# ajgupta93/d4pg-pytorch

Hardware: NVIDIA H100
Metric: learner grad-steps/sec (batch 256, 51 atoms) (higher is better)
Workload: dtype f32

## Files before the change

d4pg-pytorch_b200/csrc/adam.cu:

```cuda
#include "adam_dev.cuh"
#include <math.h>
#include <cmath>
#include <algorithm>

namespace d4pg {

__global__ void __launch_bounds__(256) adam_polyak_kernel(const AdamArgs a) {
  __shared__ float red[2][8];
  pdl_trigger(a.pdl);
  pdl_wait();
  if (int(blockIdx.y) == a.nseg) {
    if (blockIdx.x == 0) adam_tail(a, red);
    return;
  }
  step_stamp(a.trace, 7);
  adam_segment<false>(a, blockIdx.y, blockIdx.x, gridDim.x);
  step_stamp(a.trace, 7 + 16);
  pdl_trigger_end(a.pdl);
}

__global__ void __launch_bounds__(256) adam_polyak_clip_kernel(const AdamArgs a) {
  __shared__ float red[2][8];
  __shared__ double bcast;
  pdl_trigger(a.pdl);
  pdl_wait();
  if (int(blockIdx.y) == a.nseg) {
    if (blockIdx.x == 0) adam_tail(a, red);
    return;
  }
  step_stamp(a.trace, 7);
  adam_segment<true>(a, blockIdx.y, blockIdx.x, gridDim.x, &bcast);
  step_stamp(a.trace, 7 + 16);
  pdl_trigger_end(a.pdl);
}

static_assert(GRAD_NORM_CTAS == 64, "clip_coef sums the partials as one warp, two per lane");
__global__ void __launch_bounds__(256) grad_sqnorm_kernel(const GradNormArgs a) {
  __shared__ double red[8];
  pdl_trigger(a.pdl);
  pdl_wait();
  const int sg = blockIdx.y;
  const float4* g4 = reinterpret_cast<const float4*>(sg ? a.g[1] : a.g[0]);
  const int64_t n4 = (sg ? a.n[1] : a.n[0]) >> 2;
  double acc = 0.0;
  for (int64_t i = blockIdx.x * int64_t(256) + threadIdx.x; i < n4; i += int64_t(GRAD_NORM_CTAS) * 256) {
    const float4 g = g4[i];
    const double x = g.x, y = g.y, z = g.z, w = g.w;
    acc += (x * x + y * y) + (z * z + w * w);
  }
  acc = warp_sum_f64(acc);
  if ((threadIdx.x & 31) == 0) red[threadIdx.x >> 5] = acc;
  __syncthreads();
  if (threadIdx.x == 0) {
    double s = 0.0;
    for (int w = 0; w < 8; ++w) s += red[w];
    (sg ? a.partials[1] : a.partials[0])[blockIdx.x] = s;
  }
  pdl_trigger_end(a.pdl);
}

int launch_grad_sqnorm(const AdamArgs& a, cudaStream_t st) {
  GradNormArgs n{};
  for (int i = 0; i < a.nseg; ++i)
    if (a.seg[i].sq_partials) {
      n.g[n.nseg] = a.seg[i].g; n.partials[n.nseg] = const_cast<double*>(a.seg[i].sq_partials); n.n[n.nseg] = a.seg[i].n;
      ++n.nseg;
    }
  D4PG_REQUIRE(n.nseg > 0, D4PG_EINVAL, "launch_grad_sqnorm: no segment clips");
  n.pdl = pdl_mode();
  D4PG_MAX_CARVEOUT(grad_sqnorm_kernel);
  D4PG_CUDA_OK(launch_pdl(grad_sqnorm_kernel, dim3(GRAD_NORM_CTAS, n.nseg), dim3(256), 0, st, n));
  return D4PG_OK;
}


int launch_adam(const AdamArgs& a_in, cudaStream_t st) {
  AdamArgs a = a_in;
  a.pdl = pdl_mode();
  a.trace = (a.clock && debug_trace_buffer()) ? debug_trace_buffer() + STEP_TRACE_BASE : nullptr;
  int64_t nmax = 0;
  for (int i = 0; i < a.nseg; ++i) nmax = a.seg[i].n > nmax ? a.seg[i].n : nmax;
  int blocks = int((nmax / 4 + 255) / 256);
  if (blocks > 4 * device_sm_count()) blocks = 4 * device_sm_count();
  if (blocks < 1) blocks = 1;
  const int tail = ((a.clock || a.loss_out) && !a.skip_tail) ? 1 : 0;
  bool ex = adam_clips(a);
  for (int i = 0; i < a.nseg; ++i) ex = ex || a.seg[i].wd != 0.f;
  if (ex) {
    D4PG_MAX_CARVEOUT(adam_polyak_clip_kernel);
    D4PG_CUDA_OK(launch_pdl(adam_polyak_clip_kernel, dim3(blocks, a.nseg + tail), dim3(256), 0, st, a));
    return D4PG_OK;
  }
  D4PG_MAX_CARVEOUT(adam_polyak_kernel);
  D4PG_CUDA_OK(launch_pdl(adam_polyak_kernel, dim3(blocks, a.nseg + tail), dim3(256), 0, st, a));
  return D4PG_OK;
}

}

using namespace d4pg;

extern "C" int32_t d4pg_adam_polyak_ex(float* p, const float* g, float* m, float* v, float* target, int64_t n,
                                       double lr, double beta1, double beta2, double eps, int64_t step,
                                       double tau, float grad_scale, d4pg_stream_t stream,
                                       double weight_decay, double max_grad_norm, double* partials, float* norm_out) {
  D4PG_REQUIRE(p && g && m && v, D4PG_EINVAL, "d4pg_adam_polyak: null buffer");
  D4PG_REQUIRE(n > 0 && n % 4 == 0, D4PG_EINVAL, "d4pg_adam_polyak: n must be a positive multiple of 4 (flat layout is 4-aligned)");
  D4PG_REQUIRE(step >= 1, D4PG_EINVAL, "d4pg_adam_polyak: step is the post-increment count (>= 1)");
  D4PG_REQUIRE(std::isfinite(weight_decay) && weight_decay >= 0.0, D4PG_EINVAL,
               "d4pg_adam_polyak_ex: weight_decay must be finite and >= 0 (got %g)", weight_decay);
  D4PG_REQUIRE(max_grad_norm == 0.0 || max_grad_norm > 0.0, D4PG_EINVAL,
               "d4pg_adam_polyak_ex: max_grad_norm must be 0 (off), +inf (report only) or > 0 (got %g)", max_grad_norm);
  D4PG_REQUIRE(max_grad_norm == 0.0 || partials, D4PG_EINVAL,
               "d4pg_adam_polyak_ex: clipping needs a device workspace of %d doubles", GRAD_NORM_CTAS);
  AdamArgs a{};
  const double bc1 = 1.0 - pow(beta1, double(step));
  const double bc2 = 1.0 - pow(beta2, double(step));
  a.seg[0] = AdamSeg{p, g, m, v, target, n, nullptr, 0, float(-(lr / bc1)), -1};
  a.seg[0].wd = float(weight_decay);
  if (max_grad_norm > 0.0) { a.seg[0].sq_partials = partials; a.seg[0].max_norm = max_grad_norm; a.seg[0].norm_out = norm_out; }
  a.nseg = 1;
  a.w1 = float(1.0 - beta1); a.w2 = float(1.0 - beta2); a.beta2 = float(beta2); a.eps = float(eps);
  a.bc2_sqrt = float(sqrt(bc2)); a.tau = float(tau); a.one_minus_tau = float(1.0 - tau);
  a.grad_scale = grad_scale; a.pipe_slot = -1;
  if (adam_clips(a))
    if (int rc = launch_grad_sqnorm(a, as_stream(stream))) return rc;
  return launch_adam(a, as_stream(stream));
}

extern "C" int32_t d4pg_adam_polyak(float* p, const float* g, float* m, float* v, float* target, int64_t n,
                                    double lr, double beta1, double beta2, double eps, int64_t step,
                                    double tau, float grad_scale, d4pg_stream_t stream) {
  return d4pg_adam_polyak_ex(p, g, m, v, target, n, lr, beta1, beta2, eps, step, tau, grad_scale, stream, 0.0, 0.0, nullptr, nullptr);
}

namespace d4pg {
__global__ void polyak_kernel(float* t, const float* s, int64_t n, float tau, float omt) {
  for (int64_t i = blockIdx.x * int64_t(blockDim.x) + threadIdx.x; i < n; i += int64_t(gridDim.x) * blockDim.x)
    t[i] = __fadd_rn(__fmul_rn(omt, t[i]), __fmul_rn(tau, s[i]));
}
}

extern "C" int32_t d4pg_polyak(float* target, const float* src, int64_t n, double tau, d4pg_stream_t stream) {
  D4PG_REQUIRE(target && src && n > 0, D4PG_EINVAL, "d4pg_polyak: bad arguments");
  int blocks = int(std::min<int64_t>(4 * d4pg::device_sm_count(), (n + 255) / 256));
  polyak_kernel<<<blocks, 256, 0, as_stream(stream)>>>(target, src, n, float(tau), float(1.0 - tau));
  D4PG_LAUNCH_OK();
  return D4PG_OK;
}

extern "C" int32_t d4pg_copy_f32(float* dst, const float* src, int64_t n, d4pg_stream_t stream) {
  D4PG_REQUIRE(dst && src && n >= 0, D4PG_EINVAL, "d4pg_copy_f32: bad arguments");
  D4PG_CUDA_OK(cudaMemcpyAsync(dst, src, size_t(n) * sizeof(float), cudaMemcpyDeviceToDevice, as_stream(stream)));
  return D4PG_OK;
}
```

d4pg-pytorch_b200/csrc/adam.cuh:

```cuda
#pragma once
#include "common.cuh"

namespace d4pg {

struct LearnerClock {
  int64_t adam_step;
  int64_t beta_t;
  int64_t steps_done;
  int64_t reserved;
  float beta;
  float neg_step_size[2];
  float bc2_sqrt;
  float pad;
  int64_t s_adam_step, s_beta_t, s_steps_done;
  float d_neg_step_size[2][2];
  float d_bc2_sqrt[2];
};

struct ClockParams {
  double lr_actor, lr_critic, beta1, beta2;
  double per_beta0, per_beta_final; int64_t per_beta_iters;
};

__device__ __forceinline__ void clock_derive_pipelined(LearnerClock* c, const ClockParams& a, int slot) {
  const double step = double(c->s_adam_step + 1);
  const double bc1 = 1.0 - pow(a.beta1, step);
  const double bc2 = 1.0 - pow(a.beta2, step);
  c->d_neg_step_size[slot][0] = float(-(a.lr_actor / bc1));
  c->d_neg_step_size[slot][1] = float(-(a.lr_critic / bc1));
  c->d_bc2_sqrt[slot] = float(sqrt(bc2));
}
__device__ __forceinline__ void clock_derive(LearnerClock* c, const ClockParams& a) {
  const double step = double(c->adam_step + 1);
  const double bc1 = 1.0 - pow(a.beta1, step);
  const double bc2 = 1.0 - pow(a.beta2, step);
  c->neg_step_size[0] = float(-(a.lr_actor / bc1));
  c->neg_step_size[1] = float(-(a.lr_critic / bc1));
  c->bc2_sqrt = float(sqrt(bc2));
}
__device__ __forceinline__ float clock_beta(const LearnerClock* c, const ClockParams& a, bool pipelined = false) {
  const double frac = fmin(double(pipelined ? c->s_beta_t : c->beta_t) / double(a.per_beta_iters), 1.0);
  return float(a.per_beta0 + frac * (a.per_beta_final - a.per_beta0));
}

constexpr int D4PG_MAX_PEERS = 8;
struct PeerSignal {
  unsigned long long* local;
  unsigned long long* inbox[8];
  int world;
};
__device__ __forceinline__ void peer_signal_last_cta(const PeerSignal& s, unsigned nblocks) {
  __threadfence();
  unsigned long long* f = s.local;
  if (atomicAdd(f + 2, 1ull) == nblocks - 1) {
    f[2] = 0ull;
    const unsigned long long v = f[1] + 1ull;
    f[1] = v;
    __threadfence_system();
    for (int p = 0; p < s.world; ++p) asm volatile("st.relaxed.sys.global.u64 [%0], %1;" ::"l"(s.inbox[p]), "l"(v) : "memory");
  }
}
__device__ __forceinline__ void peer_wait_all(const unsigned long long* block, int world) {
  const int r = threadIdx.x;
  if (r < world) {
    const unsigned long long target = __ldcg(block + 1);
    unsigned long long v;
    do {
      asm volatile("ld.acquire.sys.global.u64 %0, [%1];" : "=l"(v) : "l"(block + 8 + r) : "memory");
    } while (v < target);
  }
  __syncthreads();
}

struct PeerInfo {
  int world, rank; int64_t n;
  float* x[D4PG_MAX_PEERS]; float* red[D4PG_MAX_PEERS];
  unsigned long long* flag[D4PG_MAX_PEERS]; unsigned long long* flag2[D4PG_MAX_PEERS];
  const float* mc; float* mc_uc;
};

struct AdamImgLayer { int64_t w_off, w_end; int ld, nchunks; uint8_t* img; uint8_t* img_t; };
struct AdamSeg {
  float* p; const float* g; float* m; float* v; float* target; int64_t n;
  float* g_out; int64_t g_off;
  float neg_step_size; int clock_slot;
  AdamImgLayer imgl[4]; int nimg;
  const double* sq_partials;
  double max_norm;
  float* norm_out;
  float wd;
};
struct AdamArgs {
  AdamSeg seg[2]; int nseg;
  float w1, w2, beta2, eps, bc2_sqrt, tau, one_minus_tau, grad_scale;
  LearnerClock* clock;
  unsigned long long* trace;
  const float* peer_g[D4PG_MAX_PEERS]; int npeers;
  const float* mc_g;
  int peer_reduced;
  const unsigned long long* my_flags; int rank;
  int pipe_slot;
  const float* loss_rows; const float* pi_rows; int B; float inv_count; float* loss_out;
  int pdl;
  int skip_tail;
};
int launch_adam(const AdamArgs& a, cudaStream_t st);

constexpr int GRAD_NORM_CTAS = 64;
constexpr double GRAD_NORM_EPS = 1e-6;
struct GradNormArgs { const float* g[2]; double* partials[2]; int64_t n[2]; int nseg; int pdl; };
static inline bool adam_clips(const AdamArgs& a) {
  for (int i = 0; i < a.nseg; ++i) if (a.seg[i].sq_partials) return true;
  return false;
}
int launch_grad_sqnorm(const AdamArgs& a, cudaStream_t st);


}
```

d4pg-pytorch_b200/csrc/common.cuh:

```cuda
#pragma once
#include <cuda_runtime.h>
#include <stdint.h>
#include <stdio.h>
#include <stdarg.h>
#include "../../include/d4pg_b200.h"

namespace d4pg {

void set_error(const char* fmt, ...);

#define D4PG_CUDA_OK(expr)                                                              \
  do {                                                                                  \
    cudaError_t _e = (expr);                                                            \
    if (_e != cudaSuccess) {                                                            \
      ::d4pg::set_error("%s:%d: %s -> %s", __FILE__, __LINE__, #expr, cudaGetErrorString(_e)); \
      return D4PG_ECUDA;                                                                \
    }                                                                                   \
  } while (0)

#define D4PG_REQUIRE(cond, code, ...)                                                   \
  do {                                                                                  \
    if (!(cond)) { ::d4pg::set_error(__VA_ARGS__); return (code); }                     \
  } while (0)

#define D4PG_LAUNCH_OK()                                                                \
  do {                                                                                  \
    cudaError_t _e = cudaGetLastError();                                                \
    if (_e != cudaSuccess) {                                                            \
      ::d4pg::set_error("%s:%d: kernel launch -> %s", __FILE__, __LINE__, cudaGetErrorString(_e)); \
      return D4PG_ECUDA;                                                                \
    }                                                                                   \
  } while (0)

#define D4PG_MAX_CARVEOUT(kernel)                                                                     \
  do {                                                                                                \
    static bool _carved = false;                                                                      \
    if (!_carved) {                                                                                   \
      cudaFuncSetAttribute(kernel, cudaFuncAttributePreferredSharedMemoryCarveout,                    \
                           int(cudaSharedmemCarveoutMaxShared));                                      \
      _carved = true;                                                                                 \
    }                                                                                                 \
  } while (0)

__device__ __forceinline__ void pdl_trigger_raw() { asm volatile("griddepcontrol.launch_dependents;" ::: "memory"); }
__device__ __forceinline__ void pdl_trigger(int mode) { if (mode == 1) pdl_trigger_raw(); }
__device__ __forceinline__ void pdl_trigger_end(int mode) { if (mode == 2) pdl_trigger_raw(); }
int pdl_mode();
int device_sm_count();
__device__ __forceinline__ void pdl_wait() { asm volatile("griddepcontrol.wait;" ::: "memory"); }
bool pdl_enabled();
template <typename... KArgs, typename... Args>
static inline cudaError_t launch_pdl(void (*kernel)(KArgs...), dim3 grid, dim3 block, size_t smem, cudaStream_t st,
                                     Args... args) {
  cudaLaunchConfig_t cfg{};
  cfg.gridDim = grid; cfg.blockDim = block; cfg.dynamicSmemBytes = smem; cfg.stream = st;
  cudaLaunchAttribute attr[1];
  attr[0].id = cudaLaunchAttributeProgrammaticStreamSerialization;
  attr[0].val.programmaticStreamSerializationAllowed = 1;
  cfg.attrs = attr; cfg.numAttrs = pdl_enabled() ? 1 : 0;
  return cudaLaunchKernelEx(&cfg, kernel, KArgs(args)...);
}

__device__ __forceinline__ void step_stamp(unsigned long long* tr, int slot) {
  if (tr && blockIdx.x == 0 && blockIdx.y == 0 && threadIdx.x == 0) {
    unsigned long long t;
    asm volatile("mov.u64 %0, %%globaltimer;" : "=l"(t));
    tr[slot] = t;
  }
}
unsigned long long* debug_trace_buffer();
constexpr int STEP_TRACE_BASE = 96;

static inline cudaStream_t as_stream(d4pg_stream_t s) { return reinterpret_cast<cudaStream_t>(s); }

__host__ __device__ static inline int64_t align4(int64_t x) { return (x + 3) & ~int64_t(3); }
__host__ __device__ static inline int cdiv(int a, int b) { return (a + b - 1) / b; }

__device__ __forceinline__ float warp_sum(float v) {
#pragma unroll
  for (int o = 16; o > 0; o >>= 1) v += __shfl_xor_sync(0xffffffffu, v, o);
  return v;
}
__device__ __forceinline__ float warp_max(float v) {
#pragma unroll
  for (int o = 16; o > 0; o >>= 1) v = fmaxf(v, __shfl_xor_sync(0xffffffffu, v, o));
  return v;
}

struct Philox {
  __device__ static inline void round(uint32_t (&c)[4], uint32_t k0, uint32_t k1) {
    const uint32_t M0 = 0xD2511F53u, M1 = 0xCD9E8D57u;
    uint32_t hi0 = __umulhi(M0, c[0]), lo0 = M0 * c[0];
    uint32_t hi1 = __umulhi(M1, c[2]), lo1 = M1 * c[2];
    uint32_t n0 = hi1 ^ c[1] ^ k0, n1 = lo1, n2 = hi0 ^ c[3] ^ k1, n3 = lo0;
    c[0] = n0; c[1] = n1; c[2] = n2; c[3] = n3;
  }
  __device__ static inline double uniform53(uint64_t seed, uint64_t counter, uint32_t lane) {
    uint32_t c[4] = {uint32_t(counter), uint32_t(counter >> 32), lane, 0x9E3779B9u};
    uint32_t k0 = uint32_t(seed), k1 = uint32_t(seed >> 32);
#pragma unroll
    for (int i = 0; i < 10; ++i) {
      round(c, k0, k1);
      k0 += 0x9E3779B9u; k1 += 0xBB67AE85u;
    }
    uint32_t a = c[0] >> 5, b = c[1] >> 6;
    return (double(a) * 67108864.0 + double(b)) * (1.0 / 9007199254740992.0);
  }
};

enum GemmEpi {
  EPI_NONE = 0, EPI_BIAS = 1, EPI_BIAS_RELU = 2, EPI_BIAS_TANH = 3,
  EPI_RELU_MASK = 4,
  EPI_TANH_MASK = 5
};
struct NetDims {
  int in[4], out[4];
  int ld[4];
  int epi[4];
  int64_t w_off[4], b_off[4];
  int64_t total;
};
static inline int dx_mask(const NetDims& d, int l) {
  return l > 0 && d.epi[l - 1] == EPI_BIAS_RELU ? EPI_RELU_MASK : EPI_NONE;
}
__host__ __device__ static inline int pitch4(int x) { return (x + 3) & ~3; }
NetDims actor_dims(int obs_dim, int act_dim);
NetDims critic_dims(int obs_dim, int act_dim, int n_atoms);

}
```

d4pg-pytorch_b200/csrc/gemm_ffma.cu:

```cuda
#include "gemm_ffma_dev.cuh"
#include "mlp_chain.cuh"
#include <algorithm>

namespace d4pg {

template <bool ALLOW_SPLIT>
__global__ void __launch_bounds__(GEMM_THREADS, 2) gemm_ffma_kernel(const __grid_constant__ GemmBatch batch) {
  __shared__ __align__(16) float smem[2 * KC * LDS_A + 2 * KC * LDS_B];
  static_assert(2 * KC * LDS_A + 2 * KC * LDS_B >= GEMM_WARPS * BM * BN, "partial-tile buffer must fit");
  pdl_trigger(batch.pdl);
  pdl_wait();
  int pi = 0;
#pragma unroll
  for (int i = 1; i < GEMM_MAX_PROBLEMS; ++i)
    if (i < batch.n && int(blockIdx.x) >= batch.p[i].tile_begin) pi = i;
  const GemmProblem P = batch.p[pi];
  gemm_tile_dispatch<ALLOW_SPLIT>(P, smem, blockIdx.x - P.tile_begin);
  pdl_trigger_end(batch.pdl);
}

template <bool ALLOW_SPLIT>
__global__ void __launch_bounds__(GEMM_THREADS, 3) gemm_wide_kernel(const __grid_constant__ GemmWideBatch batch) {
  extern __shared__ __align__(16) float smem[];
  pdl_trigger(batch.pdl);
  pdl_wait();
  int pi = 0;
#pragma unroll
  for (int i = 1; i < GEMM_WIDE_MAX; ++i)
    if (i < batch.n && int(blockIdx.x) >= batch.p[i].tile_begin) pi = i;
  const GemmProblem& P = batch.p[pi];
  const int tile = blockIdx.x - P.tile_begin;
  step_stamp(batch.trace, 6);
  if (ALLOW_SPLIT && P.ksplit > 1) {
    const int per_slice = P.tiles_m * P.tiles_n;
    const int ks = tile / per_slice, t2 = tile - ks * per_slice;
    const int tm = t2 / P.tiles_n, tn = t2 - tm * P.tiles_n;
    const int kbeg = ks * P.kslice;
    gemm_dw_tile_async<true>(P, smem, tm * BM, tn * BN, tn, kbeg, min(P.K, kbeg + P.kslice));
  } else {
    const int tm = tile / P.tiles_n, tn = tile - tm * P.tiles_n;
    gemm_dw_tile_async<false>(P, smem, tm * BM, tn * BN, tn, 0, P.K);
  }
  step_stamp(batch.trace, 6 + 16);
  if (batch.has_peer_sig) {
    __syncthreads();
    if (threadIdx.x == 0) peer_signal_last_cta(batch.peer_sig, gridDim.x);
  }
  pdl_trigger_end(batch.pdl);
}

GemmProblem gemm_fwd(const float* X, int ldx, const float* X2, int ldx2, int K1, const float* W, int ldw,
                     const float* bias, float* Y, int ldy, int M, int N, int K, int epi) {
  GemmProblem p{};
  p.A = X; p.lda = ldx; p.A2 = X2 ? X2 : X; p.lda2 = X2 ? ldx2 : ldx; p.K1 = X2 ? K1 : K;
  p.Bm = W; p.ldb = ldw; p.bias = bias; p.C = Y; p.ldc = ldy; p.M = M; p.N = N; p.K = K;
  p.mode = GEMM_FWD; p.epi = epi;
  return p;
}
GemmProblem gemm_dx(const float* dZ, int lddz, const float* W, int ldw, float* dX, int lddx,
                    int M, int N_in, int K_out, int epi, const float* aux, int ldaux) {
  GemmProblem p{};
  p.A = dZ; p.lda = lddz; p.A2 = dZ; p.lda2 = lddz; p.K1 = K_out;
  p.Bm = W; p.ldb = ldw; p.C = dX; p.ldc = lddx; p.M = M; p.N = N_in; p.K = K_out;
  p.mode = GEMM_DX; p.epi = epi; p.aux = aux; p.ldaux = ldaux;
  return p;
}
GemmProblem gemm_dw(const float* dZ, int lddz, const float* X, int ldx, float* dW, int lddw,
                    float* db, int N_out, int K_in, int M_batch) {
  GemmProblem p{};
  p.A = dZ; p.lda = lddz; p.A2 = dZ; p.lda2 = lddz; p.K1 = M_batch;
  p.Bm = X; p.ldb = ldx; p.C = dW; p.ldc = lddw; p.bias_grad = db;
  p.M = N_out; p.N = K_in; p.K = M_batch;
  p.mode = GEMM_DW; p.epi = EPI_NONE;
  return p;
}
void gemm_batch_begin(GemmBatch& b) { b.n = 0; b.total_tiles = 0; b.trace = nullptr; }
static bool aligned16(const void* p) { return (reinterpret_cast<uintptr_t>(p) & 15) == 0; }
static void prepare_problem(GemmProblem& p) {
  bool avec, bvec;
  if (p.mode == GEMM_DW) avec = aligned16(p.A) && p.lda % 4 == 0 && p.M % 4 == 0;
  else avec = aligned16(p.A) && p.lda % 4 == 0 && p.K1 % 4 == 0;
  if (p.mode == GEMM_FWD) bvec = aligned16(p.Bm) && p.ldb % 4 == 0 && p.K % 4 == 0;
  else bvec = aligned16(p.Bm) && p.ldb % 4 == 0 && p.N % 4 == 0;
  p.flags = (avec ? GEMM_A_VEC : 0) | (bvec ? GEMM_B_VEC : 0);
  if (p.mode == GEMM_DW && aligned16(p.A) && p.lda % 4 == 0 && aligned16(p.Bm) && p.ldb % 4 == 0) p.flags |= GEMM_ASYNC_OK;
  p.ksplit = 1; p.kslice = p.K;
  if (p.mode == GEMM_DW && p.K >= 1024) {
    p.ksplit = std::min(8, cdiv(p.K, 512));
    p.kslice = cdiv(cdiv(p.K, p.ksplit), 64) * 64;
    p.ksplit = cdiv(p.K, p.kslice);
  }
  p.tiles_m = cdiv(p.M, BM); p.tiles_n = cdiv(p.N, BN);
}
void gemm_batch_add(GemmBatch& b, const GemmProblem& pin) {
  GemmProblem p = pin;
  prepare_problem(p);
  p.tile_begin = b.total_tiles;
  b.total_tiles += p.tiles_m * p.tiles_n * p.ksplit;
  b.p[b.n++] = p;
}
void gemm_batch_retile(GemmBatch& b, int bm, int bn) {
  b.total_tiles = 0;
  for (int i = 0; i < b.n; ++i) {
    GemmProblem& p = b.p[i];
    p.tiles_m = cdiv(p.M, bm); p.tiles_n = cdiv(p.N, bn); p.tile_begin = b.total_tiles;
    b.total_tiles += p.tiles_m * p.tiles_n * p.ksplit;
  }
}
void gemm_wide_begin(GemmWideBatch& b, const PeerSignal* sig) {
  b.n = 0; b.total_tiles = 0; b.pdl = 0; b.trace = nullptr; b.has_peer_sig = sig ? 1 : 0;
  if (sig) b.peer_sig = *sig;
}
void gemm_wide_add(GemmWideBatch& b, const GemmProblem& pin) {
  if (b.n >= GEMM_WIDE_MAX) { b.n = GEMM_WIDE_MAX + 1; return; }
  GemmProblem p = pin;
  prepare_problem(p);
  p.tile_begin = b.total_tiles;
  b.total_tiles += p.tiles_m * p.tiles_n * p.ksplit;
  b.p[b.n++] = p;
}
int gemm_wide_launch(GemmWideBatch& b, cudaStream_t st) {
  D4PG_REQUIRE(b.n > 0 && b.n <= GEMM_WIDE_MAX, D4PG_EINVAL, "gemm_wide_launch: %d problems (max %d)", b.n, GEMM_WIDE_MAX);
  bool split = false;
  for (int i = 0; i < b.n; ++i) {
    split = split || b.p[i].ksplit > 1;
    D4PG_REQUIRE(b.p[i].mode == GEMM_DW && (b.p[i].flags & GEMM_ASYNC_OK), D4PG_ENOTSUP,
                 "gemm_wide_launch: problem %d is not a dW with 16-B aligned, 16-B pitched operands", i);
  }
  D4PG_MAX_CARVEOUT(gemm_wide_kernel<false>);
  D4PG_MAX_CARVEOUT(gemm_wide_kernel<true>);
  const size_t smem = DW_SMEM_FLOATS * sizeof(float);
  static bool smem_set = false;
  if (!smem_set) {
    D4PG_CUDA_OK(cudaFuncSetAttribute(gemm_wide_kernel<false>, cudaFuncAttributeMaxDynamicSharedMemorySize, int(smem)));
    D4PG_CUDA_OK(cudaFuncSetAttribute(gemm_wide_kernel<true>, cudaFuncAttributeMaxDynamicSharedMemorySize, int(smem)));
    smem_set = true;
  }
  b.pdl = pdl_mode();
  b.trace = debug_trace_buffer() ? debug_trace_buffer() + STEP_TRACE_BASE : nullptr;
  if (split) D4PG_CUDA_OK(launch_pdl(gemm_wide_kernel<true>, dim3(b.total_tiles), dim3(GEMM_THREADS), smem, st, b));
  else D4PG_CUDA_OK(launch_pdl(gemm_wide_kernel<false>, dim3(b.total_tiles), dim3(GEMM_THREADS), smem, st, b));
  return D4PG_OK;
}
bool gemm_batch_has_splitk(const GemmBatch& b) {
  for (int i = 0; i < b.n; ++i) if (b.p[i].ksplit > 1) return true;
  return false;
}
int gemm_launch(GemmBatch& b, int precision, cudaStream_t st) {
  if (precision == 0) return gemm_batch_launch(b, st);
  if (precision == 3) return gemm_bf16_batch_launch(b, st);
  gemm_tc_prepare(b);
  return gemm_tc_batch_launch(b, precision == 1 ? 3 : 1, st);
}
int gemm_batch_launch(const GemmBatch& b, cudaStream_t st) {
  D4PG_REQUIRE(b.n > 0 && b.n <= GEMM_MAX_PROBLEMS, D4PG_EINVAL, "gemm_batch_launch: %d problems", b.n);
  for (int i = 0; i < b.n; ++i)
    D4PG_REQUIRE(b.p[i].mode != GEMM_FWD || b.p[i].K1 == b.p[i].K || b.p[i].K1 % KC == 0, D4PG_ENOTSUP,
                 "gemm_batch_launch: concat split K1=%d must be a multiple of %d", b.p[i].K1, KC);
  D4PG_MAX_CARVEOUT(gemm_ffma_kernel<false>);
  D4PG_MAX_CARVEOUT(gemm_ffma_kernel<true>);
  const_cast<GemmBatch&>(b).pdl = pdl_mode();
  if (gemm_batch_has_splitk(b)) D4PG_CUDA_OK(launch_pdl(gemm_ffma_kernel<true>, dim3(b.total_tiles), dim3(GEMM_THREADS), 0, st, b));
  else D4PG_CUDA_OK(launch_pdl(gemm_ffma_kernel<false>, dim3(b.total_tiles), dim3(GEMM_THREADS), 0, st, b));
  return D4PG_OK;
}

}
```

d4pg-pytorch_b200/csrc/learner.cu:

```cuda
#include "common.cuh"
#include "gemm_ffma.cuh"
#include "adam.cuh"
#include <string.h>
#include <stdlib.h>
#include <initializer_list>
#include <new>
#include <string>
#include <vector>

#include "internal.cuh"
#include "mlp_chain.cuh"
#include "mlp_tc_chain.cuh"

namespace d4pg {

struct Batch { float *s, *a, *s2; double* r; uint8_t* done; int32_t* idx; float* wts; uint8_t* hz; };

struct Workspace {
  Batch batch[2];
  float *h1[5], *h2[5], *h3[5], *out[5];
  float *m, *q_probs, *target_probs, *dlogits_q, *dlogits_pi, *loss_rows, *pi_rows;
  float *c_dz22, *c_dz2, *c_dz1, *p_dz22, *p_dz2, *a_dz3, *a_dz22, *a_dh2, *a_dz1;
  LearnerClock* clock;
  float* xchg;
  unsigned long long* pipe_epoch;
  double* sq_partials;
  int64_t total;
};

enum StepPlan { PLAN_LEVELS, PLAN_CHAIN, PLAN_TC_CHAIN };
constexpr int CHAIN_MAX_BATCH = 512;
static bool chain_pre_ok(const d4pg_learner_config_t& c) { return c.precision == 0 && c.act_dim <= 8; }
static bool chain_plan_fits(const d4pg_learner_config_t& c) {
  const int H = D4PG_HIDDEN, S = c.obs_dim, A = c.act_dim, N = c.n_atoms;
  ChainArgs f, b;
  chain_args_begin(f, c.batch, nullptr, c.precision);
  chain_add(f, 0, chain_fwd(nullptr, 0, nullptr, H, S, EPI_BIAS_RELU, nullptr, 0, 1));
  chain_add(f, 0, chain_fwd(nullptr, 0, nullptr, H, H, EPI_BIAS_RELU, nullptr, 0, 1));
  ChainSlot fc2 = chain_fwd(nullptr, 0, nullptr, H, H + A, EPI_BIAS_RELU, nullptr, 0, 1);
  if (chain_pre_ok(c)) chain_pre_layer(fc2, nullptr, 0, nullptr, nullptr, 0, A, H, EPI_BIAS_TANH, nullptr, 0, 0, H, false);
  else chain_add(f, 0, chain_fwd(nullptr, 0, nullptr, A, H, EPI_BIAS_TANH, nullptr, 0, 1));
  chain_add(f, 0, fc2);
  chain_add(f, 0, chain_fwd(nullptr, 0, nullptr, N, H, EPI_BIAS, nullptr, 0, 0));
  chain_args_begin(b, c.batch, nullptr, c.precision);
  chain_add(b, 0, chain_dx(nullptr, 0, H, N, EPI_RELU_MASK, nullptr, 0, nullptr, 0, 1));
  chain_add(b, 0, chain_dx(nullptr, 0, H, H, EPI_RELU_MASK, nullptr, 0, nullptr, 0, 1));
  ChainSlot fc3 = chain_dx(nullptr, 0, H, A, EPI_RELU_MASK, nullptr, 0, nullptr, 0, 1);
  if (chain_pre_ok(c)) chain_pre_layer(fc3, nullptr, 0, nullptr, nullptr, 0, A, H, EPI_TANH_MASK, nullptr, 0, 0, H, true);
  else chain_add(b, 0, chain_dx(nullptr, 0, A, H, EPI_TANH_MASK, nullptr, 0, nullptr, 0, 1));
  chain_add(b, 0, fc3);
  return chain_fits(f) && chain_fits(b);
}
static StepPlan step_plan(const d4pg_learner_config_t& c) {
  if (c.batch > CHAIN_MAX_BATCH || c.chain != 1) return PLAN_LEVELS;
  if (c.precision == 3) return PLAN_LEVELS;
  if (c.precision >= 1 && c.obs_dim <= 32 && c.act_dim <= 32 && c.n_atoms <= 256) return PLAN_TC_CHAIN;
  return chain_plan_fits(c) ? PLAN_CHAIN : PLAN_LEVELS;
}
static d4pg_learner_config_t with_head_width(const d4pg_learner_config_t& c) {
  d4pg_learner_config_t e = c;
  if (c.dist_type == 1) e.n_atoms = 3 * c.n_components;
  return e;
}
static_assert((CHAIN_MAX_BATCH + SAMPLE_ROWS - 1) / SAMPLE_ROWS <= TCC_THREADS, "sampler epochs exceed the chain CTA's threads");

static Workspace carve(float* base, int B, int S, int A, int N, StepPlan plan, bool prefetch, bool clip, bool tails) {
  Workspace w{};
  int64_t off = 0;
  auto take = [&](int64_t n) { float* p = base ? base + off : nullptr; off += align4(n); return p; };
  const int H = D4PG_HIDDEN, Sp = pitch4(S), Ap = pitch4(A), Np = pitch4(N);
  auto take_rows = [&](Batch& h) {
    h.s = take(int64_t(B) * Sp); h.a = take(int64_t(B) * Ap); h.s2 = take(int64_t(B) * Sp);
    h.r = reinterpret_cast<double*>(take(int64_t(B) * 2));
    h.done = reinterpret_cast<uint8_t*>(take((B + 3) / 4));
  };
  take_rows(w.batch[0]);
  for (int k = 0; k < 5; ++k) {
    if (k != 4) w.h1[k] = take(int64_t(B) * H);
    w.h2[k] = take(int64_t(B) * H); w.h3[k] = take(int64_t(B) * H);
  }
  w.out[0] = take(int64_t(B) * Ap); w.out[3] = take(int64_t(B) * Ap);
  w.out[1] = take(int64_t(B) * Np); w.out[2] = take(int64_t(B) * Np); w.out[4] = take(int64_t(B) * Np);
  w.m = take(int64_t(B) * Np); w.q_probs = take(int64_t(B) * Np); w.target_probs = take(int64_t(B) * Np);
  w.dlogits_q = take(int64_t(B) * Np); w.dlogits_pi = take(int64_t(B) * Np);
  w.loss_rows = take(B); w.pi_rows = take(B);
  w.c_dz22 = take(int64_t(B) * H); w.c_dz2 = take(int64_t(B) * H); w.c_dz1 = take(int64_t(B) * H);
  w.p_dz22 = take(int64_t(B) * H); w.p_dz2 = take(int64_t(B) * H);
  w.a_dz3 = take(int64_t(B) * Ap); w.a_dz22 = take(int64_t(B) * H); w.a_dh2 = take(int64_t(B) * H);
  w.a_dz1 = take(int64_t(B) * H);
  w.clock = reinterpret_cast<LearnerClock*>(take(sizeof(LearnerClock) / 4 + 4));
  w.xchg = plan != PLAN_LEVELS ? take(std::max(chain_xchg_floats(B), tcc_xchg_floats(B))) : nullptr;
  w.pipe_epoch = reinterpret_cast<unsigned long long*>(take(2 * int64_t((B + SAMPLE_ROWS - 1) / SAMPLE_ROWS)));
  if (prefetch) {
    take_rows(w.batch[1]);
    for (int k = 0; k < 2; ++k) { w.batch[k].idx = reinterpret_cast<int32_t*>(take(B)); w.batch[k].wts = take(B); }
  }
  if (clip) w.sq_partials = reinterpret_cast<double*>(take(2 * GRAD_NORM_CTAS * 2));
  if (tails)
    for (int k = 0; k < (prefetch ? 2 : 1); ++k) w.batch[k].hz = reinterpret_cast<uint8_t*>(take((B + 3) / 4));
  w.total = off;
  return w;
}
}

using namespace d4pg;

struct d4pg_learner {
  d4pg_learner_config_t cfg;
  d4pg_learner_buffers_t buf;
  d4pg_replay* replay;
  d4pg_comm* comm;
  StepPlan plan;
  Workspace ws;
  NetDims da, dc;
  ClockParams clock_params;
  cudaGraphExec_t graph_exec[4];
  bool graph_ready[4];
  cudaGraphExec_t multi_exec[2];
  bool multi_ready[2];
  int pipe_par;
  int last_par;
  bool prefetch_valid;
  int64_t seen_gen;
  int64_t steps_done;
  int kernels_per_step;
  cudaStream_t side; cudaEvent_t ev_fork, ev_join;
  ChainArgs chain_fwd_args, chain_bwd_args;
  uint8_t* tcc_images; TccPackArgs tcc_pack_fwd, tcc_pack_dx; TccImage tcc_img[32];
  cudaEvent_t ev_fork2, ev_join2;
  TccArgs tcc_fwd_args, tcc_bwd_args;
  GemmWideBatch dw_batch;
  double* host_u[4]; int32_t* host_pos[4]; float* host_losses; cudaEvent_t ev_in, ev_out, ev_h2d[4];
  int64_t host_steps;
  float* loss_ring[2]; cudaEvent_t ev_loss[2]; int64_t loss_steps;
  cudaStream_t ing; cudaEvent_t ev_ing; unsigned long long* gate_flag;
  bool images_dirty;
  const float* norm_affine; float norm_clip;
  double* gtab;
  bool profiling;
  std::vector<cudaEvent_t> ev;
  std::vector<std::string> ev_name;
  std::vector<int> ev_reps;
};

static bool prefetching(const d4pg_learner_config_t& c) { return c.prefetch != 0 && c.sample_mode == 1; }
static bool host_pipe(const d4pg_learner_config_t& c) { return c.prefetch != 0 && c.sample_mode == 0 && c.use_graph != 0; }
static bool piped(const d4pg_learner_config_t& c) { return prefetching(c) || host_pipe(c); }
static bool clipping(const d4pg_learner_config_t& c) { return c.max_grad_norm_actor != 0.0 || c.max_grad_norm_critic != 0.0; }

enum Net { ACTOR, ACTOR_TARGET, CRITIC, CRITIC_TARGET };
struct Layer { const float* W; int ldw; const float* bias; int n_out, k_in, epi; };
static Layer layer(const d4pg_learner* L, Net net, int l) {
  const bool critic = net >= CRITIC;
  const NetDims& d = critic ? L->dc : L->da;
  const float* P[4] = {L->buf.actor, L->buf.actor_target, L->buf.critic, L->buf.critic_target};
  return Layer{P[net] + d.w_off[l], d.ld[l], P[net] + d.b_off[l], d.out[l], d.in[l], d.epi[l]};
}
static int64_t critic_fc2_action_off(const d4pg_learner* L) { return L->dc.w_off[1] + D4PG_HIDDEN; }
struct LayerDx { const float* W; int ldw, n_in, k_out; };
static LayerDx layer_dx(const d4pg_learner* L, Net net, int l) {
  const Layer y = layer(L, net, l);
  return LayerDx{y.W, y.ldw, (net == CRITIC && l == 1) ? D4PG_HIDDEN : y.k_in, y.n_out};
}
static LayerDx critic_fc2_action_dx(const d4pg_learner* L) {
  return LayerDx{L->buf.critic + critic_fc2_action_off(L), L->dc.ld[1], L->cfg.act_dim, D4PG_HIDDEN};
}

enum { U_A_F1, U_A_F2, U_A_F22, U_A_F3, U_A_D3, U_A_D22, U_A_D2, U_AT_F1, U_AT_F2, U_AT_F22, U_AT_F3,
       U_C_F1, U_C_F2, U_C_F22, U_C_F3, U_C_D3, U_C_D22, U_C_D2H, U_C_D2A, U_CT_F1, U_CT_F2, U_CT_F22, U_CT_F3, U_COUNT };
static int fwd_image(Net net, int l) {
  const int fc1[4] = {U_A_F1, U_AT_F1, U_C_F1, U_CT_F1};
  return fc1[net] + l;
}

static int tcc_setup(d4pg_learner* L) {
  TccPackArgs& pf = L->tcc_pack_fwd; TccPackArgs& pd = L->tcc_pack_dx;
  tcc_pack_begin(pf, nullptr); tcc_pack_begin(pd, nullptr);
  int use_of[U_COUNT]; bool is_dx[U_COUNT];
  auto add_dx = [&](int id, const LayerDx& d) {
    is_dx[id] = true;
    use_of[id] = tcc_pack_add(pd, d.W, d.ldw, GEMM_DX, d.n_in, d.k_out);
  };
  for (int net = ACTOR; net <= CRITIC_TARGET; ++net)
    for (int l = 0; l < 4; ++l) {
      const Layer y = layer(L, Net(net), l);
      const int id = fwd_image(Net(net), l);
      is_dx[id] = false;
      use_of[id] = tcc_pack_add(pf, y.W, y.ldw, GEMM_FWD, y.n_out, y.k_in);
    }
  add_dx(U_A_D3, layer_dx(L, ACTOR, 3));
  add_dx(U_A_D22, layer_dx(L, ACTOR, 2));
  add_dx(U_A_D2, layer_dx(L, ACTOR, 1));
  add_dx(U_C_D3, layer_dx(L, CRITIC, 3));
  add_dx(U_C_D22, layer_dx(L, CRITIC, 2));
  add_dx(U_C_D2H, layer_dx(L, CRITIC, 1));
  add_dx(U_C_D2A, critic_fc2_action_dx(L));
  for (int i = 0; i < U_COUNT; ++i) D4PG_REQUIRE(use_of[i] >= 0, D4PG_ENOTSUP, "tcc_setup: too many weight images");
  const long long fwd_bytes = tcc_pack_bytes(pf), all_bytes = fwd_bytes + tcc_pack_bytes(pd);
  D4PG_CUDA_OK(cudaMalloc(&L->tcc_images, size_t(all_bytes)));
  D4PG_CUDA_OK(cudaMemset(L->tcc_images, 0, size_t(all_bytes)));
  tcc_pack_set_base(pf, L->tcc_images, 0);
  tcc_pack_set_base(pd, L->tcc_images, fwd_bytes);
  for (int i = 0; i < U_COUNT; ++i) L->tcc_img[i] = tcc_image(is_dx[i] ? pd : pf, use_of[i]);
  (void)tcc_watchdog_device();
  return D4PG_OK;
}

enum Exchange { XCHG_NONE, XCHG_ALLREDUCE, XCHG_PULL, XCHG_MC, XCHG_MC2, XCHG_RS };
static Exchange exchange_mode(d4pg_learner* L, PeerInfo* peers) {
  if (L->cfg.world_size <= 1) return XCHG_NONE;
  if (!comm_peer_info(L->comm, peers)) return XCHG_ALLREDUCE;
  static const int comm_mode = [] { const char* e = getenv("D4PG_COMM_MODE");
                                    return !e ? 0 : (e[0] == 'p' ? 1 : (e[0] == 'r' ? 2 : (e[0] == 'm' && e[1] == 'c' && e[2] == '2' ? 4 : 3))); }();
  static const int mc_from = [] { const char* e = getenv("D4PG_COMM_MC_FROM"); return e ? atoi(e) : 3; }();
  static const int mc2_from = [] { const char* e = getenv("D4PG_COMM_MC2_FROM"); return e ? atoi(e) : 1000; }();
  const bool mc_avail = peers->mc != nullptr && L->plan != PLAN_LEVELS;
  if (mc_avail && (comm_mode == 4 || (comm_mode == 0 && peers->world >= mc2_from))) return XCHG_MC2;
  if (mc_avail && (comm_mode == 3 || (comm_mode == 0 && peers->world >= mc_from))) return XCHG_MC;
  return comm_mode == 2 ? XCHG_RS : XCHG_PULL;
}

struct Step {
  d4pg_learner* L; cudaStream_t st;
  const d4pg_learner_config_t& c; const d4pg_learner_buffers_t& b; const Workspace& w;
  Batch bt;
  int par; bool cold;
  bool pf;
  bool h7;
  int B, S, A, N, Sp, Ap, Np;
  Exchange xm; PeerInfo peers; int gpar;
  float *Ga, *Gc;
  int nk;
};
static bool peer_exchange(const Step& x) { return x.xm >= XCHG_PULL; }

constexpr int PROFILE_REPS = 16;
template <class F>
static int run_launch(Step& x, const char* name, bool repeatable, F launch) {
  d4pg_learner* L = x.L;
  int rc;
  if (L->profiling) {
    cudaEvent_t e0, e1; cudaEventCreate(&e0); cudaEventCreate(&e1);
    cudaEventRecord(e0, x.st); rc = launch();
    for (int r = 1; repeatable && r < PROFILE_REPS && rc == 0; ++r) rc = launch();
    cudaEventRecord(e1, x.st);
    L->ev.push_back(e0); L->ev.push_back(e1); L->ev_reps.push_back(repeatable ? PROFILE_REPS : 1);
    L->ev_name.push_back(name);
  } else rc = launch();
  if (rc == 0) ++x.nk;
  return rc;
}
#define RUN(name, repeatable, call) \
  do { if (int rc_ = run_launch(x, name, repeatable, [&] { return (call); })) return rc_; } while (0)
static int run_level(Step& x, std::initializer_list<GemmProblem> problems) {
  GemmBatch g;
  gemm_batch_begin(g);
  for (const GemmProblem& p : problems) gemm_batch_add(g, p);
  RUN("gemm_launch", !gemm_batch_has_splitk(g), gemm_launch(g, x.c.precision, x.st));
  return D4PG_OK;
}

static int sample_batch(Step& x) {
  const d4pg_learner_config_t& c = x.c;
  RUN("learner_sample", false,
      learner_sample(x.L->replay, x.B, c.prioritized, c.sample_mode == 0 ? x.b.uniforms : nullptr,
                     (c.sample_mode == 0 && !c.prioritized) ? x.b.positions : nullptr,
                     c.philox_seed, x.w.clock, x.L->clock_params,
                     x.bt.idx, x.bt.wts, x.bt.s, x.bt.a, x.bt.r, x.bt.s2, x.bt.done, x.bt.hz, x.Sp, x.Ap, x.L->norm_affine,
                     x.L->norm_clip, x.pf ? x.par : -1, x.st));
  return D4PG_OK;
}

static void tcc_begin(const Step& x, TccArgs& a, int step_slot) {
  tcc_args_begin(a, x.B, reinterpret_cast<uint8_t*>(x.w.xchg), x.c.precision == 1 ? 3 : 1);
  a.step_slot = step_slot;
}
static int tcc_fwd_group(TccArgs& fa, int ci, int sl, const Step& x, Net net, int l, float* C, int ldc, int publish) {
  const Layer y = layer(x.L, net, l);
  return tcc_slot_group(fa, ci, sl, x.L->tcc_img[fwd_image(net, l)], y.epi, y.bias, nullptr, 0, C, ldc, publish);
}
static void tcc_build_actor_critic(TccArgs& fa, int ci, const Step& x, Net an, Net cn, const float* s, int ka, int kc,
                                   bool keep, bool actor_only = false) {
  const Workspace& w = x.w;
  const int H = D4PG_HIDDEN;
  int l, p1, p2 = -1;
  tcc_chain_x0(fa, ci, s, x.Sp, x.S);
  l = tcc_slot_begin(fa, ci); tcc_slot_src_x(fa, ci, l);
  p1 = tcc_fwd_group(fa, ci, l, x, an, 0, keep ? w.h1[ka] : nullptr, H, 1);
  if (!actor_only) p2 = tcc_fwd_group(fa, ci, l, x, cn, 0, nullptr, H, 1);
  l = tcc_slot_begin(fa, ci); tcc_slot_src_plane(fa, ci, l, p1, 8);
  p1 = tcc_fwd_group(fa, ci, l, x, an, 1, keep ? w.h2[ka] : nullptr, H, 1);
  l = tcc_slot_begin(fa, ci); tcc_slot_src_plane(fa, ci, l, p1, 8);
  p1 = tcc_fwd_group(fa, ci, l, x, an, 2, keep ? w.h3[ka] : nullptr, H, 1);
  l = tcc_slot_begin(fa, ci); tcc_slot_src_plane(fa, ci, l, p1, 8);
  const int pa = tcc_fwd_group(fa, ci, l, x, an, 3, w.out[ka], x.Ap, 1);
  if (actor_only) return;
  l = tcc_slot_begin(fa, ci); tcc_slot_src_plane(fa, ci, l, p2, 8); tcc_slot_src_plane(fa, ci, l, pa, 1);
  p1 = tcc_fwd_group(fa, ci, l, x, cn, 1, keep ? w.h2[kc] : nullptr, H, 1);
  l = tcc_slot_begin(fa, ci); tcc_slot_src_plane(fa, ci, l, p1, 8);
  p1 = tcc_fwd_group(fa, ci, l, x, cn, 2, keep ? w.h3[kc] : nullptr, H, 1);
  l = tcc_slot_begin(fa, ci); tcc_slot_src_plane(fa, ci, l, p1, 8);
  tcc_fwd_group(fa, ci, l, x, cn, 3, w.out[kc], x.Np, 0);
}
static void tcc_build_Q(TccArgs& fa, int ci, const Step& x, const float* act, float* h1, float* h2, float* h3, float* logits) {
  const int H = D4PG_HIDDEN;
  int l, p1;
  tcc_chain_x0(fa, ci, x.bt.s, x.Sp, x.S);
  l = tcc_slot_begin(fa, ci); tcc_slot_src_x(fa, ci, l); tcc_slot_reconvert_x(fa, ci, l, act, x.Ap, x.A);
  p1 = tcc_fwd_group(fa, ci, l, x, CRITIC, 0, h1, H, 1);
  l = tcc_slot_begin(fa, ci); tcc_slot_src_plane(fa, ci, l, p1, 8); tcc_slot_src_x(fa, ci, l);
  p1 = tcc_fwd_group(fa, ci, l, x, CRITIC, 1, h2, H, 1);
  l = tcc_slot_begin(fa, ci); tcc_slot_src_plane(fa, ci, l, p1, 8);
  p1 = tcc_fwd_group(fa, ci, l, x, CRITIC, 2, h3, H, 1);
  l = tcc_slot_begin(fa, ci); tcc_slot_src_plane(fa, ci, l, p1, 8);
  tcc_fwd_group(fa, ci, l, x, CRITIC, 3, logits, x.Np, 0);
}
static int forward_tc_chain(Step& x, bool pack_fwd) {
  d4pg_learner* L = x.L; const Workspace& w = x.w;
  if (pack_fwd) RUN("launch_tcc_pack", false, launch_tcc_pack(L->tcc_pack_fwd, x.st));
  D4PG_CUDA_OK(cudaEventRecord(L->ev_fork2, x.st));
  D4PG_CUDA_OK(cudaStreamWaitEvent(L->side, L->ev_fork2, 0));
  RUN("launch_tcc_pack", false, launch_tcc_pack(L->tcc_pack_dx, L->side));
  D4PG_CUDA_OK(cudaEventRecord(L->ev_join2, L->side));
  TccArgs& fa = L->tcc_fwd_args;
  tcc_begin(x, fa, 1);
  tcc_build_actor_critic(fa, 0, x, ACTOR_TARGET, CRITIC_TARGET, x.bt.s2, 0, 1, false);
  tcc_build_actor_critic(fa, 1, x, ACTOR, CRITIC, x.bt.s, 3, 4, true, x.h7);
  tcc_build_Q(fa, 2, x, x.bt.a, w.h1[2], w.h2[2], w.h3[2], w.out[2]);
  if (host_pipe(x.c) && !x.cold) {
    fa.wait_epoch = w.pipe_epoch; fa.wait_clock = reinterpret_cast<const long long*>(&w.clock->steps_done);
    fa.wait_n = cdiv(x.B, SAMPLE_ROWS);
  }
  RUN("launch_mlp_tc_chain", true, launch_mlp_tc_chain(fa, x.st));
  return D4PG_OK;
}

static ChainSlot chain_layer(const Step& x, Net net, int l, float* C, int ldc, int publish) {
  const Layer y = layer(x.L, net, l);
  return chain_fwd(y.W, y.ldw, y.bias, y.n_out, y.k_in, y.epi, C, ldc, publish);
}
static void chain_build_actor_critic(const Step& x, ChainArgs& ca, int ci, Net an, Net cn, const float* s, int ka,
                                     float* c_h1, int kc) {
  const Workspace& w = x.w;
  const int H = D4PG_HIDDEN;
  ChainSlot sl; int t, a3 = -1;
  sl = chain_layer(x, an, 0, w.h1[ka], H, 1); chain_src_global(sl, s, x.Sp); t = chain_add(ca, ci, sl);
  sl = chain_layer(x, an, 1, w.h2[ka], H, 1); chain_src_plane(sl, t); t = chain_add(ca, ci, sl);
  sl = chain_layer(x, an, 2, w.h3[ka], H, 1); chain_src_plane(sl, t); const int a22 = chain_add(ca, ci, sl);
  if (!chain_pre_ok(x.c)) { sl = chain_layer(x, an, 3, w.out[ka], x.Ap, 1); chain_src_plane(sl, a22); a3 = chain_add(ca, ci, sl); }
  sl = chain_layer(x, cn, 0, c_h1, H, 1); chain_src_global(sl, s, x.Sp); t = chain_add(ca, ci, sl);
  sl = chain_layer(x, cn, 1, w.h2[kc], H, 1); chain_src_plane(sl, t);
  if (chain_pre_ok(x.c)) {
    const Layer y = layer(x.L, an, 3);
    chain_pre_layer(sl, y.W, y.ldw, y.bias, nullptr, 0, y.n_out, y.k_in, y.epi, w.out[ka], x.Ap, a22, H, false);
  } else chain_src2_plane(sl, H, a3);
  t = chain_add(ca, ci, sl);
  sl = chain_layer(x, cn, 2, w.h3[kc], H, 1); chain_src_plane(sl, t); t = chain_add(ca, ci, sl);
  sl = chain_layer(x, cn, 3, w.out[kc], x.Np, 0); chain_src_plane(sl, t); chain_add(ca, ci, sl);
}
static int forward_chain(Step& x) {
  const Workspace& w = x.w;
  const int H = D4PG_HIDDEN;
  ChainArgs& ca = x.L->chain_fwd_args;
  chain_args_begin(ca, x.B, w.xchg, x.c.precision);
  chain_build_actor_critic(x, ca, 0, ACTOR_TARGET, CRITIC_TARGET, x.bt.s2, 0, w.h1[1], 1);
  ChainSlot sl; int t;
  sl = chain_layer(x, CRITIC, 0, w.h1[2], H, 1); chain_src_global(sl, x.bt.s, x.Sp); t = chain_add(ca, 2, sl);
  sl = chain_layer(x, CRITIC, 1, w.h2[2], H, 1); chain_src_plane(sl, t); chain_src2_global(sl, H, x.bt.a, x.Ap); t = chain_add(ca, 2, sl);
  sl = chain_layer(x, CRITIC, 2, w.h3[2], H, 1); chain_src_plane(sl, t); t = chain_add(ca, 2, sl);
  sl = chain_layer(x, CRITIC, 3, w.out[2], x.Np, 0); chain_src_plane(sl, t); chain_add(ca, 2, sl);
  chain_build_actor_critic(x, ca, 1, ACTOR, CRITIC, x.bt.s, 3, nullptr, 4);
  RUN("launch_mlp_chain", true, launch_mlp_chain(ca, x.st));
  return D4PG_OK;
}

static GemmProblem level_fwd(const Step& x, Net net, int l, const float* X, int ldx, float* Y, int ldy,
                             const float* act = nullptr) {
  const Layer y = layer(x.L, net, l);
  return gemm_fwd(X, ldx, act, act ? x.Ap : 0, act ? D4PG_HIDDEN : 0, y.W, y.ldw, y.bias, Y, ldy, x.B, y.n_out, y.k_in, y.epi);
}
static int forward_levels(Step& x) {
  const Workspace& w = x.w; const Batch& bt = x.bt;
  const int H = D4PG_HIDDEN, Sp = x.Sp, Ap = x.Ap, Np = x.Np;
  int rc = run_level(x, {level_fwd(x, ACTOR_TARGET, 0, bt.s2, Sp, w.h1[0], H),
                         level_fwd(x, CRITIC_TARGET, 0, bt.s2, Sp, w.h1[1], H),
                         level_fwd(x, CRITIC, 0, bt.s, Sp, w.h1[2], H),
                         level_fwd(x, ACTOR, 0, bt.s, Sp, w.h1[3], H)});
  if (!rc) rc = run_level(x, {level_fwd(x, ACTOR_TARGET, 1, w.h1[0], H, w.h2[0], H),
                              level_fwd(x, CRITIC, 1, w.h1[2], H, w.h2[2], H, bt.a),
                              level_fwd(x, ACTOR, 1, w.h1[3], H, w.h2[3], H)});
  if (!rc) rc = run_level(x, {level_fwd(x, ACTOR_TARGET, 2, w.h2[0], H, w.h3[0], H),
                              level_fwd(x, CRITIC, 2, w.h2[2], H, w.h3[2], H),
                              level_fwd(x, ACTOR, 2, w.h2[3], H, w.h3[3], H)});
  if (!rc) rc = run_level(x, {level_fwd(x, ACTOR_TARGET, 3, w.h3[0], H, w.out[0], Ap),
                              level_fwd(x, CRITIC, 3, w.h3[2], H, w.out[2], Np),
                              level_fwd(x, ACTOR, 3, w.h3[3], H, w.out[3], Ap)});
  if (!rc) rc = run_level(x, {level_fwd(x, CRITIC_TARGET, 1, w.h1[1], H, w.h2[1], H, w.out[0]),
                              level_fwd(x, CRITIC, 1, w.h1[2], H, w.h2[4], H, w.out[3])});
  if (!rc) rc = run_level(x, {level_fwd(x, CRITIC_TARGET, 2, w.h2[1], H, w.h3[1], H),
                              level_fwd(x, CRITIC, 2, w.h2[4], H, w.h3[4], H)});
  if (!rc) rc = run_level(x, {level_fwd(x, CRITIC_TARGET, 3, w.h3[1], H, w.out[1], Np),
                              level_fwd(x, CRITIC, 3, w.h3[4], H, w.out[4], Np)});
  return rc;
}

static HeadCommon head_common(const Step& x, bool only_policy) {
  const d4pg_learner_config_t& c = x.c; const Workspace& w = x.w;
  HeadCommon h{};
  h.target = w.out[1]; h.q = w.out[2]; h.pi = (x.h7 && !only_policy) ? nullptr : w.out[4];
  h.rewards = x.bt.r; h.dones = x.bt.done; h.B = x.B; h.ld = x.Np;
  h.discount = (c.proj_mode == 1) ? pow(c.gamma, double(c.n_steps)) : c.gamma; h.prio_eps = c.prio_eps;
  h.grad_scale = 1.0f / (float(x.B) * float(c.world_size > 1 ? c.world_size : 1));
  h.loss_rows = w.loss_rows; h.td = x.b.td; h.prio = x.b.prio; h.dq = w.dlogits_q;
  h.pi_rows = w.pi_rows; h.dpi = w.dlogits_pi;
  h.is_weights = ((c.loss_flags & 1) && c.prioritized) ? x.bt.wts : nullptr;
  h.only_policy = only_policy ? 1 : 0;
  h.sampler_clock = (x.pf && !only_policy) ? w.clock : nullptr;
  h.horizon = x.bt.hz; h.gtab = x.L->gtab;
  return h;
}
static int launch_step_heads(Step& x, bool only_policy) {
  const d4pg_learner_config_t& c = x.c; const Workspace& w = x.w;
  const HeadCommon h = head_common(x, only_policy);
  const int ce_priority = (c.loss_flags & 2) ? 1 : 0;
  const bool rep = !x.pf;
  if (c.dist_type == 1) {
    MogArgs ma{h, c.n_components};
    RUN("launch_mog_heads", rep, launch_mog_heads(ma, x.st));
  } else if (c.dist_type == 2) {
    QrArgs qa{h, x.N, c.qr_kappa, ce_priority};
    RUN("launch_qr_heads", rep, launch_qr_heads(qa, x.st));
  } else {
    HeadsArgs ha{};
    ha.h = h; ha.N = x.N; ha.ce_priority = ce_priority;
    ha.v_min = c.v_min; ha.delta = (c.v_max - c.v_min) / double(x.N - 1);
    ha.v_max = proj_clip_top(c.v_min, c.v_max, x.N, ha.delta);
    ha.m = w.m; ha.target_probs = w.target_probs; ha.q_probs = w.q_probs;
    RUN("launch_heads", rep, launch_heads(ha, c.proj_mode, x.st));
  }
  return D4PG_OK;
}

static int side_branch(Step& x) {
  d4pg_learner* L = x.L; const d4pg_learner_config_t& c = x.c;
  D4PG_CUDA_OK(cudaEventRecord(L->ev_fork, x.st));
  D4PG_CUDA_OK(cudaStreamWaitEvent(L->side, L->ev_fork, 0));
  if (c.prioritized)
    RUN("launch_tree_update", false,
        launch_tree_update(L->replay, x.B, x.bt.idx, x.b.prio, L->side, host_pipe(c) ? L->gate_flag : nullptr));
  else if (host_pipe(c)) RUN("launch_gate_signal", false, launch_gate_signal(L->gate_flag, L->side));
  if (prefetching(c)) {
    const int q = x.par ^ 1;
    const Batch& o = x.w.batch[q];
    RUN("learner_sample", false,
        learner_sample(L->replay, x.B, c.prioritized, nullptr, nullptr, c.philox_seed, x.w.clock, L->clock_params,
                       o.idx, o.wts, o.s, o.a, o.r, o.s2, o.done, o.hz, x.Sp, x.Ap, L->norm_affine, L->norm_clip, q, L->side));
  }
  if (x.pf) {
    D4PG_CUDA_OK(cudaMemcpyAsync(x.b.idx, x.bt.idx, size_t(x.B) * sizeof(int32_t), cudaMemcpyDeviceToDevice, L->side));
    if (x.b.weights && c.prioritized)
      D4PG_CUDA_OK(cudaMemcpyAsync(x.b.weights, x.bt.wts, size_t(x.B) * sizeof(float), cudaMemcpyDeviceToDevice, L->side));
  }
  D4PG_CUDA_OK(cudaEventRecord(L->ev_join, L->side));
  return D4PG_OK;
}

static int choose_gradient_buffers(Step& x) {
  const d4pg_learner_buffers_t& b = x.b;
  x.Ga = b.grad_actor; x.Gc = b.grad_critic;
  x.peers = PeerInfo{};
  x.xm = exchange_mode(x.L, &x.peers);
  x.gpar = x.pf ? x.par : int(x.L->steps_done & 1);
  if (peer_exchange(x)) {
    const bool use_mc_buf = x.xm == XCHG_MC || x.xm == XCHG_MC2;
    x.Ga = (use_mc_buf ? x.peers.mc_uc : x.peers.x[x.peers.rank]) + int64_t(x.gpar) * x.peers.n;
    x.Gc = x.Ga + x.L->da.total;
  }
  if (x.B >= 1024)
    D4PG_CUDA_OK(cudaMemsetAsync(x.Ga, 0, size_t(x.L->da.total + x.L->dc.total) * sizeof(float), x.st));
  return D4PG_OK;
}

static void tcc_build_bwd_C(TccArgs& ba, int ci, const Step& x) {
  const TccImage* U = x.L->tcc_img; const Workspace& w = x.w;
  const int H = D4PG_HIDDEN;
  int l, p1;
  tcc_chain_pre(ba, ci, w.dlogits_q, x.Np, x.N);
  l = tcc_slot_begin(ba, ci); tcc_slot_src_pre(ba, ci, l);
  p1 = tcc_slot_group(ba, ci, l, U[U_C_D3], EPI_RELU_MASK, nullptr, w.h3[2], H, w.c_dz22, H, 1);
  l = tcc_slot_begin(ba, ci); tcc_slot_src_plane(ba, ci, l, p1, 8);
  p1 = tcc_slot_group(ba, ci, l, U[U_C_D22], EPI_RELU_MASK, nullptr, w.h2[2], H, w.c_dz2, H, 1);
  l = tcc_slot_begin(ba, ci); tcc_slot_src_plane(ba, ci, l, p1, 8);
  tcc_slot_group(ba, ci, l, U[U_C_D2H], EPI_RELU_MASK, nullptr, w.h1[2], H, w.c_dz1, H, 0);
}
static void tcc_build_bwd_P(TccArgs& ba, int ci, const Step& x) {
  const TccImage* U = x.L->tcc_img; const Workspace& w = x.w;
  const int H = D4PG_HIDDEN;
  int l, p1;
  tcc_chain_pre(ba, ci, w.dlogits_pi, x.Np, x.N);
  l = tcc_slot_begin(ba, ci); tcc_slot_src_pre(ba, ci, l);
  p1 = tcc_slot_group(ba, ci, l, U[U_C_D3], EPI_RELU_MASK, nullptr, w.h3[4], H, nullptr, H, 1);
  l = tcc_slot_begin(ba, ci); tcc_slot_src_plane(ba, ci, l, p1, 8);
  p1 = tcc_slot_group(ba, ci, l, U[U_C_D22], EPI_RELU_MASK, nullptr, w.h2[4], H, nullptr, H, 1);
  l = tcc_slot_begin(ba, ci); tcc_slot_src_plane(ba, ci, l, p1, 8);
  p1 = tcc_slot_group(ba, ci, l, U[U_C_D2A], EPI_TANH_MASK, nullptr, w.out[3], x.Ap, w.a_dz3, x.Ap, 1);
  l = tcc_slot_begin(ba, ci); tcc_slot_src_plane(ba, ci, l, p1, 1);
  p1 = tcc_slot_group(ba, ci, l, U[U_A_D3], EPI_RELU_MASK, nullptr, w.h3[3], H, w.a_dz22, H, 1);
  l = tcc_slot_begin(ba, ci); tcc_slot_src_plane(ba, ci, l, p1, 8);
  p1 = tcc_slot_group(ba, ci, l, U[U_A_D22], EPI_NONE, nullptr, nullptr, 0, w.a_dh2, H, 1);
  l = tcc_slot_begin(ba, ci); tcc_slot_src_plane(ba, ci, l, p1, 8);
  tcc_slot_group(ba, ci, l, U[U_A_D2], EPI_RELU_MASK, nullptr, w.h1[3], H, w.a_dz1, H, 0);
}
static int backward_tc_chain(Step& x) {
  D4PG_CUDA_OK(cudaStreamWaitEvent(x.st, x.L->ev_join2, 0));
  TccArgs& ba = x.L->tcc_bwd_args;
  tcc_begin(x, ba, 5);
  tcc_build_bwd_C(ba, 0, x);
  if (!x.h7) tcc_build_bwd_P(ba, 1, x);
  RUN("launch_mlp_tc_chain", true, launch_mlp_tc_chain(ba, x.st));
  return D4PG_OK;
}

static ChainSlot chain_layer_dx(const LayerDx& d, int epi, const float* aux, int ldaux, float* C, int ldc, int publish) {
  return chain_dx(d.W, d.ldw, d.n_in, d.k_out, epi, aux, ldaux, C, ldc, publish);
}
static int backward_chain(Step& x) {
  d4pg_learner* L = x.L; const Workspace& w = x.w;
  const int H = D4PG_HIDDEN, Ap = x.Ap, Np = x.Np;
  ChainArgs& cb = L->chain_bwd_args;
  chain_args_begin(cb, x.B, w.xchg, x.c.precision); cb.trace_base = 6 * CHAIN_MAX_SLOTS;
  ChainSlot sl; int t;
  sl = chain_layer_dx(layer_dx(L, CRITIC, 3), EPI_RELU_MASK, w.h3[2], H, w.c_dz22, H, 1); chain_src_global(sl, w.dlogits_q, Np); t = chain_add(cb, 0, sl);
  sl = chain_layer_dx(layer_dx(L, CRITIC, 2), EPI_RELU_MASK, w.h2[2], H, w.c_dz2, H, 1); chain_src_plane(sl, t); t = chain_add(cb, 0, sl);
  sl = chain_layer_dx(layer_dx(L, CRITIC, 1), EPI_RELU_MASK, w.h1[2], H, w.c_dz1, H, 0); chain_src_plane(sl, t); chain_add(cb, 0, sl);

  sl = chain_layer_dx(layer_dx(L, CRITIC, 3), EPI_RELU_MASK, w.h3[4], H, w.p_dz22, H, 1); chain_src_global(sl, w.dlogits_pi, Np); t = chain_add(cb, 1, sl);
  sl = chain_layer_dx(layer_dx(L, CRITIC, 2), EPI_RELU_MASK, w.h2[4], H, w.p_dz2, H, 1); chain_src_plane(sl, t); t = chain_add(cb, 1, sl);
  const LayerDx da = critic_fc2_action_dx(L);
  if (chain_pre_ok(x.c)) {
    sl = chain_layer_dx(layer_dx(L, ACTOR, 3), EPI_RELU_MASK, w.h3[3], H, w.a_dz22, H, 1);
    chain_pre_layer(sl, da.W, da.ldw, nullptr, w.out[3], Ap, da.n_in, da.k_out, EPI_TANH_MASK, w.a_dz3, Ap, t, H, true);
    t = chain_add(cb, 1, sl);
  } else {
    sl = chain_layer_dx(da, EPI_TANH_MASK, w.out[3], Ap, w.a_dz3, Ap, 1); chain_src_plane(sl, t); t = chain_add(cb, 1, sl);
    sl = chain_layer_dx(layer_dx(L, ACTOR, 3), EPI_RELU_MASK, w.h3[3], H, w.a_dz22, H, 1); chain_src_plane(sl, t); t = chain_add(cb, 1, sl);
  }
  sl = chain_layer_dx(layer_dx(L, ACTOR, 2), EPI_NONE, nullptr, 0, w.a_dh2, H, 1); chain_src_plane(sl, t); t = chain_add(cb, 1, sl);
  sl = chain_layer_dx(layer_dx(L, ACTOR, 1), EPI_RELU_MASK, w.h1[3], H, w.a_dz1, H, 0); chain_src_plane(sl, t); chain_add(cb, 1, sl);
  RUN("launch_mlp_chain", true, launch_mlp_chain(cb, x.st));
  return D4PG_OK;
}

static GemmProblem dw_problem(const Step& x, Net net, int l) {
  const Workspace& w = x.w; const NetDims& da = x.L->da; const NetDims& dc = x.L->dc;
  const int B = x.B, S = x.S, A = x.A, N = x.N, H = D4PG_HIDDEN, Sp = x.Sp, Ap = x.Ap, Np = x.Np;
  const int* la = da.ld; const int* lc = dc.ld;
  float* Ga = x.Ga; float* Gc = x.Gc;
  if (net == CRITIC) switch (l) {
    case 0: return gemm_dw(w.c_dz1, H, x.bt.s, Sp, Gc + dc.w_off[0], lc[0], Gc + dc.b_off[0], H, S, B);
    case 1: return gemm_dw(w.c_dz2, H, w.h1[2], H, Gc + dc.w_off[1], lc[1], Gc + dc.b_off[1], H, H, B);
    case 2: return gemm_dw(w.c_dz22, H, w.h2[2], H, Gc + dc.w_off[2], lc[2], Gc + dc.b_off[2], H, H, B);
    default: return gemm_dw(w.dlogits_q, Np, w.h3[2], H, Gc + dc.w_off[3], lc[3], Gc + dc.b_off[3], N, H, B);
  }
  switch (l) {
    case 0: return gemm_dw(w.a_dz1, H, x.bt.s, Sp, Ga + da.w_off[0], la[0], Ga + da.b_off[0], H, S, B);
    case 1: return gemm_dw(w.a_dh2, H, w.h1[3], H, Ga + da.w_off[1], la[1], Ga + da.b_off[1], H, H, B);
    case 2: return gemm_dw(w.a_dz22, H, w.h2[3], H, Ga + da.w_off[2], la[2], Ga + da.b_off[2], H, H, B);
    default: return gemm_dw(w.a_dz3, Ap, w.h3[3], H, Ga + da.w_off[3], la[3], Ga + da.b_off[3], A, H, B);
  }
}
static GemmProblem dw_critic_fc2_action(const Step& x) {
  return gemm_dw(x.w.c_dz2, D4PG_HIDDEN, x.bt.a, x.Ap, x.Gc + critic_fc2_action_off(x.L), x.L->dc.ld[1], nullptr,
                 D4PG_HIDDEN, x.A, x.B);
}
static int dw_wide(Step& x, bool critic, bool actor) {
  GemmWideBatch& gw = x.L->dw_batch;
  PeerSignal sig1{};
  if (peer_exchange(x)) sig1 = comm_peer_signal(x.peers, 0);
  gemm_wide_begin(gw, peer_exchange(x) ? &sig1 : nullptr);
  if (critic) gemm_wide_add(gw, dw_problem(x, CRITIC, 2));
  if (critic) gemm_wide_add(gw, dw_problem(x, CRITIC, 1));
  if (actor) gemm_wide_add(gw, dw_problem(x, ACTOR, 2));
  if (actor) gemm_wide_add(gw, dw_problem(x, ACTOR, 1));
  if (critic) gemm_wide_add(gw, dw_problem(x, CRITIC, 3));
  if (critic) gemm_wide_add(gw, dw_critic_fc2_action(x));
  if (critic) gemm_wide_add(gw, dw_problem(x, CRITIC, 0));
  if (actor) gemm_wide_add(gw, dw_problem(x, ACTOR, 3));
  if (actor) gemm_wide_add(gw, dw_problem(x, ACTOR, 0));
  RUN("gemm_wide_launch", false, gemm_wide_launch(gw, x.st));
  return D4PG_OK;
}

static GemmProblem level_dx(const Step& x, const LayerDx& d, const float* dZ, int lddz, float* dX, int lddx, int epi,
                            const float* aux, int ldaux) {
  return gemm_dx(dZ, lddz, d.W, d.ldw, dX, lddx, x.B, d.n_in, d.k_out, epi, aux, ldaux);
}
static int backward_levels(Step& x) {
  d4pg_learner* L = x.L; const Workspace& w = x.w;
  const int H = D4PG_HIDDEN, Ap = x.Ap, Np = x.Np;
  int rc = run_level(x, {level_dx(x, layer_dx(L, CRITIC, 3), w.dlogits_q, Np, w.c_dz22, H, EPI_RELU_MASK, w.h3[2], H),
                         level_dx(x, layer_dx(L, CRITIC, 3), w.dlogits_pi, Np, w.p_dz22, H, EPI_RELU_MASK, w.h3[4], H),
                         dw_problem(x, CRITIC, 3)});
  if (!rc) rc = run_level(x, {level_dx(x, layer_dx(L, CRITIC, 2), w.c_dz22, H, w.c_dz2, H, EPI_RELU_MASK, w.h2[2], H),
                              level_dx(x, layer_dx(L, CRITIC, 2), w.p_dz22, H, w.p_dz2, H, EPI_RELU_MASK, w.h2[4], H),
                              dw_problem(x, CRITIC, 2)});
  if (!rc) rc = run_level(x, {level_dx(x, layer_dx(L, CRITIC, 1), w.c_dz2, H, w.c_dz1, H, EPI_RELU_MASK, w.h1[2], H),
                              level_dx(x, critic_fc2_action_dx(L), w.p_dz2, H, w.a_dz3, Ap, EPI_TANH_MASK, w.out[3], Ap),
                              dw_problem(x, CRITIC, 1),
                              dw_critic_fc2_action(x)});
  if (!rc) rc = run_level(x, {dw_problem(x, CRITIC, 0),
                              level_dx(x, layer_dx(L, ACTOR, 3), w.a_dz3, Ap, w.a_dz22, H, EPI_RELU_MASK, w.h3[3], H),
                              dw_problem(x, ACTOR, 3)});
  if (!rc) rc = run_level(x, {level_dx(x, layer_dx(L, ACTOR, 2), w.a_dz22, H, w.a_dh2, H, EPI_NONE, nullptr, 0),
                              dw_problem(x, ACTOR, 2)});
  if (!rc) rc = run_level(x, {level_dx(x, layer_dx(L, ACTOR, 1), w.a_dh2, H, w.a_dz1, H, EPI_RELU_MASK, w.h1[3], H),
                              dw_problem(x, ACTOR, 1)});
  if (!rc) rc = run_level(x, {dw_problem(x, ACTOR, 0)});
  return rc;
}

static bool inline_sync(const Step& x) { return peer_exchange(x) && x.L->plan != PLAN_LEVELS; }
static int exchange_gradients(Step& x) {
  d4pg_learner* L = x.L;
  if (peer_exchange(x) && !inline_sync(x)) RUN("comm_peer_barrier", false, comm_peer_barrier(L->comm, x.st));
  if (x.xm == XCHG_MC2) RUN("comm_mc_reduce_bcast", false, comm_mc_reduce_bcast(L->comm, x.gpar, x.st));
  else if (x.xm == XCHG_RS) RUN("comm_peer_reduce_scatter", false, comm_peer_reduce_scatter(L->comm, x.gpar, x.st));
  else if (x.xm == XCHG_ALLREDUCE)
    RUN("comm_allreduce", false, comm_allreduce(L->comm, x.Ga, L->da.total + L->dc.total, x.st));
  return D4PG_OK;
}

static AdamArgs adam_args(const Step& x) {
  d4pg_learner* L = x.L; const d4pg_learner_config_t& c = x.c; const d4pg_learner_buffers_t& b = x.b;
  const NetDims& da = L->da; const NetDims& dc = L->dc; const PeerInfo& peers = x.peers;
  AdamArgs aa{};
  aa.seg[0] = AdamSeg{b.actor, x.Ga, b.adam_m_actor, b.adam_v_actor, b.actor_target, da.total, nullptr, 0, 0.f, 0};
  aa.seg[1] = AdamSeg{b.critic, x.Gc, b.adam_m_critic, b.adam_v_critic, b.critic_target, dc.total, nullptr, 0, 0.f, 1};
  if (peer_exchange(x)) {
    aa.npeers = peers.world;
    for (int r = 0; r < peers.world; ++r) aa.peer_g[r] = peers.x[r] + int64_t(x.gpar) * peers.n;
    aa.seg[0].g_out = b.grad_actor; aa.seg[0].g_off = 0;
    aa.seg[1].g_out = b.grad_critic; aa.seg[1].g_off = da.total;
    aa.my_flags = inline_sync(x) ? peers.flag[peers.rank] : nullptr; aa.rank = peers.rank;
    if (x.xm == XCHG_MC) aa.mc_g = peers.mc + int64_t(x.gpar) * peers.n;
    if (x.xm == XCHG_MC2) {
      aa.peer_reduced = 1;
      aa.seg[0].g = peers.mc_uc + 2 * peers.n; aa.seg[1].g = peers.mc_uc + 2 * peers.n + da.total;
      aa.my_flags = peers.flag2[peers.rank];
    }
    if (x.xm == XCHG_RS) {
      aa.peer_reduced = 1;
      aa.seg[0].g = peers.red[peers.rank]; aa.seg[1].g = peers.red[peers.rank] + da.total;
      aa.my_flags = peers.flag2[peers.rank];
    }
  }
  aa.nseg = 2;
  aa.seg[0].wd = float(c.weight_decay_actor); aa.seg[1].wd = float(c.weight_decay_critic);
  const double max_norm[2] = {c.max_grad_norm_actor, c.max_grad_norm_critic};
  for (int sg = 0; sg < 2; ++sg)
    if (max_norm[sg] != 0.0) {
      aa.seg[sg].sq_partials = x.w.sq_partials + sg * GRAD_NORM_CTAS; aa.seg[sg].max_norm = max_norm[sg];
      aa.seg[sg].norm_out = b.losses + 2 + sg;
    }
  if (L->plan == PLAN_TC_CHAIN) {
    const TccImage* U = L->tcc_img;
    const NetDims* nd[2] = {&da, &dc};
    const Net online[2] = {ACTOR, CRITIC}, target[2] = {ACTOR_TARGET, CRITIC_TARGET};
    for (int sg = 0; sg < 2; ++sg) {
      aa.seg[sg].nimg = 4;
      for (int ly = 0; ly < 4; ++ly) {
        AdamImgLayer& I = aa.seg[sg].imgl[ly];
        I.w_off = nd[sg]->w_off[ly]; I.w_end = I.w_off + int64_t(nd[sg]->out[ly]) * nd[sg]->ld[ly];
        I.ld = nd[sg]->ld[ly]; I.nchunks = U[fwd_image(online[sg], ly)].kchunks;
        I.img = const_cast<uint8_t*>(U[fwd_image(online[sg], ly)].ptr);
        I.img_t = const_cast<uint8_t*>(U[fwd_image(target[sg], ly)].ptr);
      }
    }
  }
  aa.w1 = float(1.0 - c.beta1); aa.w2 = float(1.0 - c.beta2); aa.beta2 = float(c.beta2); aa.eps = float(c.adam_eps);
  aa.tau = float(c.tau); aa.one_minus_tau = float(1.0 - c.tau); aa.grad_scale = 1.0f; aa.clock = x.w.clock;
  aa.pipe_slot = x.pf ? x.par : -1;
  aa.loss_rows = x.w.loss_rows; aa.pi_rows = x.w.pi_rows; aa.B = x.B; aa.inv_count = 1.0f / float(x.B); aa.loss_out = b.losses;
  return aa;
}
static int launch_update(Step& x, const AdamArgs& a) {
  if (adam_clips(a)) RUN("launch_grad_sqnorm", true, launch_grad_sqnorm(a, x.st));
  RUN("launch_adam", false, launch_adam(a, x.st));
  return D4PG_OK;
}
static int post_update_half(Step& x, const AdamArgs& aa) {
  d4pg_learner* L = x.L; const Workspace& w = x.w;
  AdamArgs ac = aa;
  ac.seg[0] = aa.seg[1]; ac.nseg = 1; ac.skip_tail = 1;
  if (int rc = launch_update(x, ac)) return rc;
  RUN("launch_tcc_pack", false, launch_tcc_pack(L->tcc_pack_dx, x.st));
  TccArgs& fb = L->tcc_fwd_args;
  tcc_begin(x, fb, 1);
  tcc_build_Q(fb, 0, x, w.out[3], nullptr, w.h2[4], w.h3[4], w.out[4]);
  RUN("launch_mlp_tc_chain", true, launch_mlp_tc_chain(fb, x.st));
  if (int rc = launch_step_heads(x, true)) return rc;
  TccArgs& bb = L->tcc_bwd_args;
  tcc_begin(x, bb, 5);
  tcc_build_bwd_P(bb, 0, x);
  RUN("launch_mlp_tc_chain", true, launch_mlp_tc_chain(bb, x.st));
  if (int rc = dw_wide(x, false, true)) return rc;
  AdamArgs ab = aa;
  ab.nseg = 1;
  return launch_update(x, ab);
}

static int update(Step& x) {
  const AdamArgs aa = adam_args(x);
  if (x.h7) return post_update_half(x, aa);
  return launch_update(x, aa);
}

static int enqueue_step(d4pg_learner* L, cudaStream_t st, int par, bool cold, bool pack_fwd) {
  const d4pg_learner_config_t& c = L->cfg;
  const bool pf = piped(c);
  Step x{L, st, c, L->buf, L->ws, L->ws.batch[par], par, cold, pf, (c.loss_flags & 4) != 0,
         c.batch, c.obs_dim, c.act_dim, c.n_atoms, pitch4(c.obs_dim), pitch4(c.act_dim), pitch4(c.n_atoms)};
  const StepPlan plan = L->plan;
  const bool side = c.prioritized || pf;
  int rc = (!pf || cold) ? sample_batch(x) : D4PG_OK;
  if (!rc) rc = plan == PLAN_TC_CHAIN ? forward_tc_chain(x, pack_fwd) : plan == PLAN_CHAIN ? forward_chain(x) : forward_levels(x);
  if (!rc) rc = launch_step_heads(x, false);
  if (!rc && side) rc = side_branch(x);
  if (!rc) rc = choose_gradient_buffers(x);
  if (!rc && plan == PLAN_TC_CHAIN) rc = backward_tc_chain(x);
  if (!rc && plan == PLAN_CHAIN) rc = backward_chain(x);
  if (!rc) rc = plan == PLAN_LEVELS ? backward_levels(x) : dw_wide(x, true, !x.h7);
  if (!rc) rc = exchange_gradients(x);
  if (!rc) rc = update(x);
  if (rc) return rc;
  if (side) D4PG_CUDA_OK(cudaStreamWaitEvent(st, L->ev_join, 0));
  L->kernels_per_step = x.nk;
  return D4PG_OK;
}
#undef RUN

extern "C" int64_t d4pg_learner_workspace_floats(const d4pg_learner_config_t* cfg) {
  if (!cfg) return -1;
  const d4pg_learner_config_t ec = with_head_width(*cfg);
  return carve(nullptr, ec.batch, ec.obs_dim, ec.act_dim, ec.n_atoms, step_plan(ec), piped(ec), clipping(ec),
               ec.nstep_tails != 0).total;
}

extern "C" int32_t d4pg_learner_create(const d4pg_learner_config_t* cfg, const d4pg_learner_buffers_t* buf,
                                       d4pg_replay_t* replay, d4pg_comm_t* comm, d4pg_learner_t** out) {
  D4PG_REQUIRE(cfg && buf && replay && out, D4PG_EINVAL, "d4pg_learner_create: null argument");
  D4PG_REQUIRE(cfg->batch > 0 && cfg->obs_dim > 0 && cfg->act_dim > 0, D4PG_EINVAL, "d4pg_learner_create: bad dims");
  D4PG_REQUIRE(cfg->dist_type >= 0 && cfg->dist_type <= 2, D4PG_EINVAL,
               "d4pg_learner_create: dist_type must be 0 (categorical), 1 (mixture of Gaussians) or 2 (quantile regression)");
  if (cfg->dist_type == 2) {
    D4PG_REQUIRE(cfg->n_atoms >= 2 && cfg->n_atoms <= D4PG_MAX_ATOMS, D4PG_EINVAL,
                 "d4pg_learner_create: the quantile critic's n_atoms (its N quantiles) must be in [2,%d]", D4PG_MAX_ATOMS);
    D4PG_REQUIRE(std::isfinite(cfg->qr_kappa) && cfg->qr_kappa > 0.0, D4PG_EINVAL,
                 "d4pg_learner_create: qr_kappa must be finite and > 0 (got %g)", cfg->qr_kappa);
  } else if (cfg->dist_type == 1) {
    D4PG_REQUIRE(cfg->n_components >= 1 && cfg->n_components <= D4PG_MAX_COMPONENTS, D4PG_EINVAL,
                 "d4pg_learner_create: n_components must be in [1,%d]", D4PG_MAX_COMPONENTS);
    D4PG_REQUIRE(!(cfg->loss_flags & 2), D4PG_ENOTSUP,
                 "d4pg_learner_create: loss_flags & 2 (cross-entropy priority) is not supported by the mixture critic: the cross-entropy of a density can be negative");
  } else {
    D4PG_REQUIRE(cfg->n_atoms >= 2 && cfg->n_atoms <= D4PG_MAX_ATOMS, D4PG_EINVAL, "d4pg_learner_create: n_atoms must be in [2,%d]", D4PG_MAX_ATOMS);
    D4PG_REQUIRE(cfg->v_max > cfg->v_min, D4PG_EINVAL, "d4pg_learner_create: v_max <= v_min");
  }
  const d4pg_learner_config_t ec = with_head_width(*cfg);
  D4PG_REQUIRE(cfg->proj_mode == 0 || cfg->proj_mode == 1, D4PG_EINVAL, "d4pg_learner_create: proj_mode must be 0/1");
  D4PG_REQUIRE(cfg->precision >= 0 && cfg->precision <= 3, D4PG_ENOTSUP,
               "d4pg_learner_create: precision %d unknown (0 fp32 FFMA, 1 3xTF32 wgmma, 2 TF32 wgmma, 3 bf16 wgmma)", cfg->precision);
  D4PG_REQUIRE(!clipping(*cfg) || cfg->world_size <= 1, D4PG_EINVAL,
               "d4pg_learner_create: max_grad_norm is not supported with world_size > 1: the ranks' gradients are summed "
               "inside the Adam kernel, so the norm of the summed gradient does not exist before the update");
  D4PG_REQUIRE(cfg->obs_norm == 0 || cfg->obs_norm == 1, D4PG_EINVAL, "d4pg_learner_create: obs_norm must be 0 or 1");
  D4PG_REQUIRE(!cfg->obs_norm || cfg->world_size <= 1, D4PG_EINVAL,
               "d4pg_learner_create: obs_norm is not supported with world_size > 1: each rank would normalize with the "
               "statistics of its own shard");
  double norm_clip = 0.0;
  const float* norm_affine = cfg->obs_norm ? replay_obs_norm(replay, &norm_clip) : nullptr;
  D4PG_REQUIRE(!cfg->obs_norm || norm_affine, D4PG_EINVAL,
               "d4pg_learner_create: obs_norm needs a replay with an observation normalizer (d4pg_replay_set_obs_norm)");
  D4PG_REQUIRE(cfg->nstep_tails == 0 || cfg->nstep_tails == 1, D4PG_EINVAL, "d4pg_learner_create: nstep_tails must be 0 or 1");
  D4PG_REQUIRE(!cfg->nstep_tails || cfg->proj_mode == 1 || cfg->n_steps <= 1, D4PG_EINVAL,
               "d4pg_learner_create: nstep_tails with proj_mode 0 (gamma for every row) and n_steps > 1: a per-row horizon "
               "has no meaning there");
  D4PG_REQUIRE(!cfg->nstep_tails || replay_horizons(replay), D4PG_EINVAL,
               "d4pg_learner_create: nstep_tails needs a replay with a horizon column (d4pg_replay_set_horizons)");
  D4PG_REQUIRE(cfg->world_size <= 1 || comm, D4PG_EINVAL, "d4pg_learner_create: world_size>1 needs a communicator");
  D4PG_REQUIRE(cfg->chain == 0 || cfg->chain == 1, D4PG_EINVAL, "d4pg_learner_create: chain must be 0 or 1");
  for (double mn : {cfg->max_grad_norm_actor, cfg->max_grad_norm_critic})
    D4PG_REQUIRE(mn == 0.0 || mn > 0.0, D4PG_EINVAL,
                 "d4pg_learner_create: max_grad_norm must be 0 (off), +inf (report only) or > 0 (got %g)", mn);
  for (double wd : {cfg->weight_decay_actor, cfg->weight_decay_critic})
    D4PG_REQUIRE(std::isfinite(wd) && wd >= 0.0, D4PG_EINVAL, "d4pg_learner_create: weight_decay must be finite and >= 0 (got %g)", wd);
  D4PG_REQUIRE(!(cfg->loss_flags & 4) || (step_plan(ec) == PLAN_TC_CHAIN && cfg->world_size <= 1), D4PG_ENOTSUP,
               "d4pg_learner_create: loss_flags & 4 (post-update-critic actor gradient) needs the tensor-core chain plan: precision 1 or 2 (not 0 or 3), chain 1, "
               "batch <= 512, obs_dim <= 32, act_dim <= 32, on one GPU");
  D4PG_REQUIRE(buf->actor && buf->actor_target && buf->critic && buf->critic_target && buf->grad_actor && buf->grad_critic &&
               buf->adam_m_actor && buf->adam_v_actor && buf->adam_m_critic && buf->adam_v_critic &&
               buf->idx && buf->prio && buf->td && buf->losses && buf->workspace, D4PG_EINVAL,
               "d4pg_learner_create: null device buffer");
  d4pg_learner* L = new (std::nothrow) d4pg_learner();
  D4PG_REQUIRE(L, D4PG_EINVAL, "d4pg_learner_create: out of host memory");
  L->cfg = ec; L->buf = *buf; L->replay = replay; L->comm = comm; L->plan = step_plan(ec);
  L->da = actor_dims(cfg->obs_dim, cfg->act_dim);
  L->dc = critic_dims(ec.obs_dim, ec.act_dim, ec.n_atoms);
  if (buf->grad_critic != buf->grad_actor + L->da.total) {
    set_error("d4pg_learner_create: grad_critic must equal grad_actor + P_a (one flat gradient buffer)");
    delete L; return D4PG_EINVAL;
  }
  L->ws = carve(buf->workspace, ec.batch, ec.obs_dim, ec.act_dim, ec.n_atoms, L->plan, piped(ec), clipping(ec),
                ec.nstep_tails != 0);
  if (!piped(ec)) { L->ws.batch[0].idx = buf->idx; L->ws.batch[0].wts = buf->weights; }
  L->clock_params = ClockParams{ec.lr_actor, ec.lr_critic, ec.beta1, ec.beta2, ec.per_beta0, ec.per_beta_final,
                                ec.per_beta_iters > 0 ? ec.per_beta_iters : 1};
  for (int i = 0; i < 4; ++i) { L->graph_exec[i] = nullptr; L->graph_ready[i] = false; }
  for (int i = 0; i < 2; ++i) { L->multi_exec[i] = nullptr; L->multi_ready[i] = false; }
  L->pipe_par = 0; L->last_par = 0; L->prefetch_valid = false; L->seen_gen = -1;
  L->steps_done = 0; L->kernels_per_step = 0;
  L->profiling = false;
  (void)debug_trace_buffer();
  if (L->plan == PLAN_TC_CHAIN)
    if (int rc = tcc_setup(L)) { delete L; return rc; }
  L->host_steps = 0; L->host_losses = nullptr; L->ev_in = nullptr; L->ev_out = nullptr;
  for (int i = 0; i < 4; ++i) { L->host_u[i] = nullptr; L->host_pos[i] = nullptr; L->ev_h2d[i] = nullptr; }
  for (int i = 0; i < 2; ++i) { L->loss_ring[i] = nullptr; L->ev_loss[i] = nullptr; }
  L->loss_steps = 0;
  L->ing = nullptr; L->ev_ing = nullptr; L->gate_flag = nullptr; L->images_dirty = true;
  L->norm_affine = norm_affine; L->norm_clip = float(norm_clip);
  L->gtab = nullptr;
  if (cfg->nstep_tails) {
    double g[D4PG_STEPS_MAX_N];
    for (int k = 0; k < D4PG_STEPS_MAX_N; ++k) g[k] = pow(cfg->gamma, double(k));
    if (cudaMalloc(reinterpret_cast<void**>(&L->gtab), sizeof(g)) != cudaSuccess ||
        cudaMemcpy(L->gtab, g, sizeof(g), cudaMemcpyHostToDevice) != cudaSuccess) {
      set_error("d4pg_learner_create: horizon table upload failed"); delete L; return D4PG_ECUDA;
    }
  }
  if (host_pipe(*cfg)) {
    L->gate_flag = replay_gate_flag(replay);
    const bool ok = L->gate_flag && cudaStreamCreateWithFlags(&L->ing, cudaStreamNonBlocking) == cudaSuccess &&
                    cudaEventCreateWithFlags(&L->ev_ing, cudaEventDisableTiming) == cudaSuccess;
    if (!ok) {
      set_error("d4pg_learner_create: ingest stream setup failed"); delete L; return D4PG_ECUDA;
    }
  }
  {
    const size_t nb = size_t(cfg->batch);
    bool ok = cudaEventCreateWithFlags(&L->ev_in, cudaEventDisableTiming) == cudaSuccess &&
              cudaEventCreateWithFlags(&L->ev_out, cudaEventDisableTiming) == cudaSuccess &&
              cudaHostAlloc(reinterpret_cast<void**>(&L->host_losses), 4 * sizeof(float), cudaHostAllocDefault) == cudaSuccess;
    for (int i = 0; i < 2 && ok; ++i)
      ok = cudaEventCreateWithFlags(&L->ev_loss[i], cudaEventDisableTiming) == cudaSuccess &&
           cudaHostAlloc(reinterpret_cast<void**>(&L->loss_ring[i]), 4 * sizeof(float), cudaHostAllocDefault) == cudaSuccess;
    for (int i = 0; i < 4 && ok; ++i)
      ok = cudaEventCreateWithFlags(&L->ev_h2d[i], cudaEventDisableTiming) == cudaSuccess &&
           cudaHostAlloc(reinterpret_cast<void**>(&L->host_u[i]), nb * sizeof(double), cudaHostAllocMapped) == cudaSuccess &&
           cudaHostAlloc(reinterpret_cast<void**>(&L->host_pos[i]), nb * sizeof(int32_t), cudaHostAllocMapped) == cudaSuccess;
    if (!ok) { set_error("d4pg_learner_create: pinned staging allocation failed"); delete L; return D4PG_ECUDA; }
  }
  if (cudaStreamCreateWithFlags(&L->side, cudaStreamNonBlocking) != cudaSuccess ||
      cudaEventCreateWithFlags(&L->ev_fork, cudaEventDisableTiming) != cudaSuccess ||
      cudaEventCreateWithFlags(&L->ev_join, cudaEventDisableTiming) != cudaSuccess ||
      cudaEventCreateWithFlags(&L->ev_fork2, cudaEventDisableTiming) != cudaSuccess ||
      cudaEventCreateWithFlags(&L->ev_join2, cudaEventDisableTiming) != cudaSuccess) {
    set_error("d4pg_learner_create: stream/event creation failed"); delete L; return D4PG_ECUDA;
  }
  trace_set_side_stream(L->side);
  cudaError_t e = cudaMemset(L->ws.clock, 0, sizeof(LearnerClock));
  if (e == cudaSuccess) e = cudaMemset(L->ws.pipe_epoch, 0, sizeof(unsigned long long) * size_t(cdiv(cfg->batch, SAMPLE_ROWS)));
  if (e != cudaSuccess) { set_error("d4pg_learner_create: %s", cudaGetErrorString(e)); delete L; return D4PG_ECUDA; }
  *out = L;
  return D4PG_OK;
}

extern "C" int32_t d4pg_learner_destroy(d4pg_learner_t* L) {
  if (!L) return D4PG_OK;
  for (int i = 0; i < 4; ++i) if (L->graph_exec[i]) cudaGraphExecDestroy(L->graph_exec[i]);
  for (int i = 0; i < 2; ++i) if (L->multi_exec[i]) cudaGraphExecDestroy(L->multi_exec[i]);
  cudaEventDestroy(L->ev_fork); cudaEventDestroy(L->ev_join); cudaEventDestroy(L->ev_fork2); cudaEventDestroy(L->ev_join2);
  cudaStreamDestroy(L->side);
  if (L->tcc_images) cudaFree(L->tcc_images);
  if (L->gtab) cudaFree(L->gtab);
  if (L->ing) { cudaStreamSynchronize(L->ing); cudaStreamDestroy(L->ing); }
  if (L->ev_ing) cudaEventDestroy(L->ev_ing);
  if (L->ev_in) cudaEventDestroy(L->ev_in);
  if (L->ev_out) cudaEventDestroy(L->ev_out);
  if (L->host_losses) cudaFreeHost(L->host_losses);
  for (int i = 0; i < 2; ++i) {
    if (L->ev_loss[i]) cudaEventDestroy(L->ev_loss[i]);
    if (L->loss_ring[i]) cudaFreeHost(L->loss_ring[i]);
  }
  for (int i = 0; i < 4; ++i) {
    if (L->ev_h2d[i]) cudaEventDestroy(L->ev_h2d[i]);
    if (L->host_u[i]) cudaFreeHost(L->host_u[i]);
    if (L->host_pos[i]) cudaFreeHost(L->host_pos[i]);
  }
  delete L;
  return D4PG_OK;
}

static void next_variant(d4pg_learner* L, int* par, bool* cold) {
  if (!piped(L->cfg)) { *par = 0; *cold = true; return; }
  *par = L->pipe_par;
  *cold = host_pipe(L->cfg) || !L->prefetch_valid || replay_generation(L->replay) != L->seen_gen;
}
static void commit_variant(d4pg_learner* L, int par) {
  ++L->steps_done;
  if (!piped(L->cfg)) return;
  L->last_par = par; L->pipe_par = par ^ 1; L->prefetch_valid = true; L->seen_gen = replay_generation(L->replay);
}

static int wait_for_ingest(d4pg_learner* L, cudaStream_t st) {
  if (!L->ing) return D4PG_OK;
  D4PG_CUDA_OK(cudaEventRecord(L->ev_ing, L->ing));
  D4PG_CUDA_OK(cudaStreamWaitEvent(st, L->ev_ing, 0));
  return D4PG_OK;
}

template <class F>
static int capture_graph(cudaStream_t st, cudaGraphExec_t* exec, const char* what, F body) {
  D4PG_REQUIRE(st != nullptr, D4PG_EINVAL, "%s: graph capture needs a non-default stream", what);
  cudaGraph_t graph = nullptr;
  D4PG_CUDA_OK(cudaStreamBeginCapture(st, cudaStreamCaptureModeThreadLocal));
  const int rc = body();
  cudaError_t e = cudaStreamEndCapture(st, &graph);
  if (rc != D4PG_OK) { if (graph) cudaGraphDestroy(graph); return rc; }
  if (e != cudaSuccess) { set_error("%s: end capture: %s", what, cudaGetErrorString(e)); return D4PG_ECUDA; }
  e = cudaGraphInstantiate(exec, graph, 0);
  cudaGraphDestroy(graph);
  if (e != cudaSuccess) { set_error("%s: instantiate: %s", what, cudaGetErrorString(e)); return D4PG_ECUDA; }
  return D4PG_OK;
}

static int step_eager(d4pg_learner* L, cudaStream_t st, int par, bool cold) {
  const int rc = enqueue_step(L, st, par, cold, !(host_pipe(L->cfg) && !cold));
  if (rc == D4PG_OK) { commit_variant(L, par); if (L->ing) replay_arm_gate(L->replay); }
  return rc;
}

static int launch_variant(d4pg_learner* L, cudaStream_t st, int par, bool cold) {
  if (!L->cfg.use_graph) return step_eager(L, st, par, cold);
  const int v = piped(L->cfg) ? par * 2 + (cold ? 1 : 0) : int(L->steps_done & 1);
  if (!L->graph_ready[v]) {
    const int rc = capture_graph(st, &L->graph_exec[v], "d4pg_learner_step",
                                 [&] { return enqueue_step(L, st, par, cold, !(host_pipe(L->cfg) && !cold)); });
    if (rc) return rc;
    L->graph_ready[v] = true;
  }
  D4PG_CUDA_OK(cudaGraphLaunch(L->graph_exec[v], st));
  commit_variant(L, par);
  if (L->ing) replay_arm_gate(L->replay);
  return D4PG_OK;
}

extern "C" int32_t d4pg_learner_step(d4pg_learner_t* L, d4pg_stream_t stream) {
  D4PG_REQUIRE(L, D4PG_EINVAL, "d4pg_learner_step: null handle");
  cudaStream_t st = as_stream(stream);
  int par; bool cold;
  next_variant(L, &par, &cold);
  if (int rc = wait_for_ingest(L, st)) return rc;
  return launch_variant(L, st, par, cold);
}

static int presample(d4pg_learner* L, int par, const double* uniforms, const int32_t* positions, cudaStream_t st) {
  const d4pg_learner_config_t& c = L->cfg; const Workspace& w = L->ws; const Batch& o = w.batch[par];
  return learner_sample(L->replay, c.batch, c.prioritized, uniforms, !c.prioritized ? positions : nullptr, c.philox_seed,
                        w.clock, L->clock_params, o.idx, o.wts, o.s, o.a, o.r, o.s2, o.done, o.hz, pitch4(c.obs_dim),
                        pitch4(c.act_dim), L->norm_affine, L->norm_clip, par, st, true, w.pipe_epoch);
}

static int step_host_common(d4pg_learner_t* L, const double* uniforms, const uint32_t* mt_words, const int32_t* positions,
                            d4pg_stream_t caller_stream, d4pg_stream_t learner_stream) {
  cudaStream_t cs = as_stream(caller_stream), ls = as_stream(learner_stream);
  const int B = L->cfg.batch;
  D4PG_CUDA_OK(cudaEventRecord(L->ev_in, cs));
  D4PG_CUDA_OK(cudaStreamWaitEvent(ls, L->ev_in, 0));
  const bool pipe = L->ing != nullptr && (uniforms || mt_words || positions);
  const int par = int(L->host_steps & (pipe ? 3 : 1));
  double* du = L->buf.uniforms;
  int32_t* dpos = L->buf.positions;
  if (uniforms || mt_words || positions) {
    if (L->host_steps >= (pipe ? 4 : 2)) D4PG_CUDA_OK(cudaEventSynchronize(L->ev_h2d[par]));
    if (uniforms || mt_words) {
      D4PG_REQUIRE(du, D4PG_ESTATE, "d4pg_learner_step_host: no device uniforms buffer");
      double* u = L->host_u[par];
      if (uniforms) memcpy(u, uniforms, size_t(B) * sizeof(double));
      else
        for (int i = 0; i < B; ++i)
          u[i] = (double(mt_words[2 * i] >> 5) * 67108864.0 + double(mt_words[2 * i + 1] >> 6)) * (1.0 / 9007199254740992.0);
      if (pipe) D4PG_CUDA_OK(cudaHostGetDevicePointer(reinterpret_cast<void**>(&du), u, 0));
      else D4PG_CUDA_OK(cudaMemcpyAsync(du, u, size_t(B) * sizeof(double), cudaMemcpyHostToDevice, ls));
    }
    if (positions) {
      D4PG_REQUIRE(dpos, D4PG_ESTATE, "d4pg_learner_step_host: no device positions buffer");
      memcpy(L->host_pos[par], positions, size_t(B) * sizeof(int32_t));
      if (pipe) D4PG_CUDA_OK(cudaHostGetDevicePointer(reinterpret_cast<void**>(&dpos), L->host_pos[par], 0));
      else D4PG_CUDA_OK(cudaMemcpyAsync(dpos, L->host_pos[par], size_t(B) * sizeof(int32_t), cudaMemcpyHostToDevice, ls));
    }
    if (!pipe) D4PG_CUDA_OK(cudaEventRecord(L->ev_h2d[par], ls));
    ++L->host_steps;
  }
  int rc;
  if (pipe) {
    const int bpar = L->pipe_par;
    rc = replay_gate_consume(L->replay, L->ing);
    if (rc) return rc;
    rc = presample(L, bpar, du, dpos, L->ing);
    if (rc) return rc;
    D4PG_CUDA_OK(cudaEventRecord(L->ev_h2d[par], L->ing));
    D4PG_CUDA_OK(cudaEventRecord(L->ev_ing, L->ing));
    if (L->images_dirty && L->plan == PLAN_TC_CHAIN) {
      rc = launch_tcc_pack(L->tcc_pack_fwd, ls);
      if (rc) return rc;
    }
    L->images_dirty = false;
    if (L->plan != PLAN_TC_CHAIN) D4PG_CUDA_OK(cudaStreamWaitEvent(ls, L->ev_ing, 0));
    rc = launch_variant(L, ls, bpar, false);
  } else {
    rc = d4pg_learner_step(L, learner_stream);
  }
  if (rc) return rc;
  {
    const int slot = int(L->loss_steps & 1);
    D4PG_CUDA_OK(cudaMemcpyAsync(L->loss_ring[slot], L->buf.losses, 4 * sizeof(float), cudaMemcpyDeviceToHost, ls));
    D4PG_CUDA_OK(cudaEventRecord(L->ev_loss[slot], ls));
    ++L->loss_steps;
  }
  D4PG_CUDA_OK(cudaEventRecord(L->ev_out, ls));
  D4PG_CUDA_OK(cudaStreamWaitEvent(cs, L->ev_out, 0));
  return D4PG_OK;
}

extern "C" int32_t d4pg_learner_fetch_losses(d4pg_learner_t* L, int32_t lag, float* out4) {
  D4PG_REQUIRE(L && out4 && (lag == 0 || lag == 1), D4PG_EINVAL, "d4pg_learner_fetch_losses: lag must be 0 or 1");
  D4PG_REQUIRE(L->loss_steps > lag, D4PG_ESTATE, "d4pg_learner_fetch_losses: no such step yet");
  const int slot = int((L->loss_steps - 1 - lag) & 1);
  D4PG_CUDA_OK(cudaEventSynchronize(L->ev_loss[slot]));
  for (int i = 0; i < 4; ++i) out4[i] = L->loss_ring[slot][i];
  return D4PG_OK;
}

extern "C" int32_t d4pg_learner_step_host(d4pg_learner_t* L, const double* uniforms, const int32_t* positions,
                                          d4pg_stream_t caller_stream, d4pg_stream_t learner_stream) {
  D4PG_REQUIRE(L, D4PG_EINVAL, "d4pg_learner_step_host: null handle");
  return step_host_common(L, uniforms, nullptr, positions, caller_stream, learner_stream);
}

extern "C" int32_t d4pg_learner_step_host_mt(d4pg_learner_t* L, const uint32_t* mt_words,
                                             d4pg_stream_t caller_stream, d4pg_stream_t learner_stream) {
  D4PG_REQUIRE(L && mt_words, D4PG_EINVAL, "d4pg_learner_step_host_mt: null argument");
  return step_host_common(L, nullptr, mt_words, nullptr, caller_stream, learner_stream);
}

extern "C" int32_t d4pg_learner_read_losses(d4pg_learner_t* L, float* out4, d4pg_stream_t learner_stream) {
  D4PG_REQUIRE(L && out4, D4PG_EINVAL, "d4pg_learner_read_losses: null argument");
  cudaStream_t ls = as_stream(learner_stream);
  D4PG_CUDA_OK(cudaMemcpyAsync(L->host_losses, L->buf.losses, 4 * sizeof(float), cudaMemcpyDeviceToHost, ls));
  D4PG_CUDA_OK(cudaStreamSynchronize(ls));
  for (int i = 0; i < 4; ++i) out4[i] = L->host_losses[i];
  return D4PG_OK;
}

constexpr int RUN_UNROLL = 8;
extern "C" int32_t d4pg_learner_run(d4pg_learner_t* L, int32_t n_steps, d4pg_stream_t stream) {
  D4PG_REQUIRE(L && n_steps > 0, D4PG_EINVAL, "d4pg_learner_run: bad arguments");
  cudaStream_t st = as_stream(stream);
  int n = n_steps;
  while (n > 0) {
    int par; bool cold;
    next_variant(L, &par, &cold);
    if (L->cfg.use_graph && prefetching(L->cfg) && !cold && n >= RUN_UNROLL && st != nullptr) {
      if (!L->multi_ready[par]) {
        const int rc = capture_graph(st, &L->multi_exec[par], "d4pg_learner_run", [&] {
          int rc = D4PG_OK;
          for (int i = 0; i < RUN_UNROLL && rc == D4PG_OK; ++i) rc = enqueue_step(L, st, par ^ (i & 1), false, i == 0);
          return rc;
        });
        if (rc) return rc;
        L->multi_ready[par] = true;
      }
      D4PG_CUDA_OK(cudaGraphLaunch(L->multi_exec[par], st));
      for (int i = 0; i < RUN_UNROLL; ++i) commit_variant(L, par ^ (i & 1));
      n -= RUN_UNROLL;
      continue;
    }
    int rc = d4pg_learner_step(L, stream);
    if (rc) return rc;
    --n;
  }
  return D4PG_OK;
}

extern "C" int32_t d4pg_learner_profile_step(d4pg_learner_t* L, d4pg_stream_t stream, int32_t max_launches,
                                             float* ms_out, char* names_out, int32_t name_stride, int32_t* n_out) {
  D4PG_REQUIRE(L && ms_out && n_out && max_launches > 0, D4PG_EINVAL, "d4pg_learner_profile_step: bad arguments");
  cudaStream_t st = as_stream(stream);
  int par; bool cold;
  next_variant(L, &par, &cold);
  if (int rc = wait_for_ingest(L, st)) return rc;
  L->profiling = true; L->ev.clear(); L->ev_name.clear(); L->ev_reps.clear();
  const int rc = step_eager(L, st, par, cold);
  L->profiling = false;
  cudaError_t e = cudaStreamSynchronize(st);
  const int n = int(L->ev_name.size());
  *n_out = n < max_launches ? n : max_launches;
  for (int i = 0; i < n; ++i) {
    float ms = 0.f;
    if (e == cudaSuccess) cudaEventElapsedTime(&ms, L->ev[2 * i], L->ev[2 * i + 1]);
    ms /= float(L->ev_reps[i]);
    if (i < max_launches) {
      ms_out[i] = ms;
      if (names_out && name_stride > 1) {
        strncpy(names_out + size_t(i) * name_stride, L->ev_name[i].c_str(), name_stride - 1);
        names_out[size_t(i) * name_stride + name_stride - 1] = 0;
      }
    }
    cudaEventDestroy(L->ev[2 * i]); cudaEventDestroy(L->ev[2 * i + 1]);
  }
  L->ev.clear(); L->ev_name.clear(); L->ev_reps.clear();
  if (e != cudaSuccess) { set_error("d4pg_learner_profile_step: %s", cudaGetErrorString(e)); return D4PG_ECUDA; }
  return rc;
}

extern "C" int32_t d4pg_learner_weights_changed(d4pg_learner_t* L) {
  D4PG_REQUIRE(L, D4PG_EINVAL, "d4pg_learner_weights_changed: null handle");
  L->images_dirty = true;
  return D4PG_OK;
}
extern "C" void* d4pg_learner_ingest_stream(const d4pg_learner_t* L) { return L ? static_cast<void*>(L->ing) : nullptr; }
extern "C" int64_t d4pg_learner_steps_done(const d4pg_learner_t* L) { return L ? L->steps_done : -1; }
extern "C" int32_t d4pg_learner_kernels_per_step(const d4pg_learner_t* L) { return L ? L->kernels_per_step : -1; }

extern "C" int32_t d4pg_learner_set_counters(d4pg_learner_t* L, int64_t adam_step, int64_t beta_t, d4pg_stream_t stream) {
  D4PG_REQUIRE(L && adam_step >= 0 && beta_t >= 0, D4PG_EINVAL, "d4pg_learner_set_counters: bad arguments");
  LearnerClock c{};
  c.adam_step = adam_step; c.beta_t = beta_t; c.steps_done = adam_step;
  c.s_adam_step = adam_step; c.s_beta_t = beta_t; c.s_steps_done = adam_step;
  L->prefetch_valid = false;
  D4PG_CUDA_OK(cudaMemsetAsync(L->ws.pipe_epoch, 0, sizeof(unsigned long long) * size_t(cdiv(L->cfg.batch, SAMPLE_ROWS)), as_stream(stream)));
  D4PG_CUDA_OK(cudaMemcpyAsync(L->ws.clock, &c, sizeof(c), cudaMemcpyHostToDevice, as_stream(stream)));
  D4PG_CUDA_OK(cudaStreamSynchronize(as_stream(stream)));
  return D4PG_OK;
}

extern "C" int32_t d4pg_learner_tensor(d4pg_learner_t* L, const char* name, void** ptr, int64_t* count, int32_t* ld) {
  D4PG_REQUIRE(L && name && ptr && count && ld, D4PG_EINVAL, "d4pg_learner_tensor: null argument");
  const Workspace& w = L->ws; const Batch& bt = w.batch[L->last_par];
  const int64_t B = L->cfg.batch;
  const int Sp = pitch4(L->cfg.obs_dim), Ap = pitch4(L->cfg.act_dim), Np = pitch4(L->cfg.n_atoms);
  struct E { const char* n; void* p; int64_t c; int ld; };
  const E table[] = {
      {"s", bt.s, B * Sp, Sp}, {"a", bt.a, B * Ap, Ap}, {"r", bt.r, B, 1}, {"s2", bt.s2, B * Sp, Sp}, {"done", bt.done, B, 1},
      {"h", bt.hz, bt.hz ? B : 0, 1},
      {"target_logits", w.out[1], B * Np, Np}, {"q_logits", w.out[2], B * Np, Np}, {"pi_logits", w.out[4], B * Np, Np},
      {"m", w.m, B * Np, Np}, {"q_probs", w.q_probs, B * Np, Np}, {"target_probs", w.target_probs, B * Np, Np},
      {"dlogits_q", w.dlogits_q, B * Np, Np}, {"dlogits_pi", w.dlogits_pi, B * Np, Np},
      {"actor_out", w.out[3], B * Ap, Ap}, {"actor_target_out", w.out[0], B * Ap, Ap},
      {"loss_rows", w.loss_rows, B, 1}, {"pi_rows", w.pi_rows, B, 1},
      {"h1_c", w.h1[2], B * 256, 256}, {"h2_c", w.h2[2], B * 256, 256}, {"h3_c", w.h3[2], B * 256, 256},
      {"h1_a", w.h1[3], B * 256, 256}, {"h2_a", w.h2[3], B * 256, 256}, {"h3_a", w.h3[3], B * 256, 256},
      {"h2_p", w.h2[4], B * 256, 256}, {"h3_p", w.h3[4], B * 256, 256},
      {"h1_at", w.h1[0], B * 256, 256}, {"h2_at", w.h2[0], B * 256, 256}, {"h3_at", w.h3[0], B * 256, 256},
      {"h1_ct", w.h1[1], B * 256, 256}, {"h2_ct", w.h2[1], B * 256, 256}, {"h3_ct", w.h3[1], B * 256, 256},
      {"p_dz22", w.p_dz22, B * 256, 256}, {"p_dz2", w.p_dz2, B * 256, 256},
      {"c_dz22", w.c_dz22, B * 256, 256}, {"c_dz2", w.c_dz2, B * 256, 256}, {"c_dz1", w.c_dz1, B * 256, 256},
      {"a_dz3", w.a_dz3, B * Ap, Ap}, {"a_dz22", w.a_dz22, B * 256, 256}, {"a_dh2", w.a_dh2, B * 256, 256},
      {"a_dz1", w.a_dz1, B * 256, 256}};
  for (const E& e : table)
    if (e.p && strcmp(e.n, name) == 0) { *ptr = e.p; *count = e.c; *ld = e.ld; return D4PG_OK; }
  set_error("d4pg_learner_tensor: unknown tensor '%s'", name);
  return D4PG_EINVAL;
}
```

d4pg-pytorch_b200/csrc/mlp_chain.cu:

```cuda
#include "gemm_ffma_dev.cuh"
#include "mlp_chain_dev.cuh"
#include <stdlib.h>
#include <algorithm>

namespace d4pg {

__device__ __forceinline__ void tf32_split(float x, uint32_t& hi, uint32_t& lo) {
  asm("cvt.rna.tf32.f32 %0, %1;" : "=r"(hi) : "f"(x));
  const float r = x - __uint_as_float(hi);
  asm("cvt.rna.tf32.f32 %0, %1;" : "=r"(lo) : "f"(r));
}
__device__ __forceinline__ void mma_tf32(float (&c)[4], const uint32_t (&a)[4], const uint32_t (&b)[2]) {
  asm volatile("mma.sync.aligned.m16n8k8.row.col.f32.tf32.tf32.f32 {%0,%1,%2,%3}, {%4,%5,%6,%7}, {%8,%9}, {%0,%1,%2,%3};"
               : "+f"(c[0]), "+f"(c[1]), "+f"(c[2]), "+f"(c[3])
               : "r"(a[0]), "r"(a[1]), "r"(a[2]), "r"(a[3]), "r"(b[0]), "r"(b[1]));
}
constexpr int CHAIN_RED_PITCH = 36;

template <int MODE, int PREC>
__device__ __forceinline__ void chain_tile_mma(const ChainSlot& S, float* As, const float* Ws, int m0, int n0, int B, float* xout,
                                               const float (&eop)[4], unsigned long long* tr) {
  const int tid = threadIdx.x, warp = tid >> 5, lane = tid & 31;
  const int g = lane >> 2, t4 = lane & 3;
  const int N = S.N, K = S.K;
  const int P = chain_wpitch(K);
  float acc[2][4][4];
#pragma unroll
  for (int m = 0; m < 2; ++m)
#pragma unroll
    for (int nn = 0; nn < 4; ++nn)
#pragma unroll
      for (int i = 0; i < 4; ++i) acc[m][nn][i] = 0.f;
  const int nks = (K + 7) >> 3;
  for (int ks = warp; ks < nks; ks += GEMM_WARPS) {
    const int ka = ks * 8 + t4, kb = ka + 4;
    const bool va = ka < K, vb = kb < K;
    const int sw = t4 << 3;
    uint32_t ah[2][4], al[2][4], bh[4][2], bl[4][2];
#pragma unroll
    for (int m = 0; m < 2; ++m) {
      const int r0 = (m * 16 + g) ^ sw, r1 = (m * 16 + g + 8) ^ sw;
      const float x0 = va ? As[ka * CHAIN_ROWS + r0] : 0.f, x1 = va ? As[ka * CHAIN_ROWS + r1] : 0.f;
      const float x2 = vb ? As[kb * CHAIN_ROWS + r0] : 0.f, x3 = vb ? As[kb * CHAIN_ROWS + r1] : 0.f;
      tf32_split(x0, ah[m][0], al[m][0]); tf32_split(x1, ah[m][1], al[m][1]);
      tf32_split(x2, ah[m][2], al[m][2]); tf32_split(x3, ah[m][3], al[m][3]);
    }
#pragma unroll
    for (int nn = 0; nn < 4; ++nn) {
      float y0, y1;
      if (MODE == GEMM_FWD) { y0 = va ? Ws[(nn * 8 + g) * P + ka] : 0.f; y1 = vb ? Ws[(nn * 8 + g) * P + kb] : 0.f; }
      else { y0 = va ? Ws[ka * BN + ((nn * 8 + g) ^ sw)] : 0.f; y1 = vb ? Ws[kb * BN + ((nn * 8 + g) ^ sw)] : 0.f; }
      tf32_split(y0, bh[nn][0], bl[nn][0]); tf32_split(y1, bh[nn][1], bl[nn][1]);
    }
#pragma unroll
    for (int m = 0; m < 2; ++m)
#pragma unroll
      for (int nn = 0; nn < 4; ++nn) {
        if (PREC == 1) { mma_tf32(acc[m][nn], al[m], bh[nn]); mma_tf32(acc[m][nn], ah[m], bl[nn]); }
        mma_tf32(acc[m][nn], ah[m], bh[nn]);
      }
  }
  __syncthreads();
  if (tr) { unsigned long long t; asm volatile("mov.u64 %0, %%globaltimer;" : "=l"(t)); tr[3] = t; }
  float* red = As;
#pragma unroll
  for (int m = 0; m < 2; ++m)
#pragma unroll
    for (int nn = 0; nn < 4; ++nn) {
      float* q = red + (warp * BM + m * 16 + g) * CHAIN_RED_PITCH + nn * 8 + 2 * t4;
      *reinterpret_cast<float2*>(q) = make_float2(acc[m][nn][0], acc[m][nn][1]);
      *reinterpret_cast<float2*>(q + 8 * CHAIN_RED_PITCH) = make_float2(acc[m][nn][2], acc[m][nn][3]);
    }
  __syncthreads();
  const int orow = tid >> 3, ocol = (tid & 7) * 4;
  float4 sum = *reinterpret_cast<const float4*>(&red[orow * CHAIN_RED_PITCH + ocol]);
#pragma unroll
  for (int w = 1; w < GEMM_WARPS; ++w) {
    const float4 t = *reinterpret_cast<const float4*>(&red[(w * BM + orow) * CHAIN_RED_PITCH + ocol]);
    sum.x += t.x; sum.y += t.y; sum.z += t.z; sum.w += t.w;
  }
  const int gi = m0 + orow;
  const float v[4] = {sum.x, sum.y, sum.z, sum.w};
  const int epi = S.epi;
  float* __restrict__ C = S.C; const int ldc = S.ldc;
#pragma unroll
  for (int cc = 0; cc < 4; ++cc) {
    const int gj = n0 + ocol + cc;
    if (gj >= N) continue;
    float x = v[cc];
    if (gi < B) {
      const float e = eop[cc];
      switch (epi) {
        case EPI_BIAS: x += e; break;
        case EPI_BIAS_RELU: x = fmaxf(x + e, 0.f); break;
        case EPI_BIAS_TANH: x = tanhf(x + e); break;
        case EPI_RELU_MASK: x = (e > 0.f) ? x : 0.f; break;
        case EPI_TANH_MASK: x *= (1.f - e * e); break;
        default: break;
      }
      if (C) C[size_t(gi) * ldc + gj] = x;
    } else x = 0.f;
    if (xout) xout[gj * CHAIN_ROWS + orow] = x;
  }
}

template <int PREC>
__global__ void __cluster_dims__(CHAIN_CLUSTER, 1, 1) __launch_bounds__(GEMM_THREADS, 2)
mlp_chain_kernel(const __grid_constant__ ChainArgs args) {
  constexpr bool SWZ = PREC != 0;
  extern __shared__ __align__(16) float chain_smem[];
  float* As = chain_smem;
  float* W0 = chain_smem + args.a_floats;
  const int wf = args.w_floats;
  const int tid = threadIdx.x;
  const int rank = int(cluster_ctarank());
  const int cid = blockIdx.x / CHAIN_CLUSTER;
  const int chain = cid / args.row_blocks, rb_i = cid - chain * args.row_blocks;
  const int m0 = rb_i * CHAIN_ROWS, B = args.B;
  const int ns = args.nslots[chain];
  float* planes = args.xchg + (size_t(chain) * args.row_blocks + rb_i) * (size_t(CHAIN_MAX_SLOTS) * CHAIN_PLANE);
  const int n0 = rank * BN;

  if (n0 < args.slot[chain][0].N) fetch_weights<SWZ>(W0, args.slot[chain][0], n0, tid);
  cp_async_commit();
  unsigned long long* tr0 = (args.trace && int(blockIdx.x) == args.trace_cta && tid == 0) ? args.trace : nullptr;
  const long long clk0 = clock64();
  step_stamp(args.step_trace, args.step_slot);
  if (args.step_trace && args.step_slot == 1 && tid == 0 && blockIdx.x < 256) {
    unsigned smid;
    asm volatile("mov.u32 %0, %%smid;" : "=r"(smid));
    reinterpret_cast<unsigned char*>(args.step_trace + (128 - STEP_TRACE_BASE))[blockIdx.x] = (unsigned char)smid;
  }
  for (int l = 0; l < ns; ++l) {
    const ChainSlot& S = args.slot[chain][l];
    const bool has_tile = n0 < S.N;
    unsigned long long* tr = tr0 ? tr0 + 6 * l : nullptr;
    CTRACE(0);
    float eop[4] = {0.f, 0.f, 0.f, 0.f};
    if (has_tile && S.epi != EPI_NONE) {
      const int gi = m0 + (tid >> 3);
#pragma unroll
      for (int cc = 0; cc < 4; ++cc) {
        const int gj = n0 + ((S.mode == GEMM_FWD && PREC == 0) ? (tid & 7) + 8 * cc : (tid & 7) * 4 + cc);
        if (gj < S.N && gi < B) eop[cc] = (S.mode == GEMM_FWD) ? __ldg(S.bias + gj) : __ldg(S.aux + size_t(gi) * S.ldaux + gj);
      }
    }
    if (l > 0) cluster_wait();
    CTRACE(1);
    if (PREC == 0 && S.has_pre && has_tile) {
      float* Wp = W0 + ((l + 1) & 1) * wf;
      fetch_weights<SWZ>(Wp, S.pre_W, S.pre_ldw, S.pre_N, S.pre_K, S.mode, 0, tid);
      fill_from_plane<SWZ>(As, 0, planes + size_t(S.pre_src) * CHAIN_PLANE, S.pre_K, tid);
      cp_async_commit();
      float pe[4] = {0.f, 0.f, 0.f, 0.f};
      {
        const int gi = m0 + (tid >> 3);
#pragma unroll
        for (int cc = 0; cc < 4; ++cc) {
          const int gj = (S.mode == GEMM_FWD) ? (tid & 7) + 8 * cc : (tid & 7) * 4 + cc;
          if (gj < S.pre_N && gi < B)
            pe[cc] = (S.mode == GEMM_FWD) ? __ldg(S.pre_bias + gj) : __ldg(S.pre_aux + size_t(gi) * S.pre_ldaux + gj);
        }
      }
      cp_async_wait<0>();
      __syncthreads();
      const TileDesc D{S.pre_N, S.pre_K, S.pre_epi, rank == 0 ? S.pre_C : nullptr, S.pre_ldc};
      float* sout = As + S.pre_row * CHAIN_ROWS;
      if (S.mode == GEMM_FWD) chain_tile<GEMM_FWD>(D, As, As, Wp, m0, 0, B, nullptr, sout, pe, nullptr);
      else chain_tile<GEMM_DX>(D, As, As, Wp, m0, 0, B, nullptr, sout, pe, nullptr);
      __syncthreads();
    }
    if (has_tile) {
      const int K = S.K, K1 = S.K1;
      if (S.src >= 0) fill_from_plane<SWZ>(As, 0, planes + size_t(S.src) * CHAIN_PLANE, K1, tid);
      else if (S.src == -1) fill_from_rows<SWZ>(As, 0, S.Ag, S.ldag, m0, B, K1, tid);
      if (K > K1) {
        if (S.src2 >= 0) fill_from_plane<SWZ>(As, K1, planes + size_t(S.src2) * CHAIN_PLANE, K - K1, tid);
        else if (S.src2 == -1) fill_from_rows<SWZ>(As, K1, S.A2g, S.lda2g, m0, B, K - K1, tid);
      }
    }
    cp_async_commit();
    if (l + 1 < ns && n0 < args.slot[chain][l + 1].N) fetch_weights<SWZ>(W0 + ((l + 1) & 1) * wf, args.slot[chain][l + 1], n0, tid);
    cp_async_commit();
    cp_async_wait<1>();
    __syncthreads();
    CTRACE(2);
    if (has_tile) {
      float* xout = S.publish ? planes + size_t(l) * CHAIN_PLANE : nullptr;
      if (PREC == 0) {
        const TileDesc D = tile_of(S);
        const float* Am = As + S.a_row0 * CHAIN_ROWS;
        if (S.mode == GEMM_FWD) chain_tile<GEMM_FWD>(D, Am, As, W0 + (l & 1) * wf, m0, n0, B, xout, nullptr, eop, tr);
        else chain_tile<GEMM_DX>(D, Am, As, W0 + (l & 1) * wf, m0, n0, B, xout, nullptr, eop, tr);
      } else {
        if (S.mode == GEMM_FWD) chain_tile_mma<GEMM_FWD, PREC>(S, As, W0 + (l & 1) * wf, m0, n0, B, xout, eop, tr);
        else chain_tile_mma<GEMM_DX, PREC>(S, As, W0 + (l & 1) * wf, m0, n0, B, xout, eop, tr);
      }
    }
    CTRACE(4);
    if (l + 1 < ns) cluster_arrive();
    CTRACE(5);
  }
  cp_async_wait<0>();
  step_stamp(args.step_trace, args.step_slot + 16);
  if (tr0) tr0[6 * CHAIN_MAX_SLOTS - 1] = (unsigned long long)(clock64() - clk0);
}

static unsigned long long* chain_trace_buffer() { return debug_trace_buffer(); }

int64_t chain_xchg_floats(int B) {
  return int64_t(CHAIN_MAX) * cdiv(B, CHAIN_ROWS) * CHAIN_MAX_SLOTS * CHAIN_PLANE;
}
void chain_args_begin(ChainArgs& a, int B, float* xchg, int precision) {
  a = ChainArgs{};
  a.B = B; a.row_blocks = cdiv(B, CHAIN_ROWS); a.xchg = xchg; a.precision = precision;
  a.a_floats = precision ? GEMM_WARPS * BM * CHAIN_RED_PITCH : GEMM_WARPS * BM * BN;
  a.w_floats = 0;
}
int chain_add(ChainArgs& a, int c, const ChainSlot& s) {
  if (c >= a.nchains) a.nchains = c + 1;
  const int l = a.nslots[c]++;
  a.slot[c][l] = s;
  const int af = int(align4(int64_t(s.has_pre ? std::max(s.K, s.pre_row + 8) : s.K) * CHAIN_ROWS));
  const int wf = s.mode == GEMM_FWD ? BN * chain_wpitch(s.K) : int(align4(int64_t(s.K) * BN));
  if (af > a.a_floats) a.a_floats = af;
  if (wf > a.w_floats) a.w_floats = wf;
  return l;
}
size_t chain_smem_bytes(const ChainArgs& a) { return size_t(a.a_floats + 2 * a.w_floats) * sizeof(float); }
bool chain_fits(const ChainArgs& a) {
  for (int c = 0; c < a.nchains; ++c)
    for (int l = 0; l < a.nslots[c]; ++l)
      if (a.slot[c][l].N > CHAIN_CLUSTER * BN) return false;
  return chain_smem_bytes(a) <= CHAIN_SMEM_MAX;
}
ChainSlot chain_fwd(const float* W, int ldw, const float* bias, int N, int K, int epi, float* C, int ldc, int publish) {
  ChainSlot s{};
  s.W = W; s.ldw = ldw; s.bias = bias; s.N = N; s.K = K; s.K1 = K; s.epi = epi; s.C = C; s.ldc = ldc;
  s.mode = GEMM_FWD; s.publish = publish; s.src = -1; s.src2 = -1;
  return s;
}
ChainSlot chain_dx(const float* W, int ldw, int N_in, int K_out, int epi, const float* aux, int ldaux,
                   float* C, int ldc, int publish) {
  ChainSlot s{};
  s.W = W; s.ldw = ldw; s.N = N_in; s.K = K_out; s.K1 = K_out; s.epi = epi; s.aux = aux; s.ldaux = ldaux;
  s.C = C; s.ldc = ldc; s.mode = GEMM_DX; s.publish = publish; s.src = -1; s.src2 = -1;
  return s;
}
void chain_src_global(ChainSlot& s, const float* Ag, int ldag) { s.Ag = Ag; s.ldag = ldag; s.src = -1; }
void chain_src_plane(ChainSlot& s, int slot) { s.src = slot; }
void chain_src2_global(ChainSlot& s, int K1, const float* A2g, int lda2g) { s.K1 = K1; s.A2g = A2g; s.lda2g = lda2g; s.src2 = -1; }
void chain_src2_plane(ChainSlot& s, int K1, int slot) { s.K1 = K1; s.src2 = slot; }
void chain_pre_layer(ChainSlot& s, const float* W, int ldw, const float* bias, const float* aux, int ldaux, int N, int K, int epi,
                     float* C, int ldc, int src_slot, int pre_row, bool whole_operand) {
  s.has_pre = 1; s.pre_W = W; s.pre_ldw = ldw; s.pre_bias = bias; s.pre_aux = aux; s.pre_ldaux = ldaux;
  s.pre_N = N; s.pre_K = K; s.pre_epi = epi; s.pre_C = C; s.pre_ldc = ldc; s.pre_src = src_slot; s.pre_row = pre_row;
  if (whole_operand) { s.src = -2; s.K1 = s.K; s.a_row0 = pre_row; }
  else { s.src2 = -2; s.K1 = s.K - N; s.a_row0 = 0; }
}

int launch_mlp_chain(ChainArgs& a, cudaStream_t st) {
  D4PG_REQUIRE(a.nchains > 0 && a.nchains <= CHAIN_MAX, D4PG_EINVAL, "launch_mlp_chain: %d chains", a.nchains);
  for (int c = 0; c < a.nchains; ++c) {
    D4PG_REQUIRE(a.nslots[c] > 0 && a.nslots[c] <= CHAIN_MAX_SLOTS, D4PG_EINVAL, "launch_mlp_chain: chain %d has %d slots", c, a.nslots[c]);
    for (int l = 0; l < a.nslots[c]; ++l) {
      const ChainSlot& s = a.slot[c][l];
      D4PG_REQUIRE(s.N > 0, D4PG_EINVAL, "launch_mlp_chain: slot %d has no columns", l);
      D4PG_REQUIRE(s.ldw % 4 == 0 && (reinterpret_cast<uintptr_t>(s.W) & 15) == 0, D4PG_EINVAL, "launch_mlp_chain: weights must be 16-B pitched");
      D4PG_REQUIRE(s.src < l && s.src2 < l, D4PG_EINVAL, "launch_mlp_chain: slot %d reads a later plane", l);
      D4PG_REQUIRE(s.src >= 0 || s.src == -2 || (s.Ag && s.ldag % 4 == 0 && s.ldag >= s.K1), D4PG_EINVAL, "launch_mlp_chain: bad global A source");
      D4PG_REQUIRE(s.K == s.K1 || s.src2 >= 0 || s.src2 == -2 || (s.A2g && s.lda2g % 4 == 0 && s.lda2g >= s.K - s.K1), D4PG_EINVAL, "launch_mlp_chain: bad second A source");
      D4PG_REQUIRE((s.src != -2 && s.src2 != -2) || s.has_pre, D4PG_EINVAL, "launch_mlp_chain: slot %d expects a pre-layer", l);
      if (s.has_pre) {
        D4PG_REQUIRE(a.precision == 0, D4PG_ENOTSUP, "launch_mlp_chain: pre-layers exist for the fp32 tile only");
        D4PG_REQUIRE(s.pre_N > 0 && s.pre_N <= 8 && s.pre_K <= D4PG_HIDDEN && s.pre_row >= D4PG_HIDDEN && s.pre_src >= 0 && s.pre_src < l &&
                     a.slot[c][s.pre_src].publish && a.slot[c][s.pre_src].N >= s.pre_K && s.pre_ldw % 4 == 0 &&
                     (reinterpret_cast<uintptr_t>(s.pre_W) & 15) == 0, D4PG_EINVAL, "launch_mlp_chain: bad pre-layer in slot %d", l);
      }
      D4PG_REQUIRE(s.src < 0 || (a.slot[c][s.src].publish && a.slot[c][s.src].N >= s.K1), D4PG_EINVAL, "launch_mlp_chain: slot %d reads an unpublished plane", l);
      D4PG_REQUIRE(s.K == s.K1 || s.src2 < 0 || (a.slot[c][s.src2].publish && a.slot[c][s.src2].N >= s.K - s.K1), D4PG_EINVAL, "launch_mlp_chain: slot %d reads an unpublished plane", l);
    }
  }
  const size_t smem = chain_smem_bytes(a);
  D4PG_REQUIRE(chain_fits(a), D4PG_ENOTSUP, "launch_mlp_chain: %zu B of shared memory needed (at most %zu) or a layer wider than %d",
               smem, CHAIN_SMEM_MAX, CHAIN_CLUSTER * BN);
  D4PG_REQUIRE(a.precision >= 0 && a.precision <= 2, D4PG_EINVAL, "launch_mlp_chain: precision %d", a.precision);
  static size_t smem_set[3] = {0, 0, 0};
  void (*kern)(ChainArgs) = a.precision == 0 ? mlp_chain_kernel<0> : a.precision == 1 ? mlp_chain_kernel<1> : mlp_chain_kernel<2>;
  if (smem > smem_set[a.precision]) {
    D4PG_CUDA_OK(cudaFuncSetAttribute(kern, cudaFuncAttributeMaxDynamicSharedMemorySize, int(smem)));
    D4PG_CUDA_OK(cudaFuncSetAttribute(kern, cudaFuncAttributePreferredSharedMemoryCarveout, int(cudaSharedmemCarveoutMaxShared)));
    smem_set[a.precision] = smem;
  }
  a.trace = chain_trace_buffer() ? chain_trace_buffer() + a.trace_base : nullptr;
  a.step_trace = chain_trace_buffer() ? chain_trace_buffer() + STEP_TRACE_BASE : nullptr;
  a.step_slot = a.trace_base ? 5 : 1;
  { const char* e = getenv("D4PG_TRACE_CTA"); a.trace_cta = e ? atoi(e) : 0; if (a.trace_cta >= a.nchains * a.row_blocks * CHAIN_CLUSTER) a.trace_cta = 0; }
  cudaLaunchConfig_t cfg{};
  cfg.gridDim = dim3(a.nchains * a.row_blocks * CHAIN_CLUSTER); cfg.blockDim = dim3(GEMM_THREADS);
  cfg.dynamicSmemBytes = smem; cfg.stream = st;
  cfg.attrs = nullptr; cfg.numAttrs = 0;
  D4PG_CUDA_OK(cudaLaunchKernelEx(&cfg, kern, a));
  return D4PG_OK;
}

}
```

d4pg-pytorch_b200/csrc/mlp_chain.cuh:

```cuda
#pragma once
#include "gemm_ffma.cuh"
#include "adam.cuh"

namespace d4pg {

constexpr int CHAIN_MAX_SLOTS = 8;
constexpr int CHAIN_MAX = 3;
constexpr int CHAIN_CLUSTER = 8;
constexpr int CHAIN_ROWS = 32;
constexpr int CHAIN_PLANE = D4PG_HIDDEN * CHAIN_ROWS;

struct ChainSlot {
  const float* W; const float* bias; const float* aux;
  const float* Ag; const float* A2g;
  float* C;
  int ldw, ldaux, ldag, lda2g, ldc;
  int N, K, K1;
  int src, src2;
  int mode, epi;
  int publish;
  int has_pre, pre_src, pre_row, a_row0;
  const float* pre_W; const float* pre_bias; const float* pre_aux; float* pre_C;
  int pre_ldw, pre_ldaux, pre_ldc, pre_N, pre_K, pre_epi;
};

struct ChainArgs {
  ChainSlot slot[CHAIN_MAX][CHAIN_MAX_SLOTS];
  int nslots[CHAIN_MAX];
  int nchains, B, row_blocks;
  int precision;
  int a_floats, w_floats;
  float* xchg;
  unsigned long long* trace;
  int trace_base;
  unsigned long long* step_trace; int step_slot;
  int trace_cta;
};

int64_t chain_xchg_floats(int B);
void chain_args_begin(ChainArgs& a, int B, float* xchg, int precision = 0);
int chain_add(ChainArgs& a, int c, const ChainSlot& s);
ChainSlot chain_fwd(const float* W, int ldw, const float* bias, int N, int K, int epi, float* C, int ldc, int publish);
ChainSlot chain_dx(const float* W, int ldw, int N_in, int K_out, int epi, const float* aux, int ldaux,
                   float* C, int ldc, int publish);
void chain_src_global(ChainSlot& s, const float* Ag, int ldag);
void chain_src_plane(ChainSlot& s, int slot);
void chain_src2_global(ChainSlot& s, int K1, const float* A2g, int lda2g);
void chain_src2_plane(ChainSlot& s, int K1, int slot);
void chain_pre_layer(ChainSlot& s, const float* W, int ldw, const float* bias, const float* aux, int ldaux, int N, int K, int epi,
                     float* C, int ldc, int src_slot, int pre_row, bool whole_operand);
constexpr size_t CHAIN_SMEM_MAX = 220 * 1024;
size_t chain_smem_bytes(const ChainArgs& a);
bool chain_fits(const ChainArgs& a);
int launch_mlp_chain(ChainArgs& a, cudaStream_t st);

constexpr int GEMM_WIDE_MAX = 12;
struct GemmWideBatch {
  GemmProblem p[GEMM_WIDE_MAX];
  int n, total_tiles, pdl;
  unsigned long long* trace;
  PeerSignal peer_sig; int has_peer_sig;
};
void gemm_wide_begin(GemmWideBatch& b, const PeerSignal* sig = nullptr);
void gemm_wide_add(GemmWideBatch& b, const GemmProblem& p);
int gemm_wide_launch(GemmWideBatch& b, cudaStream_t st);

}
```

d4pg-pytorch_b200/csrc/mlp_tc_chain.cu:

```cuda
#include "mlp_tc_chain.cuh"
#include "tc_common.cuh"
#include <stdlib.h>
#include <string.h>

namespace d4pg {

using namespace tc;

constexpr uint32_t TCC_OFF_A = 0;
constexpr uint32_t TCC_OFF_W = TCC_ABUFS * TCC_A_CHUNK;
constexpr uint32_t TCC_OFF_BAR = TCC_OFF_W + TCC_MAX_CHUNKS * TCC_W_CHUNK;
constexpr uint32_t TCC_SMEM = TCC_OFF_BAR + 256 + 1024;
static_assert(TCC_SMEM <= 227 * 1024, "the chain kernel's shared memory exceeds what a Hopper CTA may use");
constexpr int TCC_CONSUMERS = 256;
constexpr int TCC_TRACE_PER_SLOT = 12;

__device__ __forceinline__ void tcc_cluster_arrive() { asm volatile("barrier.cluster.arrive.release.aligned;" ::: "memory"); }
__device__ __forceinline__ void tcc_cluster_wait() { asm volatile("barrier.cluster.wait.acquire.aligned;" ::: "memory"); }
__device__ __forceinline__ unsigned tcc_ctarank() {
  unsigned r;
  asm volatile("mov.u32 %0, %%cluster_ctarank;" : "=r"(r));
  return r;
}
__device__ __forceinline__ unsigned long long tcc_gtime() {
  unsigned long long t;
  asm volatile("mov.u64 %0, %%globaltimer;" : "=l"(t));
  return t;
}
__device__ __forceinline__ void tcc_bulk_load(void* smem_dst, const void* gsrc, uint32_t bytes, uint64_t* bar) {
  asm volatile("cp.async.bulk.shared::cluster.global.mbarrier::complete_tx::bytes [%0], [%1], %2, [%3];"
               ::"r"(smem_u32(smem_dst)), "l"(gsrc), "r"(bytes), "r"(smem_u32(bar)) : "memory");
}
__device__ __forceinline__ void tcc_wait(uint64_t* bar, uint32_t parity, unsigned long long* dbg, unsigned code, unsigned aux) {
  if (mbar_try_wait(bar, parity)) return;
  const long long t0 = clock64();
  bool recorded = false;
  while (!mbar_try_wait(bar, parity)) {
    const long long dt = clock64() - t0;
    if (dt > 4000000000ll && !recorded) {
      recorded = true;
      if (dbg) {
        if (atomicCAS(dbg, 0ull, 1ull) == 0ull) {
          dbg[1] = (unsigned long long)code | ((unsigned long long)parity << 24) | ((unsigned long long)blockIdx.x << 32);
          dbg[2] = aux;
        }
        const unsigned kind = code & 0xFFu;
        if (kind < 6 && atomicCAS(dbg + 4 + 2 * kind, 0ull, 1ull) == 0ull) {
          dbg[4 + 2 * kind] = (unsigned long long)code | ((unsigned long long)parity << 24) | ((unsigned long long)blockIdx.x << 32);
          dbg[5 + 2 * kind] = aux;
        }
        __threadfence_system();
      }
    }
    if (dt > 5000000000ll) __trap();
  }
}
#define TCC_CODE(kind, slot, rank) (unsigned(kind) | (unsigned(slot) << 8) | (unsigned(rank) << 16))
enum { WD_LOADER_DFULL = 2, WD_MMA_WFULL = 3, WD_MMA_FULL = 4 };

__device__ __forceinline__ float4 tcc_hi4(float4 v) { return make_float4(tf32_hi(v.x), tf32_hi(v.y), tf32_hi(v.z), tf32_hi(v.w)); }
__device__ __forceinline__ float4 tcc_lo4(float4 v, float4 h) {
  return make_float4(tf32_lo(v.x, h.x), tf32_lo(v.y, h.y), tf32_lo(v.z, h.z), tf32_lo(v.w, h.w));
}

__device__ __forceinline__ void tcc_convert_chunk(uint8_t* dst, const float* __restrict__ src, int ld, int k0, int ncols,
                                                  int m0, int B, int et) {
#pragma unroll
  for (int p = 0; p < 2; ++p) {
    const int e = et + p * 256, row = e >> 3, u = e & 7, k = k0 + (u << 2);
    float4 v = make_float4(0.f, 0.f, 0.f, 0.f);
    if (m0 + row < B && k < ncols) {
      v = __ldg(reinterpret_cast<const float4*>(src + size_t(m0 + row) * ld + k));
      if (k + 1 >= ncols) v.y = 0.f;
      if (k + 2 >= ncols) v.z = 0.f;
      if (k + 3 >= ncols) v.w = 0.f;
    }
    const float4 h = tcc_hi4(v);
    const uint32_t off = sw128_kmajor_off(row, u << 2);
    *reinterpret_cast<float4*>(dst + off) = h;
    *reinterpret_cast<float4*>(dst + TCC_A_HALF + off) = tcc_lo4(v, h);
  }
}

__device__ __forceinline__ bool tcc_group_active(const TccSlot& S, int g, int n0) { return g < S.ngroups && n0 < S.g[g].N; }
__device__ __forceinline__ bool tcc_slot_active(const TccSlot& S, int n0) { return tcc_group_active(S, 0, n0) || tcc_group_active(S, 1, n0); }

__device__ __forceinline__ void tcc_issue_weights(const TccSlot& S, int rank, int n0, uint8_t* Wb, uint64_t* wfull) {
  const uint32_t gbytes = uint32_t(S.nchunks) * TCC_W_CHUNK;
  uint32_t bytes = 0;
#pragma unroll
  for (int g = 0; g < TCC_MAX_GROUPS; ++g)
    if (tcc_group_active(S, g, n0)) bytes += gbytes;
  mbar_expect_tx(wfull, bytes);
#pragma unroll
  for (int g = 0; g < TCC_MAX_GROUPS; ++g)
    if (tcc_group_active(S, g, n0)) tcc_bulk_load(Wb + g * gbytes, S.g[g].wimg + size_t(rank) * gbytes, gbytes, wfull);
}

template <int PASSES>
__global__ void __cluster_dims__(TCC_CLUSTER, 1, 1) __launch_bounds__(TCC_THREADS, 1)
mlp_tc_chain_kernel(const __grid_constant__ TccArgs args) {
  static_assert(PASSES == 1 || PASSES == 3, "the chain kernel runs one TF32 pass or 3xTF32");
  extern __shared__ uint8_t tcc_smem_raw[];
  uint8_t* smem = reinterpret_cast<uint8_t*>((reinterpret_cast<uintptr_t>(tcc_smem_raw) + 1023) & ~uintptr_t(1023));
  uint8_t* Ab = smem + TCC_OFF_A;
  uint8_t* Xb = Ab + 8 * TCC_A_CHUNK;
  uint8_t* Wb = smem + TCC_OFF_W;
  uint64_t* bars = reinterpret_cast<uint64_t*>(smem + TCC_OFF_BAR);
  uint64_t* full = bars;
  uint64_t* wfull = bars + TCC_ABUFS;
  uint64_t* dfull = wfull + 1;

  const int tid = threadIdx.x, warp = tid >> 5, lane = tid & 31;
  const int rank = int(tcc_ctarank());
  const int cid = blockIdx.x / TCC_CLUSTER;
  const int chain = cid / args.row_blocks, rb = cid - chain * args.row_blocks;
  const int m0 = rb * TCC_ROWS, B = args.B;
  const TccChain& CH = args.chain[chain];
  const int ns = CH.nslots;
  const int n0 = rank * TCC_BN;
  uint8_t* planes = args.xchg + (size_t(chain) * args.row_blocks + rb) * (size_t(TCC_PLANES) * TCC_PLANE_BYTES);
  const int npre = CH.pre ? (CH.precols + TCC_KC - 1) / TCC_KC : 0;
  unsigned long long* tr0 = (args.trace && int(blockIdx.x) == args.trace_cta) ? args.trace : nullptr;
  if (args.wait_epoch) {
    if (tid < args.wait_n) {
      const unsigned long long target = (unsigned long long)(*reinterpret_cast<const volatile long long*>(args.wait_clock) + 1);
      unsigned long long v;
      do { asm volatile("ld.acquire.gpu.global.u64 %0, [%1];" : "=l"(v) : "l"(args.wait_epoch + tid) : "memory"); } while (v < target);
    }
    __syncthreads();
  }
  step_stamp(args.step_trace, args.step_slot);

  if (tid == TCC_CONSUMERS) {
    for (int i = 0; i < TCC_ABUFS + 2; ++i) mbar_init(&bars[i], 1);
    mbar_fence_init();
  }
  if (tid < TCC_CONSUMERS) {
    if (CH.x0) tcc_convert_chunk(Xb, CH.x0, CH.x0ld, 0, CH.x0cols, m0, B, tid);
    for (int p = 0; p < npre; ++p) tcc_convert_chunk(Ab + p * TCC_A_CHUNK, CH.pre, CH.preld, p * TCC_KC, CH.precols, m0, B, tid);
    fence_proxy_async();
  }
  __syncthreads();

  if (tid == TCC_CONSUMERS)
    for (int p = 0; p < npre; ++p) mbar_arrive(&full[p]);
  uint32_t fph = 0;
  int nact = 0;
  if (tid == TCC_CONSUMERS && tcc_slot_active(CH.slot[0], n0)) tcc_issue_weights(CH.slot[0], rank, n0, Wb, wfull);

  for (int l = 0; l < ns; ++l) {
    const TccSlot& S = CH.slot[l];
    const bool active = tcc_slot_active(S, n0);
    unsigned long long* tr = tr0 ? tr0 + TCC_TRACE_PER_SLOT * l : nullptr;
    bool arrived = false;

    if (tid >= TCC_CONSUMERS) {
      if (lane == 0) {
        if (tr) tr[0] = tcc_gtime();
        if (active && S.nloads > 0) {
          asm volatile("fence.proxy.async.global;" ::: "memory");
          for (int i = 0; i < S.nloads; ++i) {
            const TccLoad L = S.ld[i];
            const uint32_t bytes = uint32_t(L.count) * TCC_A_CHUNK;
            mbar_expect_tx(&full[L.buf0], bytes);
            tcc_bulk_load(Ab + L.buf0 * TCC_A_CHUNK, planes + size_t(L.plane) * TCC_PLANE_BYTES + size_t(L.chunk0) * TCC_A_CHUNK,
                          bytes, &full[L.buf0]);
          }
        }
        if (tr) tr[1] = tcc_gtime();
        if (l + 1 < ns && tcc_slot_active(CH.slot[l + 1], n0)) {
          if (active) tcc_wait(dfull, nact & 1, args.watchdog, TCC_CODE(WD_LOADER_DFULL, l, rank), nact);
          tcc_issue_weights(CH.slot[l + 1], rank, n0, Wb, wfull);
        }
      }
      __syncwarp();
    } else {
      const int g = warp >> 2, wq = warp & 3;
      const bool mine = tcc_group_active(S, g, n0);
      const int rl = 16 * wq + (lane >> 2);
      const int cl = 2 * (lane & 3);
      if (active) {
        const TccGroup& G = S.g[g];
        constexpr int N1 = PASSES == 3 ? 32 : 16;
        float d1[N1], d2[PASSES == 3 ? 16 : 1];
#pragma unroll
        for (int i = 0; i < N1; ++i) d1[i] = 0.f;
        if constexpr (PASSES == 3) {
#pragma unroll
          for (int i = 0; i < 16; ++i) d2[i] = 0.f;
        }
        float eop[2][8];
        const int npad = mine ? (G.N + 3) & ~3 : 0;
        const bool fwd = G.epi == EPI_BIAS || G.epi == EPI_BIAS_RELU || G.epi == EPI_BIAS_TANH;
        const bool msk = G.epi == EPI_RELU_MASK || G.epi == EPI_TANH_MASK;
#pragma unroll
        for (int rr = 0; rr < 2; ++rr) {
          const int gi = m0 + rl + 8 * rr;
#pragma unroll
          for (int j = 0; j < 4; ++j) {
            const int gj = n0 + 8 * j + cl;
            float2 v = make_float2(0.f, 0.f);
            if (gj < npad) {
              if (fwd) v = __ldg(reinterpret_cast<const float2*>(G.bias + gj));
              else if (msk && gi < B) v = __ldg(reinterpret_cast<const float2*>(G.aux + size_t(gi) * G.ldaux + gj));
            }
            eop[rr][2 * j] = v.x; eop[rr][2 * j + 1] = v.y;
          }
        }
        const int nch = S.nchunks, boff = S.boff;
        const uint32_t wait_mask = S.wait_mask;
        if (mine) {
          tcc_wait(wfull, nact & 1, args.watchdog, TCC_CODE(WD_MMA_WFULL, l, rank), nact);
          if (tr && tid == 0) tr[2] = tcc_gtime();
          const uint32_t w_base = smem_u32(Wb) + uint32_t(g * nch) * TCC_W_CHUNK;
          const uint32_t a_base = smem_u32(Ab) + uint32_t(boff) * TCC_A_CHUNK;
          wg_fence_regs(d1);
          if constexpr (PASSES == 3) wg_fence_regs(d2);
          for (int c = 0; c < nch; ++c) {
            if ((wait_mask >> c) & 1u) {
              const int b = c + boff;
              tcc_wait(&full[b], (fph >> b) & 1u, args.watchdog, TCC_CODE(WD_MMA_FULL, l, rank), b);
              if (tr && tid == 0 && c == 0) tr[3] = tcc_gtime();
            }
            const uint32_t a_hi = a_base + uint32_t(c) * TCC_A_CHUNK, a_lo = a_hi + TCC_A_HALF;
            const uint32_t w = w_base + uint32_t(c) * TCC_W_CHUNK;
            wg_fence();
#pragma unroll
            for (int ks = 0; ks < 4; ++ks) {
              const uint64_t bd = wg_desc(w + 32 * ks);
              if constexpr (PASSES == 3) {
                wg_mma_n64(d1, wg_desc(a_hi + 32 * ks), bd);
                wg_mma_n32(d2, wg_desc(a_lo + 32 * ks), bd);
              } else {
                wg_mma_n32(d1, wg_desc(a_hi + 32 * ks), bd);
              }
            }
            wg_commit();
          }
          wg_wait<0>();
          wg_fence_regs(d1);
          if constexpr (PASSES == 3) wg_fence_regs(d2);
          if (tr && tid == 0) tr[4] = tcc_gtime();
        }
        for (int c = 0; c < nch; ++c)
          if ((wait_mask >> c) & 1u) fph ^= 1u << (c + boff);
        asm volatile("bar.sync 1, %0;" ::"n"(TCC_CONSUMERS) : "memory");
        if (tid == 0) mbar_arrive(dfull);
        if (tr && tid == 0) tr[5] = tcc_gtime();
        if (S.xsrc) {
          tcc_convert_chunk(Xb, S.xsrc, S.xld, 0, S.xcols, m0, B, tid);
          fence_proxy_async();
        }
        if (mine) {
          const int epi = G.epi;
          float x[16];
          if constexpr (PASSES == 3) {
#pragma unroll
            for (int i = 0; i < 16; ++i) x[i] = (d1[i + 16] + d2[i]) + d1[i];
          } else {
#pragma unroll
            for (int i = 0; i < 16; ++i) x[i] = d1[i];
          }
#pragma unroll
          for (int i = 0; i < 16; ++i) {
            const float e = eop[(i >> 1) & 1][2 * (i >> 2) + (i & 1)];
            if (epi == EPI_BIAS || epi == EPI_BIAS_RELU || epi == EPI_BIAS_TANH) x[i] += e;
            else if (epi == EPI_RELU_MASK) x[i] = (e > 0.f) ? x[i] : 0.f;
            else if (epi == EPI_TANH_MASK) x[i] *= (1.f - e * e);
          }
          if (epi == EPI_BIAS_RELU) {
#pragma unroll
            for (int i = 0; i < 16; ++i) x[i] = fmaxf(x[i], 0.f);
          } else if (epi == EPI_BIAS_TANH) {
#pragma unroll
            for (int i = 0; i < 16; ++i)
              if (n0 + 8 * (i >> 2) + cl + (i & 1) < G.N) x[i] = tanhf(x[i]);
          }
#pragma unroll
          for (int i = 0; i < 16; ++i) {
            const int gi = m0 + rl + 8 * ((i >> 1) & 1), gj = n0 + 8 * (i >> 2) + cl + (i & 1);
            x[i] = (gi < B && gj < G.N) ? x[i] : 0.f;
          }
          if (tr && tid == 0) tr[6] = tcc_gtime();
          if (G.pub >= 0) {
            uint8_t* stg = Ab + (2 + g) * TCC_A_CHUNK;
#pragma unroll
            for (int i = 0; i < 16; i += 2) {
              const int r = rl + 8 * ((i >> 1) & 1), k = 8 * (i >> 2) + cl;
              const float2 v = make_float2(x[i], x[i + 1]);
              const float2 h = make_float2(tf32_hi(v.x), tf32_hi(v.y));
              const uint32_t off = sw128_kmajor_off(r, k);
              *reinterpret_cast<float2*>(stg + off) = h;
              *reinterpret_cast<float2*>(stg + TCC_A_HALF + off) = make_float2(tf32_lo(v.x, h.x), tf32_lo(v.y, h.y));
            }
            fence_proxy_async();
            asm volatile("bar.sync %0, 128;" ::"r"(2 + g) : "memory");
            if ((tid & 127) == 0) {
              uint8_t* img = planes + size_t(G.pub) * TCC_PLANE_BYTES + size_t(rank) * TCC_A_CHUNK;
              asm volatile("cp.async.bulk.global.shared::cta.bulk_group [%0], [%1], %2;"
                           ::"l"(img), "r"(smem_u32(stg)), "r"(TCC_A_CHUNK) : "memory");
              asm volatile("cp.async.bulk.commit_group;" ::: "memory");
              asm volatile("cp.async.bulk.wait_group 0;" ::: "memory");
            }
          }
          if (tr && tid == 0) tr[8] = tcc_gtime();
          if (l + 1 < ns) { tcc_cluster_arrive(); arrived = true; }
          if (G.C) {
#pragma unroll
            for (int i = 0; i < 16; i += 2) {
              const int gi = m0 + rl + 8 * ((i >> 1) & 1), gj = n0 + 8 * (i >> 2) + cl;
              if (gi < B && gj < npad) *reinterpret_cast<float2*>(G.C + size_t(gi) * G.ldc + gj) = make_float2(x[i], x[i + 1]);
            }
          }
        }
      } else if (S.xsrc) {
        tcc_convert_chunk(Xb, S.xsrc, S.xld, 0, S.xcols, m0, B, tid);
        fence_proxy_async();
      }
      if (tr && tid == 0) tr[9] = tcc_gtime();
    }
    if (active) ++nact;
    if (l + 1 < ns) {
      if (!arrived) tcc_cluster_arrive();
      tcc_cluster_wait();
      if (tr && tid == 0) tr[10] = tcc_gtime();
    }
  }
  step_stamp(args.step_trace, args.step_slot + 16);
}

__global__ void __launch_bounds__(256) tcc_pack_kernel(const __grid_constant__ TccPackArgs args) {
  int ui = 0;
#pragma unroll 1
  for (int i = 1; i < args.n; ++i)
    if (int(blockIdx.x) >= args.use[i].block_begin) ui = i;
  const TccPackUse& U = args.use[ui];
  const int blk = blockIdx.x - U.block_begin;
  const int slice = blk / U.nchunks, chunk = blk - slice * U.nchunks;
  uint8_t* dst = args.dst + U.dst_off + size_t(blk) * TCC_W_CHUNK;
  const int tid = threadIdx.x;
  float4 v = make_float4(0.f, 0.f, 0.f, 0.f);
  int j, u;
  if (U.mode == GEMM_FWD) {
    j = tid >> 3; u = tid & 7;
    const int n = slice * TCC_BN + j, k = chunk * TCC_KC + 4 * u;
    if (n < U.N && k < U.K) {
      v = __ldg(reinterpret_cast<const float4*>(U.W + size_t(n) * U.ldw + k));
      if (k + 1 >= U.K) v.y = 0.f;
      if (k + 2 >= U.K) v.z = 0.f;
      if (k + 3 >= U.K) v.w = 0.f;
    }
  } else {
    j = tid & 31; u = tid >> 5;
    const int n = slice * TCC_BN + j, k = chunk * TCC_KC + 4 * u;
    if (n < U.N) {
      if (k < U.K) v.x = __ldg(U.W + size_t(k) * U.ldw + n);
      if (k + 1 < U.K) v.y = __ldg(U.W + size_t(k + 1) * U.ldw + n);
      if (k + 2 < U.K) v.z = __ldg(U.W + size_t(k + 2) * U.ldw + n);
      if (k + 3 < U.K) v.w = __ldg(U.W + size_t(k + 3) * U.ldw + n);
    }
  }
  const float4 h = tcc_hi4(v);
  const uint32_t off = sw128_kmajor_off(j, 4 * u);
  *reinterpret_cast<float4*>(dst + off) = h;
  *reinterpret_cast<float4*>(dst + TCC_W_HALF + off) = tcc_lo4(v, h);
}

static unsigned long long* g_tcc_watchdog_host = nullptr;
unsigned long long* tcc_watchdog_device() {
  static bool tried = false;
  static unsigned long long* dev = nullptr;
  if (!tried) {
    tried = true;
    unsigned long long* host = nullptr;
    if (cudaHostAlloc(reinterpret_cast<void**>(&host), 128, cudaHostAllocMapped) == cudaSuccess) {
      memset(host, 0, 128);
      if (cudaHostGetDevicePointer(reinterpret_cast<void**>(&dev), host, 0) != cudaSuccess) dev = nullptr;
      g_tcc_watchdog_host = host;
    }
    (void)cudaGetLastError();
  }
  return dev;
}
}
extern "C" int32_t d4pg_debug_watchdog(unsigned long long* out16) {
  if (!out16) return D4PG_EINVAL;
  for (int i = 0; i < 16; ++i) out16[i] = d4pg::g_tcc_watchdog_host ? d4pg::g_tcc_watchdog_host[i] : 0ull;
  return D4PG_OK;
}
namespace d4pg {

void tcc_pack_begin(TccPackArgs& p, uint8_t* dst) { p.n = 0; p.total_blocks = 0; p.dst = dst; }
int tcc_pack_add(TccPackArgs& p, const float* W, int ldw, int mode, int N, int K) {
  if (p.n >= TCC_MAX_USES) return -1;
  TccPackUse& u = p.use[p.n];
  u.W = W; u.ldw = ldw; u.mode = mode; u.N = N; u.K = K;
  u.nslices = cdiv(N, TCC_BN); u.nchunks = cdiv(K, TCC_KC);
  u.block_begin = p.total_blocks;
  u.dst_off = (long long)(p.total_blocks) * TCC_W_CHUNK;
  p.total_blocks += u.nslices * u.nchunks;
  return p.n++;
}
long long tcc_pack_bytes(const TccPackArgs& p) { return (long long)(p.total_blocks) * TCC_W_CHUNK; }
void tcc_pack_set_base(TccPackArgs& p, uint8_t* dst, long long first_byte) { p.dst = dst + first_byte; }
int launch_tcc_pack(const TccPackArgs& p, cudaStream_t st) {
  D4PG_REQUIRE(p.n > 0 && p.dst, D4PG_EINVAL, "launch_tcc_pack: nothing to pack");
  tcc_pack_kernel<<<p.total_blocks, 256, 0, st>>>(p);
  D4PG_LAUNCH_OK();
  return D4PG_OK;
}

int64_t tcc_xchg_floats(int B) {
  return int64_t(TCC_MAX_CHAINS) * cdiv(B, TCC_ROWS) * TCC_PLANES * (TCC_PLANE_BYTES / 4);
}
void tcc_args_begin(TccArgs& a, int B, uint8_t* xchg, int passes) {
  memset(&a, 0, sizeof(a));
  a.B = B; a.row_blocks = cdiv(B, TCC_ROWS); a.xchg = xchg; a.passes = passes;
}
void tcc_chain_x0(TccArgs& a, int c, const float* src, int ld, int cols) {
  a.chain[c].x0 = src; a.chain[c].x0ld = ld; a.chain[c].x0cols = cols;
}
void tcc_chain_pre(TccArgs& a, int c, const float* src, int ld, int cols) {
  a.chain[c].pre = src; a.chain[c].preld = ld; a.chain[c].precols = cols;
}
int tcc_slot_begin(TccArgs& a, int c) {
  if (c >= a.nchains) a.nchains = c + 1;
  TccChain& ch = a.chain[c];
  const int l = ch.nslots++;
  if (l < TCC_MAX_SLOTS) { ch.slot[l] = TccSlot{}; ch.slot[l].g[0].pub = ch.slot[l].g[1].pub = -1; }
  return l;
}
static void tcc_push_chunk(TccSlot& s, int kind, int plane, int chunk) {
  if (s.nchunks < TCC_MAX_CHUNKS) s.ch[s.nchunks] = TccChunk{short(kind), short(plane), short(chunk), 0};
  ++s.nchunks;
}
void tcc_slot_src_x(TccArgs& a, int c, int slot) { tcc_push_chunk(a.chain[c].slot[slot], TCC_SRC_X, 0, 0); }
void tcc_slot_src_pre(TccArgs& a, int c, int slot) {
  const int n = cdiv(a.chain[c].precols, TCC_KC);
  for (int i = 0; i < n; ++i) tcc_push_chunk(a.chain[c].slot[slot], TCC_SRC_PRE, 0, i);
}
void tcc_slot_src_plane(TccArgs& a, int c, int slot, int plane, int nchunks) {
  for (int i = 0; i < nchunks; ++i) tcc_push_chunk(a.chain[c].slot[slot], TCC_SRC_IMG, plane, i);
}
void tcc_slot_reconvert_x(TccArgs& a, int c, int slot, const float* src, int ld, int cols) {
  TccSlot& s = a.chain[c].slot[slot];
  s.xsrc = src; s.xld = ld; s.xcols = cols;
}
int tcc_slot_group(TccArgs& a, int c, int slot, const TccImage& img, int epi, const float* bias,
                   const float* aux, int ldaux, float* C, int ldc, int publish) {
  TccChain& ch = a.chain[c];
  TccSlot& s = ch.slot[slot];
  const int gi = s.ngroups++;
  if (gi >= TCC_MAX_GROUPS) return -1;
  TccGroup& g = s.g[gi];
  g.wimg = img.ptr; g.bias = bias; g.aux = aux; g.ldaux = ldaux; g.C = C; g.ldc = ldc;
  g.N = img.N; g.epi = epi; g.kchunks = img.kchunks;
  g.pub = publish ? ch.nplanes++ : -1;
  return g.pub;
}

int launch_mlp_tc_chain(TccArgs& a, cudaStream_t st) {
  D4PG_REQUIRE(a.nchains > 0 && a.nchains <= TCC_MAX_CHAINS, D4PG_EINVAL, "launch_mlp_tc_chain: %d chains", a.nchains);
  D4PG_REQUIRE(a.passes == 1 || a.passes == 3, D4PG_EINVAL, "launch_mlp_tc_chain: passes %d", a.passes);
  constexpr int gmax = 2;
  for (int c = 0; c < a.nchains; ++c) {
    TccChain& ch = a.chain[c];
    bool x_clobbered = false;
    D4PG_REQUIRE(ch.nslots > 0 && ch.nslots <= TCC_MAX_SLOTS, D4PG_EINVAL, "launch_mlp_tc_chain: chain %d has %d slots", c, ch.nslots);
    D4PG_REQUIRE(ch.nplanes <= TCC_PLANES, D4PG_ENOTSUP, "launch_mlp_tc_chain: chain %d publishes %d planes", c, ch.nplanes);
    D4PG_REQUIRE(!ch.x0 || (ch.x0cols <= TCC_KC && ch.x0ld % 4 == 0 && ch.x0ld >= ch.x0cols), D4PG_ENOTSUP, "launch_mlp_tc_chain: bad X source");
    D4PG_REQUIRE(!ch.pre || (ch.precols <= 8 * TCC_KC && ch.preld % 4 == 0 && ch.preld >= ch.precols), D4PG_ENOTSUP,
                 "launch_mlp_tc_chain: bad first-slot source");
    int planes_seen = 0;
    for (int l = 0; l < ch.nslots; ++l) {
      TccSlot& s = ch.slot[l];
      D4PG_REQUIRE(s.ngroups >= 1 && s.ngroups <= TCC_MAX_GROUPS, D4PG_EINVAL, "launch_mlp_tc_chain: slot %d has %d groups", l, s.ngroups);
      D4PG_REQUIRE(s.nchunks >= 1 && s.nchunks <= TCC_MAX_CHUNKS && s.ngroups * s.nchunks <= TCC_MAX_CHUNKS, D4PG_ENOTSUP,
                   "launch_mlp_tc_chain: slot %d: %d groups x %d chunks exceed the weight buffer", l, s.ngroups, s.nchunks);
      int nring = 0;
      bool uses_x = false;
      for (int i = 0; i < s.nchunks; ++i) uses_x = uses_x || s.ch[i].kind == TCC_SRC_X;
      s.nloads = 0;
      for (int i = 0; i < s.nchunks; ++i) {
        TccChunk& k = s.ch[i];
        if (k.kind == TCC_SRC_IMG) D4PG_REQUIRE(k.plane >= 0 && k.plane < planes_seen && k.chunk < TCC_CLUSTER, D4PG_EINVAL,
                                                 "launch_mlp_tc_chain: slot %d reads plane %d before it is published", l, k.plane);
        if (k.kind == TCC_SRC_PRE) D4PG_REQUIRE(l == 0 && ch.pre && k.chunk == nring && nring < 8, D4PG_EINVAL, "launch_mlp_tc_chain: pre chunks belong to slot 0, in order");
        if (k.kind == TCC_SRC_X) {
          D4PG_REQUIRE(ch.x0 != nullptr && !x_clobbered, D4PG_EINVAL, "launch_mlp_tc_chain: slot %d reads X but the chain has none (or it was overwritten)", l);
          k.buf = 8;
          continue;
        }
        if (nring < 8) k.buf = short(nring);
        else {
          D4PG_REQUIRE(nring == 8 && !uses_x && k.kind == TCC_SRC_IMG, D4PG_ENOTSUP, "launch_mlp_tc_chain: slot %d needs more than 9 A buffers", l);
          k.buf = 8; x_clobbered = true;
        }
        ++nring;
        if (k.kind == TCC_SRC_IMG) {
          TccLoad* cur = s.nloads ? &s.ld[s.nloads - 1] : nullptr;
          if (cur && cur->plane == k.plane && cur->chunk0 + cur->count == k.chunk && cur->buf0 + cur->count == k.buf && cur->count < gmax) ++cur->count;
          else s.ld[s.nloads++] = TccLoad{k.plane, k.chunk, k.buf, 1};
        }
      }
      s.boff = s.ch[0].buf;
      s.wait_mask = 0;
      for (int i = 0; i < s.nchunks; ++i) {
        D4PG_REQUIRE(s.ch[i].buf == s.boff + i, D4PG_ENOTSUP, "launch_mlp_tc_chain: slot %d: chunk %d is not in A buffer %d", l, i, s.boff + i);
        if (s.ch[i].kind == TCC_SRC_PRE) s.wait_mask |= 1u << i;
      }
      for (int i = 0; i < s.nloads; ++i) s.wait_mask |= 1u << (s.ld[i].buf0 - s.boff);
      for (int g = 0; g < s.ngroups; ++g) {
        const TccGroup& G = s.g[g];
        D4PG_REQUIRE(G.N > 0 && G.N <= TCC_CLUSTER * TCC_BN && G.wimg, D4PG_ENOTSUP, "launch_mlp_tc_chain: group width %d", G.N);
        D4PG_REQUIRE(G.kchunks == s.nchunks, D4PG_EINVAL, "launch_mlp_tc_chain: chain %d slot %d: A operand has %d chunks, the weight image %d", c, l, s.nchunks, G.kchunks);
        D4PG_REQUIRE(!G.C || (G.ldc % 4 == 0 && G.ldc >= ((G.N + 3) & ~3) && (reinterpret_cast<uintptr_t>(G.C) & 15) == 0), D4PG_EINVAL,
                     "launch_mlp_tc_chain: output pitch");
        const bool fwd = G.epi == EPI_BIAS || G.epi == EPI_BIAS_RELU || G.epi == EPI_BIAS_TANH;
        const bool msk = G.epi == EPI_RELU_MASK || G.epi == EPI_TANH_MASK;
        D4PG_REQUIRE(!fwd || (G.bias && (reinterpret_cast<uintptr_t>(G.bias) & 15) == 0), D4PG_EINVAL, "launch_mlp_tc_chain: bias");
        D4PG_REQUIRE(!msk || (G.aux && G.ldaux % 4 == 0 && (reinterpret_cast<uintptr_t>(G.aux) & 15) == 0), D4PG_EINVAL, "launch_mlp_tc_chain: mask operand");
        if (G.pub >= 0) ++planes_seen;
      }
      if (l == 0 && ch.pre) D4PG_REQUIRE(s.g[0].N > (TCC_CLUSTER - 1) * TCC_BN, D4PG_ENOTSUP, "launch_mlp_tc_chain: the first slot must span the cluster");
    }
  }
  void (*kern)(TccArgs) = a.passes == 3 ? mlp_tc_chain_kernel<3> : mlp_tc_chain_kernel<1>;
  static bool attr_set[2] = {false, false};
  const int ai = a.passes == 3 ? 1 : 0;
  if (!attr_set[ai]) {
    D4PG_CUDA_OK(cudaFuncSetAttribute(kern, cudaFuncAttributeMaxDynamicSharedMemorySize, int(TCC_SMEM)));
    D4PG_CUDA_OK(cudaFuncSetAttribute(kern, cudaFuncAttributePreferredSharedMemoryCarveout, int(cudaSharedmemCarveoutMaxShared)));
    attr_set[ai] = true;
  }
  a.watchdog = tcc_watchdog_device();
  unsigned long long* dbg = debug_trace_buffer();
  a.trace = dbg ? dbg + (a.step_slot == 5 ? 384 : 256) : nullptr;
  a.step_trace = dbg ? dbg + STEP_TRACE_BASE : nullptr;
  { const char* e = getenv("D4PG_TRACE_CTA"); a.trace_cta = e ? atoi(e) : 0; if (a.trace_cta >= a.nchains * a.row_blocks * TCC_CLUSTER) a.trace_cta = 0; }
  cudaLaunchConfig_t cfg{};
  cfg.gridDim = dim3(a.nchains * a.row_blocks * TCC_CLUSTER); cfg.blockDim = dim3(TCC_THREADS);
  cfg.dynamicSmemBytes = TCC_SMEM; cfg.stream = st;
  cfg.attrs = nullptr; cfg.numAttrs = 0;
  D4PG_CUDA_OK(cudaLaunchKernelEx(&cfg, kern, a));
  return D4PG_OK;
}

}
```

Measured before the change: 6622.

## Split critic and policy backward/update onto concurrent streams in graph runs

Measured after the change: 4953, median of 6. 25.2% lower.

```diff
diff --git a/d4pg-pytorch_b200/csrc/adam.cu b/d4pg-pytorch_b200/csrc/adam.cu
--- a/d4pg-pytorch_b200/csrc/adam.cu
+++ b/d4pg-pytorch_b200/csrc/adam.cu
@@ -13,9 +13,9 @@
     if (blockIdx.x == 0) adam_tail(a, red);
     return;
   }
-  step_stamp(a.trace, 7);
+  step_stamp(a.trace, a.trace_slot);
   adam_segment<false>(a, blockIdx.y, blockIdx.x, gridDim.x);
-  step_stamp(a.trace, 7 + 16);
+  step_stamp(a.trace, a.trace_slot + 16);
   pdl_trigger_end(a.pdl);
 }
 
@@ -28,9 +28,9 @@
     if (blockIdx.x == 0) adam_tail(a, red);
     return;
   }
-  step_stamp(a.trace, 7);
+  step_stamp(a.trace, a.trace_slot);
   adam_segment<true>(a, blockIdx.y, blockIdx.x, gridDim.x, &bcast);
-  step_stamp(a.trace, 7 + 16);
+  step_stamp(a.trace, a.trace_slot + 16);
   pdl_trigger_end(a.pdl);
 }
 
diff --git a/d4pg-pytorch_b200/csrc/adam.cuh b/d4pg-pytorch_b200/csrc/adam.cuh
--- a/d4pg-pytorch_b200/csrc/adam.cuh
+++ b/d4pg-pytorch_b200/csrc/adam.cuh
@@ -103,6 +103,7 @@
   const float* loss_rows; const float* pi_rows; int B; float inv_count; float* loss_out;
   int pdl;
   int skip_tail;
+  int trace_slot;
 };
 int launch_adam(const AdamArgs& a, cudaStream_t st);
 
diff --git a/d4pg-pytorch_b200/csrc/common.cuh b/d4pg-pytorch_b200/csrc/common.cuh
--- a/d4pg-pytorch_b200/csrc/common.cuh
+++ b/d4pg-pytorch_b200/csrc/common.cuh
@@ -70,6 +70,8 @@
 }
 unsigned long long* debug_trace_buffer();
 constexpr int STEP_TRACE_BASE = 96;
+constexpr int STEP_SLOT_DX = 5, STEP_SLOT_DW = 6, STEP_SLOT_ADAM = 7;
+constexpr int STEP_SLOT_CRITIC_DX = 13, STEP_SLOT_CRITIC_DW = 14, STEP_SLOT_CRITIC_ADAM = 15;
 
 static inline cudaStream_t as_stream(d4pg_stream_t s) { return reinterpret_cast<cudaStream_t>(s); }
 
diff --git a/d4pg-pytorch_b200/csrc/gemm_ffma.cu b/d4pg-pytorch_b200/csrc/gemm_ffma.cu
--- a/d4pg-pytorch_b200/csrc/gemm_ffma.cu
+++ b/d4pg-pytorch_b200/csrc/gemm_ffma.cu
@@ -30,7 +30,7 @@
     if (i < batch.n && int(blockIdx.x) >= batch.p[i].tile_begin) pi = i;
   const GemmProblem& P = batch.p[pi];
   const int tile = blockIdx.x - P.tile_begin;
-  step_stamp(batch.trace, 6);
+  step_stamp(batch.trace, batch.trace_slot);
   if (ALLOW_SPLIT && P.ksplit > 1) {
     const int per_slice = P.tiles_m * P.tiles_n;
     const int ks = tile / per_slice, t2 = tile - ks * per_slice;
@@ -41,7 +41,7 @@
     const int tm = tile / P.tiles_n, tn = tile - tm * P.tiles_n;
     gemm_dw_tile_async<false>(P, smem, tm * BM, tn * BN, tn, 0, P.K);
   }
-  step_stamp(batch.trace, 6 + 16);
+  step_stamp(batch.trace, batch.trace_slot + 16);
   if (batch.has_peer_sig) {
     __syncthreads();
     if (threadIdx.x == 0) peer_signal_last_cta(batch.peer_sig, gridDim.x);
@@ -108,7 +108,7 @@
   }
 }
 void gemm_wide_begin(GemmWideBatch& b, const PeerSignal* sig) {
-  b.n = 0; b.total_tiles = 0; b.pdl = 0; b.trace = nullptr; b.has_peer_sig = sig ? 1 : 0;
+  b.n = 0; b.total_tiles = 0; b.pdl = 0; b.trace = nullptr; b.trace_slot = STEP_SLOT_DW; b.has_peer_sig = sig ? 1 : 0;
   if (sig) b.peer_sig = *sig;
 }
 void gemm_wide_add(GemmWideBatch& b, const GemmProblem& pin) {
diff --git a/d4pg-pytorch_b200/csrc/learner.cu b/d4pg-pytorch_b200/csrc/learner.cu
--- a/d4pg-pytorch_b200/csrc/learner.cu
+++ b/d4pg-pytorch_b200/csrc/learner.cu
@@ -125,10 +125,11 @@
   int64_t steps_done;
   int kernels_per_step;
   cudaStream_t side; cudaEvent_t ev_fork, ev_join;
-  ChainArgs chain_fwd_args, chain_bwd_args;
+  cudaStream_t side2; cudaEvent_t ev_fork3, ev_join3, ev_dx_p, ev_dw_c, ev_norm;
+  ChainArgs chain_fwd_args, chain_bwd_args, chain_bwd_c_args;
   uint8_t* tcc_images; TccPackArgs tcc_pack_fwd, tcc_pack_dx; TccImage tcc_img[32];
   cudaEvent_t ev_fork2, ev_join2;
-  TccArgs tcc_fwd_args, tcc_bwd_args;
+  TccArgs tcc_fwd_args, tcc_bwd_args, tcc_bwd_c_args;
   GemmWideBatch dw_batch;
   double* host_u[4]; int32_t* host_pos[4]; float* host_losses; cudaEvent_t ev_in, ev_out, ev_h2d[4];
   int64_t host_steps;
@@ -230,6 +231,7 @@
   int B, S, A, N, Sp, Ap, Np;
   Exchange xm; PeerInfo peers; int gpar;
   float *Ga, *Gc;
+  bool split;
   int nk;
 };
 static bool peer_exchange(const Step& x) { return x.xm >= XCHG_PULL; }
@@ -271,8 +273,9 @@
   return D4PG_OK;
 }
 
-static void tcc_begin(const Step& x, TccArgs& a, int step_slot) {
-  tcc_args_begin(a, x.B, reinterpret_cast<uint8_t*>(x.w.xchg), x.c.precision == 1 ? 3 : 1);
+static void tcc_begin(const Step& x, TccArgs& a, int step_slot, int xchg_chain = 0) {
+  uint8_t* xchg = reinterpret_cast<uint8_t*>(x.w.xchg + xchg_chain * (tcc_xchg_floats(x.B) / TCC_MAX_CHAINS));
+  tcc_args_begin(a, x.B, xchg, x.c.precision == 1 ? 3 : 1);
   a.step_slot = step_slot;
 }
 static int tcc_fwd_group(TccArgs& fa, int ci, int sl, const Step& x, Net net, int l, float* C, int ldc, int publish) {
@@ -511,12 +514,14 @@
   l = tcc_slot_begin(ba, ci); tcc_slot_src_plane(ba, ci, l, p1, 8);
   tcc_slot_group(ba, ci, l, U[U_A_D2], EPI_RELU_MASK, nullptr, w.h1[3], H, w.a_dz1, H, 0);
 }
-static int backward_tc_chain(Step& x) {
-  D4PG_CUDA_OK(cudaStreamWaitEvent(x.st, x.L->ev_join2, 0));
-  TccArgs& ba = x.L->tcc_bwd_args;
-  tcc_begin(x, ba, 5);
-  tcc_build_bwd_C(ba, 0, x);
-  if (!x.h7) tcc_build_bwd_P(ba, 1, x);
+static int backward_tc_chain(Step& x, bool critic, bool policy) {
+  d4pg_learner* L = x.L;
+  D4PG_CUDA_OK(cudaStreamWaitEvent(x.st, L->ev_join2, 0));
+  const bool branch = critic && x.split;
+  TccArgs& ba = branch ? L->tcc_bwd_c_args : L->tcc_bwd_args;
+  tcc_begin(x, ba, branch ? STEP_SLOT_CRITIC_DX : STEP_SLOT_DX, critic ? 0 : 1);
+  if (critic) tcc_build_bwd_C(ba, 0, x);
+  if (policy) tcc_build_bwd_P(ba, critic ? 1 : 0, x);
   RUN("launch_mlp_tc_chain", true, launch_mlp_tc_chain(ba, x.st));
   return D4PG_OK;
 }
@@ -524,31 +529,41 @@
 static ChainSlot chain_layer_dx(const LayerDx& d, int epi, const float* aux, int ldaux, float* C, int ldc, int publish) {
   return chain_dx(d.W, d.ldw, d.n_in, d.k_out, epi, aux, ldaux, C, ldc, publish);
 }
-static int backward_chain(Step& x) {
+static int backward_chain(Step& x, bool critic, bool policy) {
   d4pg_learner* L = x.L; const Workspace& w = x.w;
   const int H = D4PG_HIDDEN, Ap = x.Ap, Np = x.Np;
-  ChainArgs& cb = L->chain_bwd_args;
-  chain_args_begin(cb, x.B, w.xchg, x.c.precision); cb.trace_base = 6 * CHAIN_MAX_SLOTS;
+  const bool branch = critic && x.split;
+  ChainArgs& cb = branch ? L->chain_bwd_c_args : L->chain_bwd_args;
+  chain_args_begin(cb, x.B, w.xchg + (critic ? 0 : chain_xchg_floats(x.B) / CHAIN_MAX), x.c.precision);
+  cb.trace_base = branch ? 160 : 6 * CHAIN_MAX_SLOTS;
+  cb.step_slot = branch ? STEP_SLOT_CRITIC_DX : STEP_SLOT_DX;
   ChainSlot sl; int t;
-  sl = chain_layer_dx(layer_dx(L, CRITIC, 3), EPI_RELU_MASK, w.h3[2], H, w.c_dz22, H, 1); chain_src_global(sl, w.dlogits_q, Np); t = chain_add(cb, 0, sl);
-  sl = chain_layer_dx(layer_dx(L, CRITIC, 2), EPI_RELU_MASK, w.h2[2], H, w.c_dz2, H, 1); chain_src_plane(sl, t); t = chain_add(cb, 0, sl);
-  sl = chain_layer_dx(layer_dx(L, CRITIC, 1), EPI_RELU_MASK, w.h1[2], H, w.c_dz1, H, 0); chain_src_plane(sl, t); chain_add(cb, 0, sl);
-
-  sl = chain_layer_dx(layer_dx(L, CRITIC, 3), EPI_RELU_MASK, w.h3[4], H, w.p_dz22, H, 1); chain_src_global(sl, w.dlogits_pi, Np); t = chain_add(cb, 1, sl);
-  sl = chain_layer_dx(layer_dx(L, CRITIC, 2), EPI_RELU_MASK, w.h2[4], H, w.p_dz2, H, 1); chain_src_plane(sl, t); t = chain_add(cb, 1, sl);
-  const LayerDx da = critic_fc2_action_dx(L);
-  if (chain_pre_ok(x.c)) {
-    sl = chain_layer_dx(layer_dx(L, ACTOR, 3), EPI_RELU_MASK, w.h3[3], H, w.a_dz22, H, 1);
-    chain_pre_layer(sl, da.W, da.ldw, nullptr, w.out[3], Ap, da.n_in, da.k_out, EPI_TANH_MASK, w.a_dz3, Ap, t, H, true);
-    t = chain_add(cb, 1, sl);
-  } else {
-    sl = chain_layer_dx(da, EPI_TANH_MASK, w.out[3], Ap, w.a_dz3, Ap, 1); chain_src_plane(sl, t); t = chain_add(cb, 1, sl);
-    sl = chain_layer_dx(layer_dx(L, ACTOR, 3), EPI_RELU_MASK, w.h3[3], H, w.a_dz22, H, 1); chain_src_plane(sl, t); t = chain_add(cb, 1, sl);
-  }
-  sl = chain_layer_dx(layer_dx(L, ACTOR, 2), EPI_NONE, nullptr, 0, w.a_dh2, H, 1); chain_src_plane(sl, t); t = chain_add(cb, 1, sl);
-  sl = chain_layer_dx(layer_dx(L, ACTOR, 1), EPI_RELU_MASK, w.h1[3], H, w.a_dz1, H, 0); chain_src_plane(sl, t); chain_add(cb, 1, sl);
+  if (critic) {
+    sl = chain_layer_dx(layer_dx(L, CRITIC, 3), EPI_RELU_MASK, w.h3[2], H, w.c_dz22, H, 1); chain_src_global(sl, w.dlogits_q, Np); t = chain_add(cb, 0, sl);
+    sl = chain_layer_dx(layer_dx(L, CRITIC, 2), EPI_RELU_MASK, w.h2[2], H, w.c_dz2, H, 1); chain_src_plane(sl, t); t = chain_add(cb, 0, sl);
+    sl = chain_layer_dx(layer_dx(L, CRITIC, 1), EPI_RELU_MASK, w.h1[2], H, w.c_dz1, H, 0); chain_src_plane(sl, t); chain_add(cb, 0, sl);
+  }
+  if (policy) {
+    const int cp = critic ? 1 : 0;
+    sl = chain_layer_dx(layer_dx(L, CRITIC, 3), EPI_RELU_MASK, w.h3[4], H, w.p_dz22, H, 1); chain_src_global(sl, w.dlogits_pi, Np); t = chain_add(cb, cp, sl);
+    sl = chain_layer_dx(layer_dx(L, CRITIC, 2), EPI_RELU_MASK, w.h2[4], H, w.p_dz2, H, 1); chain_src_plane(sl, t); t = chain_add(cb, cp, sl);
+    const LayerDx da = critic_fc2_action_dx(L);
+    if (chain_pre_ok(x.c)) {
+      sl = chain_layer_dx(layer_dx(L, ACTOR, 3), EPI_RELU_MASK, w.h3[3], H, w.a_dz22, H, 1);
+      chain_pre_layer(sl, da.W, da.ldw, nullptr, w.out[3], Ap, da.n_in, da.k_out, EPI_TANH_MASK, w.a_dz3, Ap, t, H, true);
+      t = chain_add(cb, cp, sl);
+    } else {
+      sl = chain_layer_dx(da, EPI_TANH_MASK, w.out[3], Ap, w.a_dz3, Ap, 1); chain_src_plane(sl, t); t = chain_add(cb, cp, sl);
+      sl = chain_layer_dx(layer_dx(L, ACTOR, 3), EPI_RELU_MASK, w.h3[3], H, w.a_dz22, H, 1); chain_src_plane(sl, t); t = chain_add(cb, cp, sl);
+    }
+    sl = chain_layer_dx(layer_dx(L, ACTOR, 2), EPI_NONE, nullptr, 0, w.a_dh2, H, 1); chain_src_plane(sl, t); t = chain_add(cb, cp, sl);
+    sl = chain_layer_dx(layer_dx(L, ACTOR, 1), EPI_RELU_MASK, w.h1[3], H, w.a_dz1, H, 0); chain_src_plane(sl, t); chain_add(cb, cp, sl);
+  }
   RUN("launch_mlp_chain", true, launch_mlp_chain(cb, x.st));
   return D4PG_OK;
+}
+static int backward_dx(Step& x, bool critic, bool policy) {
+  return x.L->plan == PLAN_TC_CHAIN ? backward_tc_chain(x, critic, policy) : backward_chain(x, critic, policy);
 }
 
 static GemmProblem dw_problem(const Step& x, Net net, int l) {
@@ -578,6 +593,7 @@
   PeerSignal sig1{};
   if (peer_exchange(x)) sig1 = comm_peer_signal(x.peers, 0);
   gemm_wide_begin(gw, peer_exchange(x) ? &sig1 : nullptr);
+  if (x.split && !actor) gw.trace_slot = STEP_SLOT_CRITIC_DW;
   if (critic) gemm_wide_add(gw, dw_problem(x, CRITIC, 2));
   if (critic) gemm_wide_add(gw, dw_problem(x, CRITIC, 1));
   if (actor) gemm_wide_add(gw, dw_problem(x, ACTOR, 2));
@@ -679,20 +695,31 @@
   }
   aa.w1 = float(1.0 - c.beta1); aa.w2 = float(1.0 - c.beta2); aa.beta2 = float(c.beta2); aa.eps = float(c.adam_eps);
   aa.tau = float(c.tau); aa.one_minus_tau = float(1.0 - c.tau); aa.grad_scale = 1.0f; aa.clock = x.w.clock;
-  aa.pipe_slot = x.pf ? x.par : -1;
+  aa.pipe_slot = x.pf ? x.par : -1; aa.trace_slot = STEP_SLOT_ADAM;
   aa.loss_rows = x.w.loss_rows; aa.pi_rows = x.w.pi_rows; aa.B = x.B; aa.inv_count = 1.0f / float(x.B); aa.loss_out = b.losses;
   return aa;
 }
+static int run_grad_sqnorm(Step& x, const AdamArgs& a) {
+  RUN("launch_grad_sqnorm", true, launch_grad_sqnorm(a, x.st));
+  return D4PG_OK;
+}
+static int run_adam(Step& x, const AdamArgs& a) {
+  RUN("launch_adam", false, launch_adam(a, x.st));
+  return D4PG_OK;
+}
 static int launch_update(Step& x, const AdamArgs& a) {
-  if (adam_clips(a)) RUN("launch_grad_sqnorm", true, launch_grad_sqnorm(a, x.st));
-  RUN("launch_adam", false, launch_adam(a, x.st));
-  return D4PG_OK;
+  if (adam_clips(a))
+    if (int rc = run_grad_sqnorm(x, a)) return rc;
+  return run_adam(x, a);
+}
+static AdamArgs critic_update(const AdamArgs& aa) {
+  AdamArgs ac = aa;
+  ac.seg[0] = aa.seg[1]; ac.nseg = 1; ac.skip_tail = 1;
+  return ac;
 }
 static int post_update_half(Step& x, const AdamArgs& aa) {
   d4pg_learner* L = x.L; const Workspace& w = x.w;
-  AdamArgs ac = aa;
-  ac.seg[0] = aa.seg[1]; ac.nseg = 1; ac.skip_tail = 1;
-  if (int rc = launch_update(x, ac)) return rc;
+  if (int rc = launch_update(x, critic_update(aa))) return rc;
   RUN("launch_tcc_pack", false, launch_tcc_pack(L->tcc_pack_dx, x.st));
   TccArgs& fb = L->tcc_fwd_args;
   tcc_begin(x, fb, 1);
@@ -700,7 +727,7 @@
   RUN("launch_mlp_tc_chain", true, launch_mlp_tc_chain(fb, x.st));
   if (int rc = launch_step_heads(x, true)) return rc;
   TccArgs& bb = L->tcc_bwd_args;
-  tcc_begin(x, bb, 5);
+  tcc_begin(x, bb, STEP_SLOT_DX);
   tcc_build_bwd_P(bb, 0, x);
   RUN("launch_mlp_tc_chain", true, launch_mlp_tc_chain(bb, x.st));
   if (int rc = dw_wide(x, false, true)) return rc;
@@ -715,7 +742,41 @@
   return launch_update(x, aa);
 }
 
-static int enqueue_step(d4pg_learner* L, cudaStream_t st, int par, bool cold, bool pack_fwd) {
+static int split_tail(Step& x) {
+  d4pg_learner* L = x.L;
+  const AdamArgs aa = adam_args(x);
+  const bool clips = adam_clips(aa);
+  D4PG_CUDA_OK(cudaEventRecord(L->ev_fork3, x.st));
+  D4PG_CUDA_OK(cudaStreamWaitEvent(L->side2, L->ev_fork3, 0));
+  Step y = x; y.st = L->side2; y.nk = 0;
+  if (int rc = backward_dx(y, true, false)) return rc;
+  if (int rc = dw_wide(y, true, false)) return rc;
+  if (clips) D4PG_CUDA_OK(cudaEventRecord(L->ev_dw_c, y.st));
+  if (int rc = backward_dx(x, false, true)) return rc;
+  if (L->plan == PLAN_CHAIN) {
+    D4PG_CUDA_OK(cudaEventRecord(L->ev_dx_p, x.st));
+    D4PG_CUDA_OK(cudaStreamWaitEvent(y.st, L->ev_dx_p, 0));
+  }
+  if (int rc = dw_wide(x, false, true)) return rc;
+  if (clips) {
+    D4PG_CUDA_OK(cudaStreamWaitEvent(x.st, L->ev_dw_c, 0));
+    if (int rc = run_grad_sqnorm(x, aa)) return rc;
+    D4PG_CUDA_OK(cudaEventRecord(L->ev_norm, x.st));
+    D4PG_CUDA_OK(cudaStreamWaitEvent(y.st, L->ev_norm, 0));
+  }
+  AdamArgs ac = critic_update(aa);
+  ac.trace_slot = STEP_SLOT_CRITIC_ADAM;
+  if (int rc = run_adam(y, ac)) return rc;
+  D4PG_CUDA_OK(cudaEventRecord(L->ev_join3, y.st));
+  x.nk += y.nk;
+  AdamArgs ab = aa;
+  ab.nseg = 1;
+  if (int rc = run_adam(x, ab)) return rc;
+  D4PG_CUDA_OK(cudaStreamWaitEvent(x.st, L->ev_join3, 0));
+  return D4PG_OK;
+}
+
+static int enqueue_step(d4pg_learner* L, cudaStream_t st, int par, bool cold, bool pack_fwd, bool split_ok = false) {
   const d4pg_learner_config_t& c = L->cfg;
   const bool pf = piped(c);
   Step x{L, st, c, L->buf, L->ws, L->ws.batch[par], par, cold, pf, (c.loss_flags & 4) != 0,
@@ -727,11 +788,14 @@
   if (!rc) rc = launch_step_heads(x, false);
   if (!rc && side) rc = side_branch(x);
   if (!rc) rc = choose_gradient_buffers(x);
-  if (!rc && plan == PLAN_TC_CHAIN) rc = backward_tc_chain(x);
-  if (!rc && plan == PLAN_CHAIN) rc = backward_chain(x);
-  if (!rc) rc = plan == PLAN_LEVELS ? backward_levels(x) : dw_wide(x, true, !x.h7);
-  if (!rc) rc = exchange_gradients(x);
-  if (!rc) rc = update(x);
+  x.split = split_ok && plan != PLAN_LEVELS && !x.h7 && x.xm == XCHG_NONE;
+  if (!rc && x.split) rc = split_tail(x);
+  else if (!rc) {
+    rc = plan == PLAN_LEVELS ? backward_levels(x) : backward_dx(x, true, !x.h7);
+    if (!rc && plan != PLAN_LEVELS) rc = dw_wide(x, true, !x.h7);
+    if (!rc) rc = exchange_gradients(x);
+    if (!rc) rc = update(x);
+  }
   if (rc) return rc;
   if (side) D4PG_CUDA_OK(cudaStreamWaitEvent(st, L->ev_join, 0));
   L->kernels_per_step = x.nk;
@@ -864,7 +928,13 @@
       cudaEventCreateWithFlags(&L->ev_fork, cudaEventDisableTiming) != cudaSuccess ||
       cudaEventCreateWithFlags(&L->ev_join, cudaEventDisableTiming) != cudaSuccess ||
       cudaEventCreateWithFlags(&L->ev_fork2, cudaEventDisableTiming) != cudaSuccess ||
-      cudaEventCreateWithFlags(&L->ev_join2, cudaEventDisableTiming) != cudaSuccess) {
+      cudaEventCreateWithFlags(&L->ev_join2, cudaEventDisableTiming) != cudaSuccess ||
+      cudaStreamCreateWithFlags(&L->side2, cudaStreamNonBlocking) != cudaSuccess ||
+      cudaEventCreateWithFlags(&L->ev_fork3, cudaEventDisableTiming) != cudaSuccess ||
+      cudaEventCreateWithFlags(&L->ev_join3, cudaEventDisableTiming) != cudaSuccess ||
+      cudaEventCreateWithFlags(&L->ev_dx_p, cudaEventDisableTiming) != cudaSuccess ||
+      cudaEventCreateWithFlags(&L->ev_dw_c, cudaEventDisableTiming) != cudaSuccess ||
+      cudaEventCreateWithFlags(&L->ev_norm, cudaEventDisableTiming) != cudaSuccess) {
     set_error("d4pg_learner_create: stream/event creation failed"); delete L; return D4PG_ECUDA;
   }
   trace_set_side_stream(L->side);
@@ -880,7 +950,9 @@
   for (int i = 0; i < 4; ++i) if (L->graph_exec[i]) cudaGraphExecDestroy(L->graph_exec[i]);
   for (int i = 0; i < 2; ++i) if (L->multi_exec[i]) cudaGraphExecDestroy(L->multi_exec[i]);
   cudaEventDestroy(L->ev_fork); cudaEventDestroy(L->ev_join); cudaEventDestroy(L->ev_fork2); cudaEventDestroy(L->ev_join2);
-  cudaStreamDestroy(L->side);
+  cudaEventDestroy(L->ev_fork3); cudaEventDestroy(L->ev_join3); cudaEventDestroy(L->ev_dx_p);
+  cudaEventDestroy(L->ev_dw_c); cudaEventDestroy(L->ev_norm);
+  cudaStreamDestroy(L->side); cudaStreamDestroy(L->side2);
   if (L->tcc_images) cudaFree(L->tcc_images);
   if (L->gtab) cudaFree(L->gtab);
   if (L->ing) { cudaStreamSynchronize(L->ing); cudaStreamDestroy(L->ing); }
@@ -1075,7 +1147,7 @@
       if (!L->multi_ready[par]) {
         const int rc = capture_graph(st, &L->multi_exec[par], "d4pg_learner_run", [&] {
           int rc = D4PG_OK;
-          for (int i = 0; i < RUN_UNROLL && rc == D4PG_OK; ++i) rc = enqueue_step(L, st, par ^ (i & 1), false, i == 0);
+          for (int i = 0; i < RUN_UNROLL && rc == D4PG_OK; ++i) rc = enqueue_step(L, st, par ^ (i & 1), false, i == 0, true);
           return rc;
         });
         if (rc) return rc;
diff --git a/d4pg-pytorch_b200/csrc/mlp_chain.cu b/d4pg-pytorch_b200/csrc/mlp_chain.cu
--- a/d4pg-pytorch_b200/csrc/mlp_chain.cu
+++ b/d4pg-pytorch_b200/csrc/mlp_chain.cu
@@ -213,7 +213,7 @@
 }
 void chain_args_begin(ChainArgs& a, int B, float* xchg, int precision) {
   a = ChainArgs{};
-  a.B = B; a.row_blocks = cdiv(B, CHAIN_ROWS); a.xchg = xchg; a.precision = precision;
+  a.B = B; a.row_blocks = cdiv(B, CHAIN_ROWS); a.xchg = xchg; a.precision = precision; a.step_slot = 1;
   a.a_floats = precision ? GEMM_WARPS * BM * CHAIN_RED_PITCH : GEMM_WARPS * BM * BN;
   a.w_floats = 0;
 }
@@ -294,7 +294,6 @@
   }
   a.trace = chain_trace_buffer() ? chain_trace_buffer() + a.trace_base : nullptr;
   a.step_trace = chain_trace_buffer() ? chain_trace_buffer() + STEP_TRACE_BASE : nullptr;
-  a.step_slot = a.trace_base ? 5 : 1;
   { const char* e = getenv("D4PG_TRACE_CTA"); a.trace_cta = e ? atoi(e) : 0; if (a.trace_cta >= a.nchains * a.row_blocks * CHAIN_CLUSTER) a.trace_cta = 0; }
   cudaLaunchConfig_t cfg{};
   cfg.gridDim = dim3(a.nchains * a.row_blocks * CHAIN_CLUSTER); cfg.blockDim = dim3(GEMM_THREADS);
diff --git a/d4pg-pytorch_b200/csrc/mlp_chain.cuh b/d4pg-pytorch_b200/csrc/mlp_chain.cuh
--- a/d4pg-pytorch_b200/csrc/mlp_chain.cuh
+++ b/d4pg-pytorch_b200/csrc/mlp_chain.cuh
@@ -58,7 +58,7 @@
 struct GemmWideBatch {
   GemmProblem p[GEMM_WIDE_MAX];
   int n, total_tiles, pdl;
-  unsigned long long* trace;
+  unsigned long long* trace; int trace_slot;
   PeerSignal peer_sig; int has_peer_sig;
 };
 void gemm_wide_begin(GemmWideBatch& b, const PeerSignal* sig = nullptr);
diff --git a/d4pg-pytorch_b200/csrc/mlp_tc_chain.cu b/d4pg-pytorch_b200/csrc/mlp_tc_chain.cu
--- a/d4pg-pytorch_b200/csrc/mlp_tc_chain.cu
+++ b/d4pg-pytorch_b200/csrc/mlp_tc_chain.cu
@@ -536,7 +536,7 @@
   }
   a.watchdog = tcc_watchdog_device();
   unsigned long long* dbg = debug_trace_buffer();
-  a.trace = dbg ? dbg + (a.step_slot == 5 ? 384 : 256) : nullptr;
+  a.trace = dbg ? dbg + (a.step_slot == STEP_SLOT_DX ? 384 : a.step_slot == STEP_SLOT_CRITIC_DX ? 160 : 256) : nullptr;
   a.step_trace = dbg ? dbg + STEP_TRACE_BASE : nullptr;
   { const char* e = getenv("D4PG_TRACE_CTA"); a.trace_cta = e ? atoi(e) : 0; if (a.trace_cta >= a.nchains * a.row_blocks * TCC_CLUSTER) a.trace_cta = 0; }
   cudaLaunchConfig_t cfg{};
```
